# parseablehq/parseable

Measured on AMD Instinct MI355X. Metric: rows/sec scanned (SELECT...WHERE...GROUP BY, Parseable parquet dialect), higher is better.
Workload: dtype int64; 1 GPU; c2s; query=SELECT host,count(*),max(latency) WHERE ts BETWEEN ... GROUP BY host, rows_per_gpu=100000000, parallelism=dp1

## Files before the change

### include/gpuq.h

```cpp
#ifndef GPUQ_H
#define GPUQ_H

#include <stdint.h>

#ifdef __cplusplus
extern "C" {
#endif

typedef struct gpuq_ctx gpuq_ctx;
typedef struct gpuq_plan gpuq_plan;

#ifndef ARROW_C_DATA_INTERFACE
#define ARROW_C_DATA_INTERFACE
struct ArrowSchema {
  const char* format;
  const char* name;
  const char* metadata;
  int64_t flags;
  int64_t n_children;
  struct ArrowSchema** children;
  struct ArrowSchema* dictionary;
  void (*release)(struct ArrowSchema*);
  void* private_data;
};
struct ArrowArray {
  int64_t length;
  int64_t null_count;
  int64_t offset;
  int64_t n_buffers;
  int64_t n_children;
  const void** buffers;
  struct ArrowArray** children;
  struct ArrowArray* dictionary;
  void (*release)(struct ArrowArray*);
  void* private_data;
};
#endif
#ifndef ARROW_C_STREAM_INTERFACE
#define ARROW_C_STREAM_INTERFACE
struct ArrowArrayStream {
  int (*get_schema)(struct ArrowArrayStream*, struct ArrowSchema* out);
  int (*get_next)(struct ArrowArrayStream*, struct ArrowArray* out);
  const char* (*get_last_error)(struct ArrowArrayStream*);
  void (*release)(struct ArrowArrayStream*);
  void* private_data;
};
#endif


typedef struct {
  const char* path;
  const int32_t* row_groups;
  int32_t n_row_groups;
} gpuq_file;

typedef enum {
  GPUQ_EQ = 0, GPUQ_NE, GPUQ_LT, GPUQ_LE, GPUQ_GT, GPUQ_GE,
  GPUQ_BETWEEN,
  GPUQ_CONTAINS,
  GPUQ_ICONTAINS = 8,
  GPUQ_STARTS_WITH,
  GPUQ_ENDS_WITH,
  GPUQ_NOT_CONTAINS,
  GPUQ_NOT_ICONTAINS,
  GPUQ_NOT_STARTS_WITH,
  GPUQ_NOT_ENDS_WITH,
  GPUQ_IS_NULL,
  GPUQ_IS_NOT_NULL
} gpuq_op;

typedef enum { GPUQ_LIT_I64 = 0, GPUQ_LIT_F64, GPUQ_LIT_STR } gpuq_lit;

typedef struct {
  const char* column;
  int32_t op;
  int32_t lit_kind;
  int64_t i64[2];
  double f64[2];
  const char* str;
  int32_t hi_exclusive;
} gpuq_pred;

typedef enum {
  GPUQ_AGG_COUNT_STAR = 0, GPUQ_AGG_COUNT, GPUQ_AGG_SUM,
  GPUQ_AGG_MIN, GPUQ_AGG_MAX,
  GPUQ_AGG_COUNT_DISTINCT
} gpuq_agg_op;

typedef struct { int32_t op; const char* column; } gpuq_agg;


gpuq_ctx* gpuq_session_create(uint64_t device_mask);
void gpuq_session_destroy(gpuq_ctx*);
const char* gpuq_last_error(gpuq_ctx*);


gpuq_plan* gpuq_plan_build(gpuq_ctx*,
    const gpuq_file* files, int32_t n_files,
    const char* const* projection, int32_t n_projection,
    const gpuq_pred* preds, int32_t n_preds,
    const char* const* group_by, int32_t n_group_by,
    const gpuq_agg* aggs, int32_t n_aggs,
    int64_t limit);

gpuq_plan* gpuq_plan_build_from_stream(gpuq_ctx*, const char* stream_dir,
    const char* const* projection, int32_t n_projection,
    const gpuq_pred* preds, int32_t n_preds,
    const char* const* group_by, int32_t n_group_by,
    const gpuq_agg* aggs, int32_t n_aggs, int64_t limit,
    int64_t* fast_count);

int32_t gpuq_plan_partition_count(gpuq_plan*);

int32_t gpuq_plan_load(gpuq_plan*, int32_t partition);

int32_t gpuq_plan_execute(gpuq_plan*, int32_t partition,
                          struct ArrowArrayStream* out);

typedef struct {
  int64_t rows_scanned;
  int64_t rows_out;
  int64_t bytes_scanned;
  int64_t rowgroup_bytes_total;
  int64_t hbm_bytes_est;
  int64_t kernel_ns;
  int64_t exec_ns;
  int64_t load_ns;
  int64_t decomp_ns;
  int64_t cache_hit_bytes;
} gpuq_metrics;
int32_t gpuq_plan_metrics(gpuq_plan*, gpuq_metrics* out);

void gpuq_plan_destroy(gpuq_plan*);

int32_t gpuq_device_count(void);



typedef struct {
  int32_t codec;
  const uint8_t* comp;
  uint32_t comp_len;
  uint32_t uncomp_len;
} gpuq_decomp_page;

enum {
  GPUQ_DECOMP_AUTO = 0,
  GPUQ_DECOMP_FORCE_SEGMENT,
  GPUQ_DECOMP_FORCE_LITPAR,
  GPUQ_DECOMP_FORCE_FALLBACK
};
#define GPUQ_DECOMP_HOST_ONLY   0x100
#define GPUQ_DECOMP_HOST_REPLAY 0x200

enum {
  GPUQ_DECOMP_PAGE_SEGMENT = 0,
  GPUQ_DECOMP_PAGE_LITPAR,
  GPUQ_DECOMP_PAGE_FALLBACK,
  GPUQ_DECOMP_PAGE_RAW,
  GPUQ_DECOMP_PAGE_HOST_IMAGE
};

typedef struct {
  int32_t mode;
  uint32_t n_seq;
  uint32_t n_segs, n_big;
  uint32_t n_lit_lane, n_lit_wave;
  uint32_t n_inl;
  uint32_t n_res_lane, n_res_wave;
  uint32_t n_pieces;
  uint32_t n_backrefs, n_far;
} gpuq_decomp_stats;

int32_t gpuq_test_decompress(gpuq_ctx*, const gpuq_decomp_page* pages,
                             int32_t n_pages, int32_t raw_lead, int32_t mode,
                             uint8_t sentinel, uint8_t* out, uint64_t out_cap,
                             uint64_t* arena_len, uint64_t* guard_len,
                             gpuq_decomp_stats* stats, int32_t* d_err);

#ifdef __cplusplus
}
#endif
#endif
```

### parseable_amd/_lib.py

```python

from __future__ import annotations

import ctypes as C
import os

_DIR = os.path.dirname(os.path.abspath(__file__))
LIB_PATH = os.path.join(_DIR, "libgpuq.so")


class GpuqFile(C.Structure):
    _fields_ = [
        ("path", C.c_char_p),
        ("row_groups", C.POINTER(C.c_int32)),
        ("n_row_groups", C.c_int32),
    ]


class GpuqPred(C.Structure):
    _fields_ = [
        ("column", C.c_char_p),
        ("op", C.c_int32),
        ("lit_kind", C.c_int32),
        ("i64", C.c_int64 * 2),
        ("f64", C.c_double * 2),
        ("str", C.c_char_p),
        ("hi_exclusive", C.c_int32),
    ]


class GpuqAgg(C.Structure):
    _fields_ = [("op", C.c_int32), ("column", C.c_char_p)]


class GpuqMetrics(C.Structure):
    _fields_ = [
        ("rows_scanned", C.c_int64),
        ("rows_out", C.c_int64),
        ("bytes_scanned", C.c_int64),
        ("rowgroup_bytes_total", C.c_int64),
        ("hbm_bytes_est", C.c_int64),
        ("kernel_ns", C.c_int64),
        ("exec_ns", C.c_int64),
        ("load_ns", C.c_int64),
        ("decomp_ns", C.c_int64),
        ("cache_hit_bytes", C.c_int64),
    ]


class GpuqDecompPage(C.Structure):
    _fields_ = [
        ("codec", C.c_int32),
        ("comp", C.c_void_p),
        ("comp_len", C.c_uint32),
        ("uncomp_len", C.c_uint32),
    ]


class GpuqDecompStats(C.Structure):
    _fields_ = [("mode", C.c_int32)] + [
        (n, C.c_uint32) for n in (
            "n_seq", "n_segs", "n_big", "n_lit_lane", "n_lit_wave", "n_inl",
            "n_res_lane", "n_res_wave", "n_pieces", "n_backrefs", "n_far")
    ]


DECOMP_MODES = {"auto": 0, "segment": 1, "litpar": 2, "fallback": 3}
DECOMP_HOST_ONLY = 0x100
DECOMP_HOST_REPLAY = 0x200
DECOMP_PATHS = ("segment", "litpar", "fallback", "raw", "host_image")
CODECS = {"uncompressed": 0, "snappy": 1, "lz4_raw": 7}

OPS = {"eq": 0, "ne": 1, "lt": 2, "le": 3, "gt": 4, "ge": 5, "between": 6, "contains": 7,
       "icontains": 8, "starts_with": 9, "ends_with": 10, "not_contains": 11,
       "not_icontains": 12, "not_starts_with": 13, "not_ends_with": 14,
       "is_null": 15, "is_not_null": 16}
STR_OPS = ("contains", "icontains", "starts_with", "ends_with", "not_contains",
           "not_icontains", "not_starts_with", "not_ends_with")
NULL_OPS = ("is_null", "is_not_null")
AGGS = {"count_star": 0, "count": 1, "sum": 2, "min": 3, "max": 4,
        "count_distinct": 5}

_lib = None


def load():
    global _lib
    if _lib is not None:
        return _lib
    if not os.path.exists(LIB_PATH):
        raise RuntimeError(
            f"libgpuq.so not built at {LIB_PATH} — run __graft_entry__.build(). "
            "parseable_amd has no CPU fallback."
        )
    lib = C.CDLL(LIB_PATH)
    lib.gpuq_session_create.restype = C.c_void_p
    lib.gpuq_session_create.argtypes = [C.c_uint64]
    lib.gpuq_session_destroy.argtypes = [C.c_void_p]
    lib.gpuq_last_error.restype = C.c_char_p
    lib.gpuq_last_error.argtypes = [C.c_void_p]
    lib.gpuq_device_count.restype = C.c_int32
    lib.gpuq_plan_build_from_stream.restype = C.c_void_p
    lib.gpuq_plan_build_from_stream.argtypes = [
        C.c_void_p, C.c_char_p,
        C.POINTER(C.c_char_p), C.c_int32,
        C.POINTER(GpuqPred), C.c_int32,
        C.POINTER(C.c_char_p), C.c_int32,
        C.POINTER(GpuqAgg), C.c_int32,
        C.c_int64, C.POINTER(C.c_int64),
    ]
    lib.gpuq_plan_build.restype = C.c_void_p
    lib.gpuq_plan_build.argtypes = [
        C.c_void_p,
        C.POINTER(GpuqFile), C.c_int32,
        C.POINTER(C.c_char_p), C.c_int32,
        C.POINTER(GpuqPred), C.c_int32,
        C.POINTER(C.c_char_p), C.c_int32,
        C.POINTER(GpuqAgg), C.c_int32,
        C.c_int64,
    ]
    lib.gpuq_plan_partition_count.restype = C.c_int32
    lib.gpuq_plan_partition_count.argtypes = [C.c_void_p]
    lib.gpuq_plan_load.restype = C.c_int32
    lib.gpuq_plan_load.argtypes = [C.c_void_p, C.c_int32]
    lib.gpuq_plan_execute.restype = C.c_int32
    lib.gpuq_plan_execute.argtypes = [C.c_void_p, C.c_int32, C.c_void_p]
    lib.gpuq_plan_metrics.restype = C.c_int32
    lib.gpuq_plan_metrics.argtypes = [C.c_void_p, C.POINTER(GpuqMetrics)]
    lib.gpuq_plan_destroy.argtypes = [C.c_void_p]
    lib.gpuq_test_decompress.restype = C.c_int32
    lib.gpuq_test_decompress.argtypes = [
        C.c_void_p, C.POINTER(GpuqDecompPage), C.c_int32, C.c_int32, C.c_int32,
        C.c_uint8, C.c_void_p, C.c_uint64,
        C.POINTER(C.c_uint64), C.POINTER(C.c_uint64),
        C.POINTER(GpuqDecompStats), C.POINTER(C.c_int32),
    ]
    _lib = lib
    return lib


def device_count() -> int:
    return load().gpuq_device_count()


def decompress_pages(pages, mode="auto", raw_lead=0, host=None, session=None,
                     sentinel=0xA5):
    lib = load()
    n = len(pages)
    arr = (GpuqDecompPage * max(n, 1))()
    keep = []
    cap = 16384 + 64
    for i, (codec, comp, uncomp) in enumerate(pages):
        buf = C.create_string_buffer(bytes(comp), max(len(comp), 1))
        keep.append(buf)
        arr[i] = GpuqDecompPage(CODECS[codec], C.addressof(buf), len(comp), uncomp)
        cap += (uncomp + 15) & ~15
    flags = DECOMP_MODES[mode] | {None: 0, "decode": DECOMP_HOST_ONLY,
                                  "replay": DECOMP_HOST_REPLAY}[host]
    out = C.create_string_buffer(cap)
    arena_len, guard_len, d_err = C.c_uint64(), C.c_uint64(), C.c_int32()
    stats = (GpuqDecompStats * max(n, 1))()
    rc = lib.gpuq_test_decompress(
        session if host is None else None, arr, n, raw_lead, flags, sentinel,
        out, cap, C.byref(arena_len), C.byref(guard_len), stats, C.byref(d_err))
    if rc != 0:
        msg = lib.gpuq_last_error(session if host is None else None)
        raise RuntimeError(msg.decode(errors="replace"))
    st = []
    for i in range(n):
        d = {f: getattr(stats[i], f) for f, _ in GpuqDecompStats._fields_}
        d["mode"] = DECOMP_PATHS[d["mode"]]
        st.append(d)
    return out.raw[:arena_len.value], st, guard_len.value, d_err.value
```

### parseable_amd/csrc/dev_types.h

```cpp
#pragma once
#include <cstdint>

namespace gpuq {

struct DevPage {
  uint64_t src_off;
  uint64_t dst_off;
  uint32_t comp_size;
  uint32_t uncomp_size;
  uint32_t num_values;
  uint32_t row_start;
  uint32_t aux;
  uint32_t aux_val;
  uint32_t aux_lut;
  uint32_t dict_n;
  uint8_t  optional;
  uint8_t  raw_copy;
  uint8_t  encoding;
  uint8_t  phys;
};

struct DevSeg {
  uint64_t src_off;
  uint64_t dst_off;
  uint32_t comp_len;
  uint32_t out_len;
  uint8_t big;
  uint8_t raw;
};
struct DevBr {
  uint64_t dst, src;
  uint32_t len;
  uint32_t _pad;
};
struct DevPageBr { uint32_t start, count; };
struct DevBrRes {
  uint64_t dst;
  uint32_t len, off;
  uint32_t piece_start, piece_n;
};
struct DevPiece { uint64_t src; uint32_t len; uint32_t _pad; };
struct DevLit { uint64_t a, b; };
struct DevBrInl { uint64_t meta, pat; };
struct DevCWin {
  uint64_t src;
  uint64_t starts;
  uint32_t nbytes;
  uint32_t n_values;
  uint32_t dense0;
  int32_t page_id;
};

enum CmpMode { CMP_EQ = 0, CMP_NE, CMP_LT, CMP_LE, CMP_GT, CMP_GE, CMP_RANGE };

enum StrKind { STR_CONTAINS = 0, STR_PREFIX = 1, STR_SUFFIX = 2 };
enum { STRF_KIND = 3, STRF_FOLD = 4, STRF_NEG = 8 };
enum { CMP_STR_LIKE = 16 };
constexpr int cmp_str_like(int mode) { return CMP_STR_LIKE | mode; }
constexpr int cmp_str_like_mode(int op) {
  return (op & CMP_STR_LIKE) ? (op & ~CMP_STR_LIKE) : -1;
}

enum { AGGK_COUNT_STAR = 0, AGGK_COUNT, AGGK_SUM_I64, AGGK_SUM_F64,
       AGGK_MIN_I64, AGGK_MAX_I64, AGGK_MIN_F64, AGGK_MAX_F64,
       AGGK_MIN_RANK, AGGK_MAX_RANK,
       AGGK_MIN_STR, AGGK_MAX_STR,
       AGGK_COUNT_DISTINCT };

constexpr int MAX_KEYS = 4;
constexpr int MAX_AGGS = 8;

struct AggArgs {
  const uint8_t* mask;
  int64_t n_rows;
  int n_keys;
  const int32_t* key_gid[MAX_KEYS];
  int32_t key_size[MAX_KEYS];
  int n_aggs;
  int32_t agg_kind[MAX_AGGS];
  const int64_t* agg_val[MAX_AGGS];
  const uint8_t* agg_valid[MAX_AGGS];
  uint8_t cnt_skip[MAX_AGGS];
  int32_t fsum_idx[MAX_AGGS];
  int32_t fsum_n;
  uint64_t* fsum;
  const uint8_t* dec;
  uint64_t* table;
  int32_t n_groups;
  int32_t* err;
};

struct DistinctArgs {
  const uint8_t* mask;
  int64_t n_rows;
  int n_keys;
  const int32_t* key_gid[MAX_KEYS];
  int32_t key_size[MAX_KEYS];
  int32_t n_groups;
  const int32_t* vgid;
  int32_t vcard;
  uint64_t* pairs;
  uint32_t* count;
  uint32_t pair_cap;
  int32_t* err;
};

enum { ERR_NONE = 0, ERR_LZ4 = 1, ERR_RLE = 2, ERR_DELTA = 3, ERR_DICT_RANGE = 4,
       ERR_PAGE = 5, ERR_FSUM_RANGE = 6, ERR_HASH_CAP = 7, ERR_HASH_PROBE = 8,
       ERR_PAIR_CAP = 9, ERR_PAIR_PROBE = 10, ERR_DISTINCT_CAP = 11,
       ERR_DISTINCT_PROBE = 12 };

}
```

### parseable_amd/csrc/gpuq.cpp

```cpp
#include "../../include/gpuq.h"
#include "catalog.h"
#include "meta.h"
#include "kernels_api.h"
#include "dev_types.h"

#include <hip/hip_runtime.h>
#include <fcntl.h>
#include <sys/mman.h>
#include <sys/stat.h>
#include <unistd.h>

#include <algorithm>
#include <array>
#include <atomic>
#include <cstring>
#include <thread>
#include <map>
#include <memory>
#include <mutex>
#include <string>
#include <unordered_map>
#include <vector>

using namespace gpuq;
// ... 42 lines not shown
    std::lock_guard<std::mutex> g(cache_mu);
    auto it = cache.find(key);
    if (it == cache.end() || it->second.bytes != expect_bytes) return false;
    it->second.refs++;
    it->second.last_use = ++cache_clock;
    return true;
  }
  void cache_unpin(const std::string& key) {
    std::lock_guard<std::mutex> g(cache_mu);
    auto it = cache.find(key);
    if (it != cache.end() && it->second.refs > 0) it->second.refs--;
  }
  void* cache_get(const std::string& key) {
    std::lock_guard<std::mutex> g(cache_mu);
    auto it = cache.find(key);
    return it == cache.end() ? nullptr : it->second.dev;
  }
  void cache_put(const std::string& key, void* dev, size_t bytes, int device) {
    std::lock_guard<std::mutex> g(cache_mu);
    if (cache.count(key)) { (void)hipFree(dev); return; }
    while (cache_bytes + bytes > cache_budget) {
      auto victim = cache.end();
      for (auto it = cache.begin(); it != cache.end(); ++it)
        if (it->second.refs == 0 &&
            (victim == cache.end() ||
             it->second.last_use < victim->second.last_use))
          victim = it;
      if (victim == cache.end()) break;
      (void)hipSetDevice(victim->second.device);
      (void)hipFree(victim->second.dev);
      cache_bytes -= victim->second.bytes;
      cache.erase(victim);
    }
    CacheEntry e;
    e.dev = dev;
    e.bytes = bytes;
    e.device = device;
    e.last_use = ++cache_clock;
    cache.emplace(key, e);
    cache_bytes += bytes;
  }
};

namespace {

struct MappedFile {
  std::string path;
  int fd = -1;
  const uint8_t* data = nullptr;
  size_t size = 0;
  int64_t mtime_ns = 0;
  FileMeta meta;
  ~MappedFile() {
    if (data) munmap((void*)data, size);
    if (fd >= 0) close(fd);
  }
};

struct ColPlan {
  std::string name;
  int phys = -1;
  bool optional = false;
  bool need_gid = false;
  bool need_val = false;
  bool val_always = false;
  bool hash_mode = false;
  bool numeric_key = false;
  bool need_gid_valid = false;
  bool distinct_val = false;
  std::vector<int> lut_preds;
  std::vector<int> cmp_preds;
  std::vector<int> contains_preds;
  std::vector<int> null_preds;
  bool need_rank = false;
  bool is_bin = false;
  int bin_src = -1;
  int64_t bin_stride = 0, bin_origin = 0, bin_min_idx = 0;
  int32_t nbins = 0;
  std::vector<int32_t> rank_to_gid;
  std::vector<std::string> gdict;
  std::unordered_map<std::string, int32_t> gmap;
  int32_t gid_of(const std::string& s) {
    auto it = gmap.find(s);
    if (it != gmap.end()) return it->second;
    gdict.push_back(s);
    int32_t id = (int32_t)gdict.size();
    gmap.emplace(gdict.back(), id);
    return id;
  }
};

struct PredPlan {
  gpuq_pred p;
  std::string col, str_lit;
};

struct AggPlan {
  int op;
  std::string col;
  int col_idx = -1;
  int kind = 0;
  bool is_f64 = false;
  bool cnt_is_presence = false;
  int fsum_idx = -1;
};

struct ChunkTask {
  int file_idx, rg_idx, col_idx;
  size_t dictv_pool_base = (size_t)-1;
  uint64_t raw_off = 0;
  const ColumnChunkMeta* cm = nullptr;
  std::vector<PageInfo> pages;
  std::vector<int32_t> remap;
  std::vector<int64_t> dictv;
  std::vector<uint8_t> lut;
  bool has_plain_data_pages = false;
  std::vector<int64_t> strof;
  std::vector<int64_t> pvals;
  std::vector<uint32_t> pval_page_n;
  std::vector<uint32_t> pval_base;
  uint64_t dict_dst = (uint64_t)-1;
  std::string cache_key;
  bool cached = false;
  uint64_t dec_base = 0, dec_len = 0;
};

struct RgRef {
  int file_idx, rg_idx;
  int64_t rows = 0, needed_bytes = 0, total_bytes = 0;
  uint32_t row_start = 0;
};

enum TaskKind { TK_DICT_GID, TK_DICT_VAL, TK_PLAIN_VAL, TK_DELTA_VAL,
                TK_DICT_MASK, TK_BYTES_CONTAINS, TK_POOL_VAL,
                TK_IS_NULL, TK_IS_NOT_NULL,
                TK_N };

struct Partition {
  int device = -1;
  std::vector<RgRef> rgs;
  int64_t n_rows = 0;
  std::vector<ChunkTask> chunks;
  std::vector<DevPage> pages;
  std::vector<int32_t> ids[TK_N];
  std::map<std::pair<int,int>, std::vector<int32_t>> tasks;
  std::vector<int32_t> remap_pool;
  std::vector<int64_t> dictv_pool;
  std::vector<uint8_t> lut_pool;
  std::vector<DevSeg> segs;
  std::vector<DevBr> brs;
  std::vector<DevPageBr> pagebrs;
  std::vector<DevBrRes> res_lane, res_wave;
  std::vector<DevPiece> piece_pool;
  std::vector<DevBrInl> brinl;
  std::vector<DevLit> lits_lane, lits_wave;
  std::vector<DevCWin> cwins;
  std::vector<uint16_t> cstarts;
  std::map<int, std::pair<uint32_t, uint32_t>> cwin_ranges;
  uint64_t raw_bytes = 0, dec_bytes = 0;
  int64_t bytes_scanned = 0, rowgroup_bytes_total = 0;
  int64_t bytes_cache_hit = 0;
  bool populated = false;
  std::map<int, std::vector<std::pair<int64_t, int64_t>>> pred_ranges;
  std::vector<std::pair<uint64_t, std::vector<uint8_t>>> himgs;

  bool loaded = false;
  hipStream_t stream = nullptr;
  uint8_t *d_raw = nullptr, *d_dec = nullptr;
  DevPage* d_pages = nullptr;
  int32_t* d_remap = nullptr;
  int64_t* d_dictv = nullptr;
  uint8_t* d_lut = nullptr;
  uint8_t* d_mask = nullptr;
  int32_t* d_err = nullptr;
  uint64_t* d_table = nullptr;
  uint64_t* d_fsum = nullptr;
  uint64_t* d_hkeys = nullptr;
  int32_t* d_hgids = nullptr;
  uint32_t* d_hcount = nullptr;
  std::map<int, uint64_t*> d_gid2ref;
  std::map<int, uint32_t> hash_claimed;
  int32_t* d_cgid = nullptr;
  std::vector<uint64_t*> d_gid2pair;
  int32_t* d_agg_kind = nullptr;
  uint8_t* d_needle = nullptr;
  std::vector<uint32_t> needle_off;
  uint32_t* d_rowof = nullptr;
  uint32_t* d_rank = nullptr;
  uint8_t* d_scr = nullptr;
  uint32_t* d_present = nullptr;
  uint8_t* d_tmpvalid = nullptr;
  int32_t* d_all_ids = nullptr;
  DevSeg* d_segs = nullptr;
  DevBr* d_brs = nullptr;
  DevPageBr* d_pagebrs = nullptr;
  DevBrRes* d_res_lane = nullptr;
  DevBrRes* d_res_wave = nullptr;
  DevBrInl* d_brinl = nullptr;
  DevPiece* d_piece_pool = nullptr;
  DevLit* d_lits_lane = nullptr;
  DevLit* d_lits_wave = nullptr;
  DevCWin* d_cwins = nullptr;
  uint16_t* d_cstarts = nullptr;
  int64_t* d_keys = nullptr;
  int64_t* d_keys_sorted = nullptr;
  uint32_t* d_rows = nullptr;
  uint32_t* d_rows_sorted = nullptr;
  unsigned long long* d_count = nullptr;
  void* d_sort_temp = nullptr;
  size_t sort_temp_bytes = 0;
  std::map<std::pair<int,int>, int32_t*> d_ids;
  std::map<int, int32_t*> d_gid;
  std::map<int, int64_t*> d_val;
  std::map<int, uint8_t*> d_valid;
  std::vector<uint8_t> col_null_free;
  std::vector<int32_t> valagg_ids;
  int32_t* d_valagg_ids = nullptr;
  uint64_t* d_dbitmap = nullptr;
  std::vector<uint64_t*> d_dpairs;
  uint32_t* d_dcount = nullptr;
  int64_t load_ns = 0;
};

struct Ring {
  static constexpr size_t BUFSZ = 256ull << 20;
  static constexpr int NBUF = 4;
  void* bufs[NBUF] = {};
  hipEvent_t evts[NBUF] = {};
  hipStream_t stream;
  int b = 0;
  explicit Ring(hipStream_t st);
  ~Ring();
  struct Span { const uint8_t* src; uint64_t len; };
  void copy_spans(uint8_t* d_dst, const std::vector<Span>& spans);
  void copy(void* d_dst, const void* src, size_t len);
};

}

namespace {
constexpr int HASH_LOG2 = 24;
constexpr int32_t GID_CAP = 1 << 22;
constexpr uint32_t DISTINCT_PAIR_CAP = 1u << 23;
constexpr uint64_t DISTINCT_BITMAP_BITS = 1ull << 28;
constexpr uint64_t DISTINCT_LDS_BITS = 1ull << 17;
}

struct gpuq_plan {
  gpuq_ctx* ctx = nullptr;
  std::vector<std::unique_ptr<MappedFile>> files;
  std::vector<ColPlan> cols;
  std::vector<PredPlan> preds;
  std::vector<AggPlan> aggs;
  std::vector<int> group_cols;
  std::vector<int> projection;
  bool is_projection = false;
  int ts_col = -1;
  int64_t limit = -1;
  std::vector<Partition> parts;
  int32_t n_groups = 0;
  int32_t n_fsum = 0;
  bool has_hash = false;
  bool needs_cascade = false;
  bool has_numkey = false;
  std::vector<std::string> pinned_keys;
  int64_t m_cache_hit_bytes = 0;
  bool fused_count = false;
  bool fused_valagg = false;
  int valagg_col = -1;
  bool valagg_late = false;
  int valagg_blocks = 1024;
  bool exec_dbg = false;
  std::vector<int> distinct_aggs;
  uint64_t distinct_bitmap_bits = DISTINCT_BITMAP_BITS;
  uint64_t distinct_lds_bits = DISTINCT_LDS_BITS;
  uint32_t distinct_pair_cap = DISTINCT_PAIR_CAP;
  bool distinct_force_hash = false;
  std::mutex mu;
  int64_t m_rows_scanned = 0, m_rows_out = 0, m_kernel_ns = 0, m_exec_ns = 0,
          m_load_ns = 0, m_decomp_ns = 0, m_hbm_est = 0;
  ~gpuq_plan();
};

extern "C" gpuq_ctx* gpuq_session_create(uint64_t device_mask) {
  auto* c = new gpuq_ctx();
  int n = 0;
  if (hipGetDeviceCount(&n) != hipSuccess) n = 0;
  if (n == 0 && getenv("GPUQ_FAKE_DEVICE")) n = 1;
  for (int i = 0; i < 64 && i < n; i++)
    if (device_mask & (1ull << i)) c->devices.push_back(i);
  if (c->devices.empty() && device_mask == 0 && n > 0) c->devices.push_back(0);
  return c;
}
extern "C" void gpuq_session_destroy(gpuq_ctx* c) { delete c; }
namespace {
thread_local std::string g_null_ctx_error = "null ctx";
}
extern "C" const char* gpuq_last_error(gpuq_ctx* c) {
  return c ? c->last_error.c_str() : g_null_ctx_error.c_str();
}
extern "C" int32_t gpuq_device_count(void) {
  int n = 0;
  if (hipGetDeviceCount(&n) != hipSuccess) return -1;
  return n;
}

namespace {

int find_or_add_col(std::vector<ColPlan>& cols, const std::string& name) {
  for (size_t i = 0; i < cols.size(); i++)
    if (cols[i].name == name) return (int)i;
  cols.push_back(ColPlan{});
  cols.back().name = name;
  return (int)cols.size() - 1;
}

bool op_is_like(int op) {
  return op == GPUQ_CONTAINS || (op >= GPUQ_ICONTAINS && op <= GPUQ_NOT_ENDS_WITH);
}
bool op_is_null(int op) { return op == GPUQ_IS_NULL || op == GPUQ_IS_NOT_NULL; }
int like_mode(int op) {
  switch (op) {
    case GPUQ_ICONTAINS: return STR_CONTAINS | STRF_FOLD;
    case GPUQ_STARTS_WITH: return STR_PREFIX;
    case GPUQ_ENDS_WITH: return STR_SUFFIX;
    case GPUQ_NOT_CONTAINS: return STR_CONTAINS | STRF_NEG;
    case GPUQ_NOT_ICONTAINS: return STR_CONTAINS | STRF_FOLD | STRF_NEG;
    case GPUQ_NOT_STARTS_WITH: return STR_PREFIX | STRF_NEG;
    case GPUQ_NOT_ENDS_WITH: return STR_SUFFIX | STRF_NEG;
    default: return STR_CONTAINS;
  }
}
const char* op_name(int op) {
  static const char* names[] = {
      "eq", "ne", "lt", "le", "gt", "ge", "between", "contains", "icontains",
      "starts_with", "ends_with", "not_contains", "not_icontains",
      "not_starts_with", "not_ends_with", "is_null", "is_not_null"};
  return (op >= 0 && op <= GPUQ_IS_NOT_NULL) ? names[op] : "?";
}

enum NullState { NULLP_EVAL = 0, NULLP_PROVEN, NULLP_UNSAT };
NullState null_pred_state(int op, const ColumnChunkMeta& cm, bool optional) {
  const bool none_null = !optional || cm.null_count == 0;
  const bool all_null = optional && cm.null_count >= 0 &&
                        cm.null_count == cm.num_values && cm.num_values > 0;
  if (op == GPUQ_IS_NOT_NULL)
    return none_null ? NULLP_PROVEN : all_null ? NULLP_UNSAT : NULLP_EVAL;
  return none_null ? NULLP_UNSAT : all_null ? NULLP_PROVEN : NULLP_EVAL;
}

bool rg_pruned_by_stats(const gpuq_plan& plan, const FileMeta& fm,
                        const RowGroupMeta& rg) {
  for (const auto& pp : plan.preds) {
// ... 97 lines not shown
  if (codec == CODEC_LZ4_RAW) {
    int n = lz4_decompress_host(src, comp, buf.data(), buf.size());
    if (n == (int)uncomp) return buf.data();
    if (comp == uncomp) return src;
    throw std::runtime_error("page lz4 failure");
  }
  if (codec == CODEC_SNAPPY) {
    int n = snappy_decompress_host(src, comp, buf.data(), buf.size());
    if (n == (int)uncomp) return buf.data();
    throw std::runtime_error("page snappy failure");
  }
  throw std::runtime_error("unsupported codec");
}

uint32_t parse_def1(const uint8_t* data, uint32_t nv, std::vector<uint8_t>& defs) {
  uint32_t dl;
  memcpy(&dl, data, 4);
  defs.assign(nv, 1);
  const uint8_t* p = data + 4;
  const uint8_t* end = p + dl;
  uint32_t v = 0;
  while (v < nv && p < end) {
    uint64_t hdr = 0;
    int sh = 0;
    for (;;) {
      uint8_t b = *p++;
      hdr |= (uint64_t)(b & 0x7f) << sh;
      if (!(b & 0x80)) break;
      sh += 7;
    }
    if (hdr & 1) {
      uint32_t groups = (uint32_t)(hdr >> 1);
      for (uint32_t g = 0; g < groups; g++) {
        uint8_t byte = p[g];
        for (int j = 0; j < 8; j++) {
          uint32_t idx = v + g * 8 + j;
          if (idx < nv) defs[idx] = (byte >> j) & 1;
        }
      }
      p += groups;
      uint32_t add = groups * 8;
      v += add > nv - v ? nv - v : add;
    } else {
      uint32_t cnt = (uint32_t)(hdr >> 1);
      uint8_t val = *p++;
      if (cnt > nv - v) cnt = nv - v;
      std::fill(defs.begin() + v, defs.begin() + v + cnt, val);
      v += cnt;
    }
  }
  return 4 + dl;
}

int64_t now_ns() {
  struct timespec ts;
  clock_gettime(CLOCK_MONOTONIC, &ts);
  return (int64_t)ts.tv_sec * 1000000000 + ts.tv_nsec;
}

template <class F>
void parallel_for(size_t n, F&& fn, size_t max_threads = 0) {
  if (n == 0) return;
  size_t hw = std::thread::hardware_concurrency();
  if (hw == 0) hw = 8;
  static const size_t env_cap = [] {
    const char* e = getenv("GPUQ_HOST_THREADS");
    return e ? (size_t)strtoul(e, nullptr, 10) : (size_t)0;
  }();
  if (env_cap) hw = std::min(hw, env_cap);
  if (max_threads) hw = std::min(hw, max_threads);
  size_t nthreads = std::min(n, hw);
  if (nthreads <= 1) {
    for (size_t i = 0; i < n; i++) fn(i);
    return;
  }
  std::atomic<size_t> next{0};
  std::mutex emu;
  std::exception_ptr eptr;
  auto worker = [&]() {
    for (;;) {
      size_t i = next.fetch_add(1);
      if (i >= n) return;
      try {
        fn(i);
      } catch (...) {
        std::lock_guard<std::mutex> g(emu);
        if (!eptr) eptr = std::current_exception();
        next.store(n);
        return;
      }
    }
  };
  std::vector<std::thread> pool;
  pool.reserve(nthreads);
  for (size_t t = 0; t < nthreads; t++) pool.emplace_back(worker);
  for (auto& th : pool) th.join();
  if (eptr) std::rethrow_exception(eptr);
}

Ring::Ring(hipStream_t st) : stream(st) {
  for (int i = 0; i < NBUF; i++) {
    HIP_TRY(hipHostMalloc(&bufs[i], BUFSZ));
    HIP_TRY(hipEventCreate(&evts[i]));
    HIP_TRY(hipEventRecord(evts[i], stream));
  }
}
Ring::~Ring() {
  for (int i = 0; i < NBUF; i++) {
    if (bufs[i]) (void)hipHostFree(bufs[i]);
    if (evts[i]) (void)hipEventDestroy(evts[i]);
  }
}
void Ring::copy_spans(uint8_t* d_dst, const std::vector<Span>& spans) {
  size_t si = 0;
  uint64_t soff = 0, dst = 0;
  while (si < spans.size()) {
    if (spans[si].len == 0) { si++; continue; }
    HIP_TRY(hipEventSynchronize(evts[b]));
    struct Fill { const uint8_t* src; uint8_t* dstp; size_t len; };
    std::vector<Fill> fills;
    size_t filled = 0;
    while (si < spans.size() && filled < BUFSZ) {
      uint64_t take = std::min<uint64_t>(spans[si].len - soff, BUFSZ - filled);
      while (take > 0) {
        uint64_t piece = std::min<uint64_t>(take, 4ull << 20);
        fills.push_back({spans[si].src + soff, (uint8_t*)bufs[b] + filled,
                         piece});
        filled += piece;
        soff += piece;
        take -= piece;
      }
      if (soff == spans[si].len) { si++; soff = 0; }
    }
    parallel_for(fills.size(), [&](size_t f) {
      memcpy(fills[f].dstp, fills[f].src, fills[f].len);
    }, 32);
    HIP_TRY(hipMemcpyAsync(d_dst + dst, bufs[b], filled,
                           hipMemcpyHostToDevice, stream));
    HIP_TRY(hipEventRecord(evts[b], stream));
    dst += filled;
    b = (b + 1) % NBUF;
  }
}
void Ring::copy(void* d_dst, const void* src, size_t len) {
  if (len) copy_spans((uint8_t*)d_dst, {{(const uint8_t*)src, len}});
}

struct DecompRecs {
  std::vector<DevSeg> segs;
  std::vector<DevBr> brs;
  std::vector<DevPageBr> pagebrs;
  std::vector<DevBrRes> res_lane, res_wave;
  std::vector<DevPiece> piece_pool;
  std::vector<DevBrInl> brinl;
  std::vector<DevLit> lits_lane, lits_wave;
  std::vector<std::pair<uint64_t, std::vector<uint8_t>>> himgs;
};

constexpr uint32_t BR_FAR = 16384 / 2;

void plan_decomp_page(DecompRecs& cb, int codec, const uint8_t* praw,
                      uint64_t src_abs, uint64_t dst_abs, uint32_t comp,
                      uint32_t uncomp, bool raw_page,
                      int force = GPUQ_DECOMP_AUTO,
                      gpuq_decomp_stats* st = nullptr) {
  Lz4Plan lp;
  if (st) *st = gpuq_decomp_stats{};
  if (!raw_page && codec == CODEC_SNAPPY) {
    lp = snappy_walk(praw, comp, uncomp);
    if (st) st->n_seq = lp.n_seq;
    if (lp.fallback) {
      std::vector<uint8_t> img(uncomp);
      if (snappy_decompress_host(praw, comp, img.data(), uncomp) !=
          (int)uncomp)
        throw std::runtime_error("snappy page decode failure");
      cb.himgs.emplace_back(dst_abs, std::move(img));
      if (st) st->mode = GPUQ_DECOMP_PAGE_HOST_IMAGE;
      return;
    }
  } else if (!raw_page) {
    static const bool env_fb =
        std::getenv("GPUQ_FORCE_LZ4_FALLBACK") != nullptr;
    const bool force_fb = force == GPUQ_DECOMP_FORCE_FALLBACK ||
                          (force == GPUQ_DECOMP_AUTO && env_fb);
    try {
      lp = lz4_walk(praw, comp, uncomp, 8192);
      if (force_fb) {
        lp.fallback = true;
        lp.resolved.clear();
        lp.pieces.clear();
      }
      const bool want_litpar =
          force == GPUQ_DECOMP_FORCE_LITPAR ||
          (force == GPUQ_DECOMP_AUTO && lp.n_seq >= 256 &&
           uncomp / lp.n_seq < 96);
      if (!lp.fallback && want_litpar) {
        Lz4Plan lp2 = lz4_walk(praw, comp, uncomp, 8192, true);
        if (!lp2.fallback) lp = std::move(lp2);
      }
    } catch (const std::exception&) {
      if (comp == uncomp) raw_page = true;
      else throw;
    }
    if (st) st->n_seq = lp.n_seq;
  }
  if (raw_page) {
    DevSeg sgl{};
    sgl.src_off = src_abs;
    sgl.dst_off = dst_abs;
    sgl.comp_len = comp;
    sgl.out_len = uncomp;
    sgl.raw = 1;
    cb.segs.push_back(sgl);
    if (st) {
      st->mode = GPUQ_DECOMP_PAGE_RAW;
      st->n_seq = 0;
      st->n_segs = 1;
    }
    return;
  }
  if (st) {
    st->mode = lp.fallback ? GPUQ_DECOMP_PAGE_FALLBACK
               : lp.litpar ? GPUQ_DECOMP_PAGE_LITPAR
                           : GPUQ_DECOMP_PAGE_SEGMENT;
    st->n_segs = (uint32_t)lp.segs.size();
    for (const auto& sg : lp.segs) st->n_big += sg.big != 0;
  }
  for (const auto& sg : lp.segs) {
    DevSeg d2{};
    d2.src_off = src_abs + sg.s_off;
    d2.dst_off = dst_abs + sg.d_off;
    d2.comp_len = sg.comp_len;
    d2.out_len = sg.out_len;
    d2.big = sg.big;
    cb.segs.push_back(d2);
  }
  for (const auto& lt : lp.lits) {
    DevLit dl{(src_abs + lt.src) | ((uint64_t)lt.len << 40),
              dst_abs + lt.dst};
    (lt.len <= 256 ? cb.lits_lane : cb.lits_wave).push_back(dl);
    if (st) (lt.len <= 256 ? st->n_lit_lane : st->n_lit_wave)++;
  }
  if (lp.fallback) {
    DevPageBr pb{(uint32_t)cb.brs.size(), (uint32_t)lp.backrefs.size()};
    cb.pagebrs.push_back(pb);
    for (const auto& br : lp.backrefs) {
      cb.brs.push_back({dst_abs + br.dst, dst_abs + br.src, br.len, 0});
      if (st) {
        st->n_backrefs++;
        st->n_far += (br.dst - br.src) + br.len > BR_FAR;
      }
    }
  } else if (!lp.resolved.empty()) {
    auto lit_bytes = [&](uint32_t src, uint32_t len,
                         uint8_t* out) -> bool {
      const auto& Ls = lp.lits;
      size_t lo = 0, hi = Ls.size();
      while (lo < hi) {
        size_t mid = (lo + hi) / 2;
        if (Ls[mid].dst <= src) lo = mid + 1;
        else hi = mid;
      }
      if (lo == 0) return false;
      const Lz4Lit& L = Ls[lo - 1];
      if (src < L.dst || src + len > L.dst + L.len) return false;
      std::memcpy(out, praw + L.src + (src - L.dst), len);
      return true;
    };
    for (const auto& rr : lp.resolved) {
      uint32_t pat_len = 0;
      for (uint32_t k = 0; k < rr.piece_n; k++)
        pat_len += lp.pieces[rr.piece_start + k].len;
      if (lp.litpar && pat_len > 0 && pat_len <= 8 && rr.len <= 256) {
        uint8_t buf[8] = {0};
        uint32_t o = 0;
        bool ok = true;
        for (uint32_t k = 0; k < rr.piece_n && ok; k++) {
          const Lz4Piece& pc = lp.pieces[rr.piece_start + k];
          ok = lit_bytes(pc.src, pc.len, buf + o);
          o += pc.len;
        }
        if (ok) {
          uint64_t pat;
          std::memcpy(&pat, buf, 8);
          cb.brinl.push_back({(dst_abs + rr.dst) |
                                  ((uint64_t)rr.len << 40) |
                                  ((uint64_t)pat_len << 52),
                              pat});
          if (st) st->n_inl++;
          continue;
        }
      }
      uint32_t ps = (uint32_t)cb.piece_pool.size();
      for (uint32_t k = 0; k < rr.piece_n; k++) {
        const Lz4Piece& pc = lp.pieces[rr.piece_start + k];
        cb.piece_pool.push_back({dst_abs + pc.src, pc.len, 0});
      }
      DevBrRes rec{dst_abs + rr.dst, rr.len, rr.off, ps, rr.piece_n};
      if (rr.len <= 256) cb.res_lane.push_back(rec);
      else cb.res_wave.push_back(rec);
      if (st) {
        (rr.len <= 256 ? st->n_res_lane : st->n_res_wave)++;
        st->n_pieces += rr.piece_n;
      }
    }
  }
}

struct DecompDev {
  const uint8_t* d_raw;
  uint8_t* d_dec;
  const DevSeg* d_segs; int n_segs;
  const DevLit* d_lits_lane; int64_t n_lits_lane;
  const DevLit* d_lits_wave; int n_lits_wave;
  const DevBrInl* d_brinl; int64_t n_brinl;
  const DevBrRes* d_res_lane; int64_t n_res_lane;
  const DevBrRes* d_res_wave; int n_res_wave;
  const DevPiece* d_piece_pool;
  const DevBr* d_brs;
  const DevPageBr* d_pagebrs; int n_pagebrs;
  int32_t* d_err;
};

void launch_decompress(hipStream_t st, const DecompDev& d) {
  launch_lz4_seg(st, d.d_raw, d.d_dec, d.d_segs, d.n_segs, d.d_err);
  launch_lit_lane(st, d.d_raw, d.d_dec, d.d_lits_lane, d.n_lits_lane);
  launch_lit_wave(st, d.d_raw, d.d_dec, d.d_lits_wave, d.n_lits_wave);
  launch_brres_inl(st, d.d_dec, d.d_brinl, d.n_brinl);
  launch_brres_lane(st, d.d_dec, d.d_res_lane, d.d_piece_pool, d.n_res_lane);
  launch_brres_wave(st, d.d_dec, d.d_res_wave, d.d_piece_pool, d.n_res_wave);
  launch_lz4_backrefs(st, d.d_dec, d.d_brs, d.d_pagebrs, d.n_pagebrs);
}

}

extern "C" gpuq_plan* gpuq_plan_build(
    gpuq_ctx* ctx, const gpuq_file* files, int32_t n_files,
    const char* const* projection, int32_t n_projection,
    const gpuq_pred* preds, int32_t n_preds,
    const char* const* group_by, int32_t n_group_by,
    const gpuq_agg* aggs, int32_t n_aggs, int64_t limit) try {
  (void)projection; (void)n_projection;
  auto plan = std::make_unique<gpuq_plan>();
  plan->ctx = ctx;
  plan->limit = limit;
  if (ctx->devices.empty())
    throw std::runtime_error("no GPU devices in session (gpuq never falls back to CPU)");
  if (n_files <= 0)
    throw std::runtime_error("empty file list: caller should use the empty-relation path "
                             "(provider returns the empty aggregate without a scan)");

  plan->files.resize(n_files);
  parallel_for((size_t)n_files, [&](size_t i) {
    auto mf = std::make_unique<MappedFile>();
    mf->path = files[i].path;
    mf->fd = open(files[i].path, O_RDONLY);
    if (mf->fd < 0) throw std::runtime_error("cannot open " + mf->path);
    struct stat st;
    fstat(mf->fd, &st);
    mf->size = st.st_size;
    mf->mtime_ns = (int64_t)st.st_mtim.tv_sec * 1000000000 + st.st_mtim.tv_nsec;
    mf->data = (const uint8_t*)mmap(nullptr, mf->size, PROT_READ, MAP_PRIVATE, mf->fd, 0);
    if (mf->data == MAP_FAILED) throw std::runtime_error("mmap failed: " + mf->path);
    mf->meta = parse_footer(mf->data, mf->size);
    plan->files[i] = std::move(mf);
  });
  const FileMeta& fm0 = plan->files[0]->meta;

  for (int32_t i = 0; i < n_preds; i++) {
    PredPlan pp;
    pp.p = preds[i];
    pp.col = preds[i].column;
    if (pp.p.op < GPUQ_EQ || pp.p.op > GPUQ_IS_NOT_NULL)
      throw std::runtime_error("unknown predicate op on " + pp.col);
    if (!op_is_null(pp.p.op) && preds[i].str) pp.str_lit = preds[i].str;
    plan->preds.push_back(std::move(pp));
  }
  for (int32_t i = 0; i < n_group_by; i++) {
    std::string g = group_by[i];
    if (g.rfind("__bin:", 0) == 0) {
      size_t a = 6, b = g.find(':', a), c2 = g.find(':', b + 1);
      std::string src = g.substr(a, b - a);
      int ci = find_or_add_col(plan->cols, g);
      auto& bc = plan->cols[ci];
      bc.is_bin = true;
      bc.bin_stride = std::stoll(g.substr(b + 1, c2 - b - 1));
      bc.bin_origin = std::stoll(g.substr(c2 + 1));
      if (bc.bin_stride <= 0) throw std::runtime_error("bad bin stride");
      int si = find_or_add_col(plan->cols, src);
      plan->cols[si].need_val = true;
      plan->cols[si].val_always = true;
      plan->cols[ci].bin_src = si;
      plan->group_cols.push_back(ci);
      continue;
    }
    int ci = find_or_add_col(plan->cols, g);
    plan->cols[ci].need_gid = true;
    plan->group_cols.push_back(ci);
  }
  for (int32_t i = 0; i < n_aggs; i++) {
    AggPlan ap;
    ap.op = aggs[i].op;
    if (aggs[i].op == GPUQ_AGG_COUNT_DISTINCT) {
      if (!aggs[i].column)
        throw std::runtime_error("count_distinct needs a column");
      if (n_projection > 0)
        throw std::runtime_error(
            "count_distinct is not allowed in a projection plan");
    }
    if (aggs[i].op != GPUQ_AGG_COUNT_STAR) {
      ap.col = aggs[i].column;
      ap.col_idx = find_or_add_col(plan->cols, ap.col);
    }
    plan->aggs.push_back(std::move(ap));
  }
  for (auto& c : plan->cols) {
    if (c.is_bin) continue;
    int si = fm0.col_index(c.name);
    if (si < 0) throw std::runtime_error("no such column: " + c.name);
    c.phys = fm0.columns[si].phys_type;
    c.optional = fm0.columns[si].optional;
    if (c.need_gid && c.phys != PT_BYTE_ARRAY) {
      if (c.phys == PT_INT64 || c.phys == PT_INT32 || c.phys == PT_DOUBLE) {
        c.need_gid = false;
        c.numeric_key = true;
        c.need_val = true;
        c.val_always = true;
        plan->has_numkey = true;
      } else {
        throw std::runtime_error(
            "unsupported group-key type (utf8/i64/i32/f64/timestamp): " +
            c.name);
      }
    }
  }
  for (size_t pi = 0; pi < plan->preds.size(); pi++) {
    auto& pp = plan->preds[pi];
    int ci = find_or_add_col(plan->cols, pp.col);
    auto& c = plan->cols[ci];
    if (c.phys == -1) {
      int si = fm0.col_index(c.name);
      if (si < 0) throw std::runtime_error("no such column: " + c.name);
      c.phys = fm0.columns[si].phys_type;
      c.optional = fm0.columns[si].optional;
    }
    if (op_is_null(pp.p.op)) {
      if (c.phys != PT_BYTE_ARRAY && c.phys != PT_INT64 &&
          c.phys != PT_INT32 && c.phys != PT_DOUBLE)
        throw std::runtime_error("unsupported predicate column type: " + pp.col);
      c.null_preds.push_back((int)pi);
      continue;
    }
    if (op_is_like(pp.p.op) && pp.p.op != GPUQ_CONTAINS &&
        c.phys != PT_BYTE_ARRAY)
      throw std::runtime_error(std::string("string predicate ") +
                               op_name(pp.p.op) + " on non-utf8 column: " +
                               pp.col);
    if (c.phys == PT_BYTE_ARRAY) {
      if (pp.p.lit_kind != GPUQ_LIT_STR)
        throw std::runtime_error("string column needs string literal: " + pp.col);
      if (op_is_like(pp.p.op) && (like_mode(pp.p.op) & STRF_FOLD)) {
        for (char& ch : pp.str_lit) {
          if ((unsigned char)ch >= 0x80)
            throw std::runtime_error(
                std::string(op_name(pp.p.op)) + " literal must be ASCII "
                "(case folding is ASCII-only): " + pp.col);
          if (ch >= 'A' && ch <= 'Z') ch = (char)(ch | 0x20);
        }
      }
      if (op_is_like(pp.p.op)) c.contains_preds.push_back((int)pi);
      c.lut_preds.push_back((int)pi);
    } else if (c.phys == PT_INT64 || c.phys == PT_INT32) {
      if (pp.p.lit_kind != GPUQ_LIT_I64)
        throw std::runtime_error("int column needs int literal: " + pp.col);
      c.cmp_preds.push_back((int)pi);
      c.need_val = true;
    } else if (c.phys == PT_DOUBLE) {
      if (pp.p.lit_kind != GPUQ_LIT_F64)
        throw std::runtime_error("double column needs float literal: " + pp.col);
      c.cmp_preds.push_back((int)pi);
      c.need_val = true;
// ... 413 lines not shown
        if (pi.type != PAGE_DATA) continue;
        uint64_t pg_dst = part.dec_bytes;
        pid_cursor++;
        part.dec_bytes += ((uint64_t)pi.uncomp_size + 15) & ~15ull;
        if (c.hash_mode && pi.encoding == ENC_PLAIN) {
          t.pval_base.push_back((uint32_t)part.dictv_pool.size());
          uint32_t nvp = t.pval_page_n[plain_i++];
          for (uint32_t k = 0; k < nvp; k++)
            part.dictv_pool.push_back((int64_t)(pg_dst + (uint64_t)t.pvals[pv_off + k]));
          pv_off += nvp;
        }
      }
      t.dec_len = part.dec_bytes - t.dec_base;
      {
        const auto& mf2 = *plan->files[t.file_idx];
        t.cache_key = mf2.path + "\x01" + std::to_string(mf2.size) + ":" +
                      std::to_string(mf2.mtime_ns) + ":" +
                      std::to_string(t.rg_idx) + ":" + c.name +
                      (c.hash_mode ? ":h" : "");
        if (ctx->cache_pin(t.cache_key, (size_t)t.dec_len)) {
          t.cached = true;
          plan->pinned_keys.push_back(t.cache_key);
          part.bytes_cache_hit += (int64_t)t.cm->total_compressed_size;
        }
      }
    }

    phase_mark("phase3 pools+cache");

    struct CItem {
      const uint8_t* praw;
      int32_t comp, uncomp, page_id;
      uint64_t dst_off;
      uint32_t num_values;
      bool optional;
      int codec;
      int col;
    };
    std::vector<CItem> citems;
    struct CB : DecompRecs {
      std::vector<DevPage> pages;
      std::map<std::pair<int,int>, std::vector<int32_t>> tasks;
      std::vector<CItem> citems;
    };
    std::vector<CB> cbs(part.chunks.size());
    parallel_for(part.chunks.size(), [&](size_t ti) {
      auto& t = part.chunks[ti];
      auto& c = plan->cols[t.col_idx];
      auto& cb = cbs[ti];
      const auto& mf = *plan->files[t.file_idx];
      const uint32_t remap_base = bases[ti].remap;
      const uint32_t dictv_base = bases[ti].dictv;
      const uint32_t lut_base = bases[ti].lut;
      uint64_t dec_off = bases[ti].dec;
      int32_t page_id = bases[ti].pid;
      const uint32_t rstart = stubs[ti].rstart;

      const int chunk_codec = t.cm->codec;
      auto plan_decomp = [&](const uint8_t* praw, uint64_t src_abs,
                             uint64_t dst_abs, uint32_t comp, uint32_t uncomp,
                             bool raw_page) {
        plan_decomp_page(cb, chunk_codec, praw, src_abs, dst_abs, comp, uncomp,
                         raw_page);
      };

      if (c.hash_mode) {
        for (auto& pi : t.pages) {
          if (pi.type != PAGE_DICT) continue;
          if (!t.cached)
            plan_decomp(mf.data + pi.payload_off,
                        t.raw_off + (uint64_t)(pi.payload_off - t.cm->start_offset()),
                        t.dict_dst, pi.comp_size, pi.uncomp_size,
                        t.cm->codec == CODEC_UNCOMPRESSED);
          dec_off += ((uint64_t)pi.uncomp_size + 15) & ~15ull;
        }
      }

      uint32_t row_in_rg = 0;
      size_t plain_i4 = 0;
      for (auto& pi : t.pages) {
        if (pi.type != PAGE_DATA) continue;
        DevPage dp{};
        dp.src_off = t.raw_off + (uint64_t)(pi.payload_off - t.cm->start_offset());
        dp.dst_off = dec_off;
        dec_off += ((uint64_t)pi.uncomp_size + 15) & ~15ull;
        dp.comp_size = pi.comp_size;
        dp.uncomp_size = pi.uncomp_size;
        dp.num_values = pi.num_values;
        dp.row_start = rstart + row_in_rg;
        row_in_rg += pi.num_values;
        dp.optional = mf.meta.columns[mf.meta.col_index(c.name)].optional;
        dp.raw_copy = (t.cm->codec == CODEC_UNCOMPRESSED);
        dp.dict_n = (uint32_t)std::max(
            {t.remap.size(), t.dictv.size(), t.lut.size(), t.strof.size()});
        dp.encoding = (uint8_t)pi.encoding;
        dp.phys = (uint8_t)c.phys;
        const int32_t this_pid = page_id++;
        if (!t.cached)
          plan_decomp(mf.data + pi.payload_off, dp.src_off, dp.dst_off,
                      pi.comp_size, pi.uncomp_size, dp.raw_copy != 0);
        bool dict_enc = (pi.encoding == ENC_RLE_DICT || pi.encoding == ENC_PLAIN_DICT);
        if (c.need_gid && dict_enc && !c.hash_mode) {
          dp.aux = remap_base;
          cb.tasks[{TK_DICT_GID, t.col_idx}].push_back(this_pid);
        }
        if (c.need_val && stubs[ti].need_val_decode) {
          if (c.hash_mode) {
            if (dict_enc) {
              dp.aux_val = dictv_base;
              cb.tasks[{TK_DICT_VAL, t.col_idx}].push_back(this_pid);
            } else if (pi.encoding == ENC_PLAIN) {
              dp.aux_val = t.pval_base[plain_i4++];
              cb.tasks[{TK_POOL_VAL, t.col_idx}].push_back(this_pid);
            } else throw std::runtime_error("unsupported encoding for hash col");
          } else if (dict_enc) {
            dp.aux_val = dictv_base;
            cb.tasks[{TK_DICT_VAL, t.col_idx}].push_back(this_pid);
          } else if (pi.encoding == ENC_PLAIN) {
            cb.tasks[{TK_PLAIN_VAL, t.col_idx}].push_back(this_pid);
          } else if (pi.encoding == ENC_DELTA_BP) {
            cb.tasks[{TK_DELTA_VAL, t.col_idx}].push_back(this_pid);
          } else throw std::runtime_error("unsupported encoding for values");
        }
        if (!c.lut_preds.empty() && !c.hash_mode) {
          if (dict_enc) {
            dp.aux_lut = lut_base;
            cb.tasks[{TK_DICT_MASK, t.col_idx}].push_back(this_pid);
          } else if (pi.encoding == ENC_PLAIN) {
            if ((int)c.contains_preds.size() != (int)c.lut_preds.size())
              throw std::runtime_error("non-LIKE predicate on PLAIN utf8 pages: next row");
            cb.tasks[{TK_BYTES_CONTAINS, t.col_idx}].push_back(this_pid);
            cb.citems.push_back({mf.data + pi.payload_off, pi.comp_size,
                                 pi.uncomp_size, this_pid, dp.dst_off,
                                 (uint32_t)pi.num_values, dp.optional != 0,
                                 t.cm->codec, t.col_idx});
          } else throw std::runtime_error("unsupported encoding for string predicate");
        }
        if (stubs[ti].need_is_null)
          cb.tasks[{TK_IS_NULL, t.col_idx}].push_back(this_pid);
        if (stubs[ti].need_is_not_null)
          cb.tasks[{TK_IS_NOT_NULL, t.col_idx}].push_back(this_pid);
        cb.pages.push_back(dp);
      }
      if (row_in_rg != (uint32_t)mf.meta.row_groups[t.rg_idx].num_rows)
        throw std::runtime_error("page rows mismatch");
    });

    phase_mark("phase4 lz4 walks");

    {
      const size_t nc = cbs.size();
      std::vector<size_t> o_pages(nc + 1, 0), o_segs(nc + 1, 0),
          o_brs(nc + 1, 0), o_pagebrs(nc + 1, 0), o_rl(nc + 1, 0),
          o_rw(nc + 1, 0), o_pp(nc + 1, 0), o_bi(nc + 1, 0),
          o_ll(nc + 1, 0), o_lw(nc + 1, 0);
      for (size_t i = 0; i < nc; i++) {
        const auto& cb = cbs[i];
        o_pages[i + 1] = o_pages[i] + cb.pages.size();
        o_segs[i + 1] = o_segs[i] + cb.segs.size();
        o_brs[i + 1] = o_brs[i] + cb.brs.size();
        o_pagebrs[i + 1] = o_pagebrs[i] + cb.pagebrs.size();
        o_rl[i + 1] = o_rl[i] + cb.res_lane.size();
        o_rw[i + 1] = o_rw[i] + cb.res_wave.size();
        o_pp[i + 1] = o_pp[i] + cb.piece_pool.size();
        o_bi[i + 1] = o_bi[i] + cb.brinl.size();
        o_ll[i + 1] = o_ll[i] + cb.lits_lane.size();
        o_lw[i + 1] = o_lw[i] + cb.lits_wave.size();
      }
      part.pages.resize(o_pages[nc]);
      part.segs.resize(o_segs[nc]);
      part.brs.resize(o_brs[nc]);
      part.pagebrs.resize(o_pagebrs[nc]);
      part.res_lane.resize(o_rl[nc]);
      part.res_wave.resize(o_rw[nc]);
      part.piece_pool.resize(o_pp[nc]);
      part.brinl.resize(o_bi[nc]);
      part.lits_lane.resize(o_ll[nc]);
      part.lits_wave.resize(o_lw[nc]);
      parallel_for(nc, [&](size_t i) {
        auto& cb = cbs[i];
        std::copy(cb.pages.begin(), cb.pages.end(),
                  part.pages.begin() + o_pages[i]);
        std::copy(cb.segs.begin(), cb.segs.end(),
                  part.segs.begin() + o_segs[i]);
        std::copy(cb.brs.begin(), cb.brs.end(), part.brs.begin() + o_brs[i]);
        const uint32_t br_base = (uint32_t)o_brs[i];
        for (size_t j = 0; j < cb.pagebrs.size(); j++) {
          DevPageBr pb = cb.pagebrs[j];
          pb.start += br_base;
          part.pagebrs[o_pagebrs[i] + j] = pb;
        }
        std::copy(cb.piece_pool.begin(), cb.piece_pool.end(),
                  part.piece_pool.begin() + o_pp[i]);
        const uint32_t piece_base = (uint32_t)o_pp[i];
        for (size_t j = 0; j < cb.res_lane.size(); j++) {
          DevBrRes r2 = cb.res_lane[j];
          r2.piece_start += piece_base;
          part.res_lane[o_rl[i] + j] = r2;
        }
        for (size_t j = 0; j < cb.res_wave.size(); j++) {
          DevBrRes r2 = cb.res_wave[j];
          r2.piece_start += piece_base;
          part.res_wave[o_rw[i] + j] = r2;
        }
        std::copy(cb.brinl.begin(), cb.brinl.end(),
                  part.brinl.begin() + o_bi[i]);
        std::copy(cb.lits_lane.begin(), cb.lits_lane.end(),
                  part.lits_lane.begin() + o_ll[i]);
        std::copy(cb.lits_wave.begin(), cb.lits_wave.end(),
                  part.lits_wave.begin() + o_lw[i]);
      });
      for (size_t i = 0; i < nc; i++) {
        auto& cb = cbs[i];
        for (auto& [key, ids] : cb.tasks) {
          auto& dstv = part.tasks[key];
          dstv.insert(dstv.end(), ids.begin(), ids.end());
        }
        citems.insert(citems.end(), cb.citems.begin(), cb.citems.end());
        for (auto& h : cb.himgs)
          part.himgs.emplace_back(h.first, std::move(h.second));
      }
    }
    phase_mark("phase5 merge");
    part.dec_bytes += 16384 + 64;

    if (!citems.empty()) {
      struct CLocal {
        std::vector<DevCWin> wins;
        std::vector<uint16_t> starts;
      };
      std::vector<CLocal> locals(citems.size());
      std::atomic<size_t> next{0};
      std::atomic<bool> failed{false};
      auto worker = [&]() {
        std::vector<uint8_t> img, defs;
        for (;;) {
          size_t i = next.fetch_add(1);
          if (i >= citems.size() || failed.load()) return;
          const auto& it = citems[i];
          auto& L = locals[i];
          const uint8_t* data;
          try {
            data = host_page_payload(it.codec, it.praw, it.comp, it.uncomp,
                                     img);
          } catch (const std::exception&) {
            failed.store(true);
            return;
          }
          uint32_t pos = 0;
          const uint32_t nv = it.num_values;
          bool has_def = false;
          if (it.optional) {
            uint32_t dl;
            std::memcpy(&dl, data, 4);
            defs.assign(nv, 1);
            const uint8_t* p = data + 4;
            const uint8_t* end = p + dl;
            uint32_t v = 0;
            while (v < nv && p < end) {
              uint64_t hdr = 0;
              int sh = 0;
              for (;;) {
                uint8_t b = *p++;
                hdr |= (uint64_t)(b & 0x7f) << sh;
                if (!(b & 0x80)) break;
                sh += 7;
              }
              if (hdr & 1) {
                uint32_t groups = (uint32_t)(hdr >> 1);
                for (uint32_t g = 0; g < groups; g++) {
                  uint8_t byte = p[g];
                  for (int j = 0; j < 8; j++) {
                    uint32_t idx = v + g * 8 + j;
                    if (idx < nv) defs[idx] = (byte >> j) & 1;
                  }
                }
                p += groups;
                uint32_t add = groups * 8;
                v += add > nv - v ? nv - v : add;
              } else {
                uint32_t cnt = (uint32_t)(hdr >> 1);
                uint8_t val = *p++;
                if (cnt > nv - v) cnt = nv - v;
                std::fill(defs.begin() + v, defs.begin() + v + cnt, val);
                v += cnt;
              }
            }
            pos = 4 + dl;
            has_def = true;
          }
          uint32_t dense = 0;
          int64_t wfirst = -1;
          uint32_t wbytes = 0, wvals = 0, wdense0 = 0;
          auto flush = [&]() {
            if (wfirst < 0) return;
            L.wins.push_back({it.dst_off + (uint64_t)wfirst,
                              (uint64_t)(L.starts.size() - wvals), wbytes,
                              wvals, wdense0, it.page_id});
            wfirst = -1;
            wbytes = wvals = 0;
          };
          for (uint32_t vI = 0; vI < nv; vI++) {
            if (has_def && !defs[vI]) continue;
            if (pos + 4 > (uint32_t)it.uncomp) { failed.store(true); return; }
            uint32_t len;
            std::memcpy(&len, data + pos, 4);
            uint64_t rec = 4ull + len;
            if (pos + rec > (uint64_t)it.uncomp) { failed.store(true); return; }
            if (rec > 16384) {
              flush();
              L.starts.push_back(0);
              L.wins.push_back({it.dst_off + pos, L.starts.size() - 1,
                                (uint32_t)rec, 1, dense, it.page_id});
            } else {
              if (wfirst >= 0 && wbytes + rec > 16384) flush();
              if (wfirst < 0) { wfirst = pos; wdense0 = dense; }
              L.starts.push_back((uint16_t)(pos - wfirst));
              wbytes += (uint32_t)rec;
              wvals++;
            }
            pos += (uint32_t)rec;
            dense++;
          }
          flush();
        }
      };
      size_t nthreads = std::min<size_t>(
          std::max(1u, std::thread::hardware_concurrency()), citems.size());
      std::vector<std::thread> pool;
      for (size_t i = 0; i < nthreads; i++) pool.emplace_back(worker);
      for (auto& th : pool) th.join();
      if (failed.load())
        throw std::runtime_error("contains window walk failed (corrupt page)");
      std::map<int32_t, size_t> by_page;
      for (size_t i = 0; i < citems.size(); i++) by_page[citems[i].page_id] = i;
      for (auto& [key, ids] : part.tasks) {
        if (key.first != TK_BYTES_CONTAINS) continue;
        uint32_t off = (uint32_t)part.cwins.size();
        for (int32_t pid : ids) {
          const auto& L = locals[by_page.at(pid)];
          uint64_t sbase = part.cstarts.size();
          part.cstarts.insert(part.cstarts.end(), L.starts.begin(),
                              L.starts.end());
          for (DevCWin w : L.wins) {
            w.starts += sbase;
            part.cwins.push_back(w);
          }
        }
        part.cwin_ranges[key.second] = {off, (uint32_t)part.cwins.size() - off};
      }
    }
  }

  for (auto& c : plan->cols) {
    if (!c.is_bin) continue;
    const auto& src = plan->cols[c.bin_src];
    bool any = false;
    int64_t mn = 0, mx = 0;
    for (auto& part : plan->parts)
      for (auto& r : part.rgs) {
        const auto& mf = *plan->files[r.file_idx];
        int si = mf.meta.col_index(src.name);
        const auto& cm = mf.meta.row_groups[r.rg_idx].chunks[si];
        if (!cm.has_i64_stats)
          throw std::runtime_error("DATE_BIN needs footer i64 stats on " + src.name);
        if (!any) { mn = cm.stat_min; mx = cm.stat_max; any = true; }
        else { mn = std::min(mn, cm.stat_min); mx = std::max(mx, cm.stat_max); }
      }
    auto fdiv = [](int64_t v, int64_t s) {
      return v >= 0 ? v / s : -((-v + s - 1) / s);
    };
    c.bin_min_idx = any ? fdiv(mn - c.bin_origin, c.bin_stride) : 0;
    int64_t max_idx = any ? fdiv(mx - c.bin_origin, c.bin_stride) : 0;
    int64_t nb = max_idx - c.bin_min_idx + 1;
    if (nb > (1 << 21)) throw std::runtime_error("too many DATE_BIN bins");
    c.nbins = (int32_t)std::max<int64_t>(nb, 1);
  }

  int64_t g = 1;
  for (int ci : plan->group_cols) {
    const auto& c = plan->cols[ci];
    int64_t sz = c.is_bin ? (int64_t)c.nbins + 1 : (int64_t)c.gdict.size() + 1;
    g = (g > (int64_t)GID_CAP) ? g : g * sz;
  }
  if (g > (int64_t)GID_CAP) {
    plan->needs_cascade = true;
    g = GID_CAP;
  }
  plan->n_groups = (int32_t)g;

  for (auto& part : plan->parts)
    plan->m_rows_scanned += part.n_rows;

  for (auto& ap : plan->aggs) {
    if (ap.op == GPUQ_AGG_COUNT_STAR || ap.col_idx < 0) continue;
    bool all0 = true;
    for (auto& part : plan->parts)
      for (auto& t : part.chunks)
        if (t.col_idx == ap.col_idx && t.cm->null_count != 0) all0 = false;
    ap.cnt_is_presence = all0;
  }

  for (size_t ci = 0; ci < plan->cols.size(); ci++) {
    auto& c = plan->cols[ci];
    if (!c.need_rank) continue;
    std::vector<int32_t> order((size_t)c.gdict.size());
    for (size_t i = 0; i < order.size(); i++) order[i] = (int32_t)i;
    std::sort(order.begin(), order.end(), [&](int32_t a, int32_t b) {
      return c.gdict[a] < c.gdict[b];
    });
    std::vector<int64_t> rank_of_gid(c.gdict.size() + 1, 0);
    c.rank_to_gid.assign(c.gdict.size(), 0);
    for (size_t r = 0; r < order.size(); r++) {
      rank_of_gid[(size_t)order[r] + 1] = (int64_t)r;
      c.rank_to_gid[r] = order[r] + 1;
    }
    for (auto& part : plan->parts)
      for (auto& t : part.chunks)
        if (t.col_idx == (int)ci && t.dictv_pool_base != (size_t)-1)
          for (size_t k = 0; k < t.dictv.size(); k++)
            part.dictv_pool[t.dictv_pool_base + k] =
                rank_of_gid[(size_t)part.dictv_pool[t.dictv_pool_base + k]];
  }

  {
    bool aggs_ok = true;
    for (auto& ap : plan->aggs) aggs_ok &= (ap.kind == AGGK_COUNT_STAR);
    plan->fused_count = plan->group_cols.size() == 1 && aggs_ok &&
                        plan->preds.empty() && plan->n_groups <= 8192 &&
                        !plan->cols[plan->group_cols[0]].is_bin &&
                        !plan->cols[plan->group_cols[0]].hash_mode &&
                        !plan->cols[plan->group_cols[0]].numeric_key;
  }

  for (auto& part : plan->parts) {
    part.col_null_free.assign(plan->cols.size(), 1);
    for (auto& t : part.chunks)
      if (t.cm->null_count != 0) part.col_null_free[t.col_idx] = 0;
  }

  plan->exec_dbg = getenv("GPUQ_PLAN_DEBUG") != nullptr;
  if (const char* e = getenv("GPUQ_VALAGG_BLOCKS"))
    plan->valagg_blocks = std::max(1, atoi(e));
  if (const char* e = getenv("GPUQ_DISTINCT_BITMAP_BITS"))
    plan->distinct_bitmap_bits =
        std::min<uint64_t>(strtoull(e, nullptr, 10), 1ull << 31);
  if (const char* e = getenv("GPUQ_DISTINCT_LDS_BITS"))
    plan->distinct_lds_bits =
        std::min<uint64_t>(strtoull(e, nullptr, 10), 64 * 1024 * 8);
  if (const char* e = getenv("GPUQ_DISTINCT_PAIR_CAP"))
    plan->distinct_pair_cap = (uint32_t)std::min<uint64_t>(
        std::max<uint64_t>(strtoull(e, nullptr, 10), 1), DISTINCT_PAIR_CAP);
  if (const char* e = getenv("GPUQ_DISTINCT_FORCE_HASH"))
    plan->distinct_force_hash = atoi(e) != 0;
  if (!plan->distinct_aggs.empty()) plan->fused_count = false;
  if (!plan->is_projection && !getenv("GPUQ_NO_FUSED_VALAGG") &&
      plan->distinct_aggs.empty() &&
      plan->group_cols.size() == 1 && plan->aggs.size() == 2 &&
      plan->aggs[0].kind == AGGK_COUNT_STAR && plan->n_fsum == 0 &&
      (plan->aggs[1].kind == AGGK_SUM_I64 || plan->aggs[1].kind == AGGK_MIN_I64 ||
       plan->aggs[1].kind == AGGK_MAX_I64) &&
      plan->aggs[1].cnt_is_presence && !plan->needs_cascade) {
    const int vc = plan->aggs[1].col_idx;
    const auto& c = plan->cols[vc];
    const auto& kc = plan->cols[plan->group_cols[0]];
    bool ok = c.phys == PT_INT64 && !c.is_bin && !c.hash_mode &&
              !c.numeric_key && !c.need_gid && !c.need_rank &&
              c.cmp_preds.empty() && c.lut_preds.empty() &&
              c.null_preds.empty() &&
              plan->group_cols[0] != vc;
    for (auto& o : plan->cols) ok &= !(o.is_bin && o.bin_src == vc);
    const bool late = kc.hash_mode || kc.numeric_key;
    if (!late) ok &= (int64_t)plan->n_groups * 16 <= 64 * 1024;
    for (auto& part : plan->parts) {
      if (!ok) break;
      for (auto& kv : part.tasks) {
        if (kv.first.second != vc) continue;
        if (kv.first.first != TK_DICT_VAL && kv.first.first != TK_PLAIN_VAL)
          ok = false;
      }
    }
    if (ok) {
      plan->fused_valagg = true;
      plan->valagg_col = vc;
      plan->valagg_late = late;
      for (auto& part : plan->parts) {
        for (int k : {TK_DICT_VAL, TK_PLAIN_VAL}) {
          auto it = part.tasks.find({k, vc});
          if (it != part.tasks.end())
            part.valagg_ids.insert(part.valagg_ids.end(), it->second.begin(),
                                   it->second.end());
        }
        std::sort(part.valagg_ids.begin(), part.valagg_ids.end());
      }
    }
  }

  if (getenv("GPUQ_PLAN_DEBUG")) {
    fprintf(stderr, "[gpuq plan] fused_count=%d fused_valagg=%d%s\n",
            (int)plan->fused_count, (int)plan->fused_valagg,
            plan->fused_valagg && plan->valagg_late
                ? " (group count checked at execute)" : "");
    for (int ai : plan->distinct_aggs) {
      const auto& c = plan->cols[plan->aggs[ai].col_idx];
      fprintf(stderr, "[gpuq plan] distinct agg=%d col=%s gids=%s\n", ai,
              c.name.c_str(),
              c.numeric_key ? "numeric" : c.hash_mode ? "hash" : "dict");
    }
    for (size_t p = 0; p < plan->parts.size(); p++) {
      const auto& pt = plan->parts[p];
      fprintf(stderr,
              "[gpuq plan] part %zu: rows=%lld chunks=%zu pages=%zu segs=%zu "
              "lits=%zu/%zu brinl=%zu res=%zu/%zu pieces=%zu raw=%.2fGB "
              "dec=%.2fGB cwins=%zu\n",
              p, (long long)pt.n_rows, pt.chunks.size(), pt.pages.size(),
              pt.segs.size(), pt.lits_lane.size(), pt.lits_wave.size(),
              pt.brinl.size(), pt.res_lane.size(), pt.res_wave.size(),
              pt.piece_pool.size(), pt.raw_bytes / 1e9, pt.dec_bytes / 1e9,
              pt.cwins.size());
    }
    for (size_t pi = 0; pi < plan->preds.size(); pi++) {
      const auto& pp = plan->preds[pi];
      std::string path;
      if (op_is_like(pp.p.op)) {
        int ci = find_or_add_col(plan->cols, pp.col);
        if (plan->cols[ci].hash_mode) {
          path = "hash";
        } else {
          bool lut = false, win = false;
          for (auto& part : plan->parts) {
            lut |= part.tasks.count({TK_DICT_MASK, ci}) != 0;
            win |= part.tasks.count({TK_BYTES_CONTAINS, ci}) != 0;
          }
          path = lut && win ? "lut+window" : win ? "window" : lut ? "lut" : "pruned";
        }
        fprintf(stderr, "[gpuq plan] pred %zu col=%s op=%s path=%s\n", pi,
                pp.col.c_str(), op_name(pp.p.op), path.c_str());
      } else if (op_is_null(pp.p.op)) {
        const auto& n = null_dbg[pi];
        static const char* nm[] = {"nulltask", "proven", "pruned"};
        for (int k = 0; k < 3; k++)
          if (n[k]) path += (path.empty() ? "" : "+") + std::string(nm[k]);
        if (path.empty()) path = "pruned";
        fprintf(stderr,
                "[gpuq plan] pred %zu col=%s op=%s path=%s rowgroups: "
                "nulltask=%lld proven=%lld pruned=%lld\n",
                pi, pp.col.c_str(), op_name(pp.p.op), path.c_str(),
                (long long)n[0], (long long)n[1], (long long)n[2]);
      }
    }
  }
  return plan.release();
} catch (const std::exception& e) {
  if (ctx) ctx->set_error(e.what());
  return nullptr;
}

extern "C" gpuq_plan* gpuq_plan_build_from_stream(
    gpuq_ctx* ctx, const char* stream_dir,
    const char* const* projection, int32_t n_projection,
    const gpuq_pred* preds, int32_t n_preds,
    const char* const* group_by, int32_t n_group_by,
    const gpuq_agg* aggs, int32_t n_aggs, int64_t limit,
    int64_t* fast_count) try {
  if (fast_count) *fast_count = -1;
  bool bare = (n_aggs == 1 && aggs && aggs[0].op == GPUQ_AGG_COUNT_STAR &&
               n_group_by == 0);
  CatalogPlanInput in = catalog_plan(stream_dir, preds, n_preds, bare);
  if (in.fast_count >= 0) {
    if (fast_count) *fast_count = in.fast_count;
    return nullptr;
  }
  if (in.files.empty()) {
    if (fast_count) *fast_count = -2;
    return nullptr;
  }
  std::vector<gpuq_file> files(in.files.size());
  for (size_t i = 0; i < in.files.size(); i++) {
    files[i].path = in.files[i].c_str();
    files[i].row_groups = nullptr;
    files[i].n_row_groups = -1;
  }
  gpuq_plan* plan = gpuq_plan_build(ctx, files.data(), (int32_t)files.size(),
                                    projection, n_projection,
                                    preds, n_preds, group_by, n_group_by,
                                    aggs, n_aggs, limit);
  bool null_pred = false;
  for (int32_t i = 0; i < n_preds; i++) null_pred |= op_is_null(preds[i].op);
  if (plan && null_pred && plan->m_rows_scanned == 0) {
    gpuq_plan_destroy(plan);
    if (fast_count) *fast_count = -2;
    return nullptr;
  }
  return plan;
} catch (const std::exception& e) {
  if (ctx) ctx->set_error(e.what());
  return nullptr;
}

extern "C" int32_t gpuq_plan_partition_count(gpuq_plan* p) {
  return p ? (int32_t)p->parts.size() : 0;
}

extern "C" int32_t gpuq_plan_load(gpuq_plan* plan, int32_t pi) try {
  if (!plan || pi < 0 || pi >= (int32_t)plan->parts.size()) return -1;
  Partition& part = plan->parts[pi];
  if (part.loaded) return 0;
  int64_t t0 = now_ns();
  HIP_TRY(hipSetDevice(part.device));
  HIP_TRY(hipStreamCreateWithFlags(&part.stream, hipStreamNonBlocking));

  HIP_TRY(hipMalloc(&part.d_raw, std::max<uint64_t>(part.raw_bytes + 8192, 16)));
  HIP_TRY(hipMalloc(&part.d_dec, std::max<uint64_t>(part.dec_bytes, 16)));
  Ring ring(part.stream);
  {
    std::vector<Ring::Span> run;
    uint64_t run_dst = 0, cursor = 0;
    auto flush = [&]() {
      if (!run.empty()) {
        ring.copy_spans(part.d_raw + run_dst, run);
        run.clear();
      }
    };
    for (auto& t : part.chunks) {
      const auto& mf = *plan->files[t.file_idx];
      uint64_t len = (uint64_t)t.cm->total_compressed_size;
      if (t.cached) {
        flush();
      } else {
        if (run.empty()) run_dst = cursor;
        run.push_back({mf.data + t.cm->start_offset(), len});
      }
      cursor += len;
    }
    flush();
    for (auto& t : part.chunks) {
      if (!t.cached || !t.dec_len) continue;
      void* src = plan->ctx->cache_get(t.cache_key);
      if (!src) throw std::runtime_error("hot-tier entry vanished while pinned");
      HIP_TRY(hipMemcpyAsync(part.d_dec + t.dec_base, src, t.dec_len,
                             hipMemcpyDeviceToDevice, part.stream));
    }
    for (auto& h : part.himgs)
      ring.copy(part.d_dec + h.first, h.second.data(), h.second.size());
  }
  HIP_TRY(hipMalloc(&part.d_pages, std::max<size_t>(part.pages.size() * sizeof(DevPage), 16)));
  HIP_TRY(hipMemcpyAsync(part.d_pages, part.pages.data(),
                         part.pages.size() * sizeof(DevPage), hipMemcpyHostToDevice,
                         part.stream));
  auto upload_pool = [&](const void* src, size_t bytes, void** dst) {
    HIP_TRY(hipMalloc(dst, std::max<size_t>(bytes, 16)));
    if (bytes) ring.copy(*dst, src, bytes);
  };
  upload_pool(part.remap_pool.data(), part.remap_pool.size() * 4, (void**)&part.d_remap);
  upload_pool(part.dictv_pool.data(), part.dictv_pool.size() * 8, (void**)&part.d_dictv);
  upload_pool(part.lut_pool.data(), part.lut_pool.size(), (void**)&part.d_lut);
  for (auto& kv : part.tasks) {
    int32_t* d = nullptr;
    upload_pool(kv.second.data(), kv.second.size() * 4, (void**)&d);
    part.d_ids[kv.first] = d;
  }
  if (plan->fused_valagg)
    upload_pool(part.valagg_ids.data(), part.valagg_ids.size() * 4,
                (void**)&part.d_valagg_ids);
  for (size_t ci = 0; ci < plan->cols.size(); ci++) {
    auto& c = plan->cols[ci];
    if (c.is_bin || c.numeric_key) {
      int32_t* d; HIP_TRY(hipMalloc(&d, std::max<int64_t>(part.n_rows * 4, 16)));
      part.d_gid[(int)ci] = d;
      if (c.is_bin) continue;
    }
    if (c.need_gid) {
      int32_t* d; HIP_TRY(hipMalloc(&d, std::max<int64_t>(part.n_rows * 4, 16)));
      part.d_gid[(int)ci] = d;
      if (c.need_gid_valid) {
        uint8_t* v; HIP_TRY(hipMalloc(&v, std::max<int64_t>(part.n_rows, 16)));
        part.d_valid[(int)ci] = v;
      }
    }
    if (plan->fused_valagg && !plan->valagg_late && (int)ci == plan->valagg_col)
      continue;
    if (c.need_val) {
      int64_t* d; HIP_TRY(hipMalloc(&d, std::max<int64_t>(part.n_rows * 8, 16)));
      part.d_val[(int)ci] = d;
      uint8_t* v; HIP_TRY(hipMalloc(&v, std::max<int64_t>(part.n_rows, 16)));
      part.d_valid[(int)ci] = v;
    }
  }
  HIP_TRY(hipMalloc(&part.d_mask, std::max<int64_t>(part.n_rows, 16)));
  HIP_TRY(hipMalloc(&part.d_rowof, std::max<int64_t>(part.n_rows * 4, 16)));
  HIP_TRY(hipMalloc(&part.d_rank, std::max<int64_t>(part.n_rows * 4, 16)));
  HIP_TRY(hipMalloc(&part.d_scr, std::max<int64_t>(part.n_rows * 8, 16)));
  HIP_TRY(hipMalloc(&part.d_present, std::max<size_t>(part.pages.size() * 4, 16)));
  HIP_TRY(hipMalloc(&part.d_tmpvalid, std::max<int64_t>(part.n_rows, 16)));
  if (plan->is_projection) {
    int64_t n = std::max<int64_t>(part.n_rows, 16);
    HIP_TRY(hipMalloc(&part.d_keys, n * 8));
    HIP_TRY(hipMalloc(&part.d_keys_sorted, n * 8));
    HIP_TRY(hipMalloc(&part.d_rows, n * 4));
    HIP_TRY(hipMalloc(&part.d_rows_sorted, n * 4));
    HIP_TRY(hipMalloc(&part.d_count, 8));
    part.sort_temp_bytes = sort_pairs_desc(part.stream, nullptr, 0, part.d_keys,
                                           part.d_keys_sorted, part.d_rows,
                                           part.d_rows_sorted, part.n_rows);
    HIP_TRY(hipMalloc(&part.d_sort_temp, std::max<size_t>(part.sort_temp_bytes, 16)));
  }
  HIP_TRY(hipMalloc(&part.d_err, 4));
  bool hash_machinery = plan->has_hash || plan->needs_cascade ||
                        plan->has_numkey;
  size_t groups_cap = hash_machinery ? (size_t)GID_CAP : (size_t)plan->n_groups;
  size_t tsz = groups_cap * (1 + 2 * plan->aggs.size()) * 8;
  HIP_TRY(hipMalloc(&part.d_table, std::max<size_t>(tsz, 16)));
  size_t fsz = (size_t)plan->n_fsum * groups_cap * 4 * 8;
  HIP_TRY(hipMalloc(&part.d_fsum, std::max<size_t>(fsz, 16)));
  if (hash_machinery) {
    HIP_TRY(hipMalloc(&part.d_hkeys, ((1ull << HASH_LOG2) + 1) * 8));
    HIP_TRY(hipMalloc(&part.d_hgids, ((1ull << HASH_LOG2) + 1) * 4));
    HIP_TRY(hipMalloc(&part.d_hcount, 4));
    for (int ci : plan->group_cols)
      if (plan->cols[ci].hash_mode || plan->cols[ci].numeric_key) {
        uint64_t* g2r = nullptr;
        HIP_TRY(hipMalloc(&g2r, (size_t)GID_CAP * 8));
        part.d_gid2ref[ci] = g2r;
      }
    if (plan->group_cols.size() >= 2) {
      HIP_TRY(hipMalloc(&part.d_cgid, std::max<int64_t>(part.n_rows * 4, 16)));
      part.d_gid2pair.resize(plan->group_cols.size() - 1, nullptr);
      for (auto& ptr : part.d_gid2pair)
        HIP_TRY(hipMalloc(&ptr, (size_t)GID_CAP * 8));
    }
  }
  if (!plan->distinct_aggs.empty()) {
    if (!part.d_hkeys)
      HIP_TRY(hipMalloc(&part.d_hkeys, ((1ull << HASH_LOG2) + 1) * 8));
    for (int ai : plan->distinct_aggs) {
      int ci = plan->aggs[ai].col_idx;
      const auto& c = plan->cols[ci];
      if ((c.hash_mode || c.numeric_key) && !part.d_gid2ref.count(ci)) {
        uint64_t* g2r = nullptr;
        HIP_TRY(hipMalloc(&g2r, (size_t)GID_CAP * 8));
        part.d_gid2ref[ci] = g2r;
      }
      uint64_t* pl = nullptr;
      HIP_TRY(hipMalloc(&pl, (size_t)plan->distinct_pair_cap * 8));
      part.d_dpairs.push_back(pl);
    }
    HIP_TRY(hipMalloc(&part.d_dcount, plan->distinct_aggs.size() * 4));
    if (!plan->distinct_force_hash)
      HIP_TRY(hipMalloc(&part.d_dbitmap,
                        std::max<uint64_t>(plan->distinct_bitmap_bits / 8 + 8, 16)));
  }
  std::vector<int32_t> kinds;
  for (auto& a : plan->aggs) kinds.push_back(a.kind);
  upload_pool(kinds.data(), kinds.size() * 4, (void**)&part.d_agg_kind);
  upload_pool(part.segs.data(), part.segs.size() * sizeof(DevSeg),
              (void**)&part.d_segs);
  upload_pool(part.brs.data(), part.brs.size() * sizeof(DevBr),
              (void**)&part.d_brs);
  upload_pool(part.pagebrs.data(), part.pagebrs.size() * sizeof(DevPageBr),
              (void**)&part.d_pagebrs);
  upload_pool(part.res_lane.data(), part.res_lane.size() * sizeof(DevBrRes),
              (void**)&part.d_res_lane);
  upload_pool(part.res_wave.data(), part.res_wave.size() * sizeof(DevBrRes),
              (void**)&part.d_res_wave);
  upload_pool(part.piece_pool.data(), part.piece_pool.size() * sizeof(DevPiece),
              (void**)&part.d_piece_pool);
  upload_pool(part.lits_lane.data(), part.lits_lane.size() * sizeof(DevLit),
              (void**)&part.d_lits_lane);
  upload_pool(part.lits_wave.data(), part.lits_wave.size() * sizeof(DevLit),
              (void**)&part.d_lits_wave);
  upload_pool(part.brinl.data(), part.brinl.size() * sizeof(DevBrInl),
              (void**)&part.d_brinl);
  upload_pool(part.cwins.data(), part.cwins.size() * sizeof(DevCWin),
              (void**)&part.d_cwins);
  upload_pool(part.cstarts.data(), part.cstarts.size() * sizeof(uint16_t),
              (void**)&part.d_cstarts);
  std::string needle;
  part.needle_off.assign(plan->preds.size(), 0);
  {
    std::string pool;
    for (size_t i = 0; i < plan->preds.size(); i++) {
      if (plan->preds[i].p.lit_kind == GPUQ_LIT_STR) {
        part.needle_off[i] = (uint32_t)pool.size();
        pool += plan->preds[i].str_lit;
        pool.push_back('\0');
      }
    }
    needle = pool;
  }
  upload_pool(needle.data(), needle.size() + 1, (void**)&part.d_needle);

  HIP_TRY(hipStreamSynchronize(part.stream));
  part.loaded = true;
  part.load_ns = now_ns() - t0;
  {
    std::lock_guard<std::mutex> g(plan->mu);
    plan->m_load_ns += part.load_ns;
  }
  return 0;
} catch (const std::exception& e) {
  if (plan && plan->ctx) plan->ctx->set_error(e.what());
  return -1;
}

namespace {

struct ExportedBatch {
  std::vector<void*> allocs;
  void* grab(size_t n) {
    void* p = malloc(n ? n : 1);
    allocs.push_back(p);
    return p;
  }
};

void release_schema(struct ArrowSchema* s) {
  if (!s || !s->release) return;
  for (int64_t i = 0; i < s->n_children; i++)
    if (s->children[i]) { release_schema(s->children[i]); free(s->children[i]); }
  free(s->children);
  free((void*)s->format);
  free((void*)s->name);
  s->release = nullptr;
}
void release_array(struct ArrowArray* a) {
  if (!a || !a->release) return;
  for (int64_t i = 0; i < a->n_children; i++)
    if (a->children[i]) { release_array(a->children[i]); free(a->children[i]); }
  free(a->children);
  if (a->private_data) {
    auto* eb = (ExportedBatch*)a->private_data;
    for (void* p : eb->allocs) free(p);
    delete eb;
  }
  free(a->buffers);
  a->release = nullptr;
}

void make_schema_field(struct ArrowSchema* s, const char* fmt, const std::string& name) {
  memset(s, 0, sizeof(*s));
  s->format = strdup(fmt);
  s->name = strdup(name.c_str());
  s->flags = 2;
  s->release = release_schema;
}

struct StreamState {
  struct ArrowSchema schema;
  bool schema_moved = false;
  struct ArrowArray batch;
  bool batch_taken = false;
  std::string err;
};

int ss_get_schema(struct ArrowArrayStream* st, struct ArrowSchema* out) {
  auto* s = (StreamState*)st->private_data;
  *out = s->schema;
  s->schema_moved = true;
  s->schema.release = nullptr;
  return 0;
}
int ss_get_next(struct ArrowArrayStream* st, struct ArrowArray* out) {
  auto* s = (StreamState*)st->private_data;
  if (s->batch_taken) {
    memset(out, 0, sizeof(*out));
    out->release = nullptr;
    return 0;
  }
  *out = s->batch;
  s->batch.release = nullptr;
  s->batch_taken = true;
  return 0;
}
const char* ss_get_last_error(struct ArrowArrayStream* st) {
  auto* s = (StreamState*)st->private_data;
  return s->err.empty() ? nullptr : s->err.c_str();
}
void ss_release(struct ArrowArrayStream* st) {
  auto* s = (StreamState*)st->private_data;
  if (s) {
    if (s->schema.release) release_schema(&s->schema);
    if (s->batch.release) release_array(&s->batch);
    delete s;
  }
  st->release = nullptr;
}

std::vector<std::string> fetch_ref_strings(Partition& part, hipStream_t st,
                                           const std::vector<uint64_t>& refs) {
  int64_t n = (int64_t)refs.size();
  std::vector<std::string> out(n);
  if (!n) return out;
  uint64_t* d_refs = nullptr;
  uint32_t* d_lens = nullptr;
  HIP_TRY(hipMalloc(&d_refs, n * 8));
  HIP_TRY(hipMalloc(&d_lens, n * 4));
  HIP_TRY(hipMemcpyAsync(d_refs, refs.data(), n * 8, hipMemcpyHostToDevice, st));
  launch_ref_lens(st, part.d_dec, d_refs, n, d_lens);
  std::vector<uint32_t> lens(n);
  HIP_TRY(hipMemcpyAsync(lens.data(), d_lens, n * 4, hipMemcpyDeviceToHost, st));
  HIP_TRY(hipStreamSynchronize(st));
  std::vector<uint64_t> offs(n);
  uint64_t total = 0;
  for (int64_t i = 0; i < n; i++) { offs[i] = total; total += lens[i]; }
  uint64_t* d_offs = nullptr;
  uint8_t* d_out = nullptr;
  HIP_TRY(hipMalloc(&d_offs, n * 8));
  HIP_TRY(hipMalloc(&d_out, std::max<uint64_t>(total, 16)));
  HIP_TRY(hipMemcpyAsync(d_offs, offs.data(), n * 8, hipMemcpyHostToDevice, st));
  launch_ref_gather(st, part.d_dec, d_refs, d_offs, n, d_out);
  std::vector<uint8_t> bytes(total);
  if (total)
    HIP_TRY(hipMemcpyAsync(bytes.data(), d_out, total, hipMemcpyDeviceToHost, st));
  HIP_TRY(hipStreamSynchronize(st));
  for (int64_t i = 0; i < n; i++)
    out[i].assign((const char*)bytes.data() + offs[i], lens[i]);
  (void)hipFree(d_refs); (void)hipFree(d_lens);
  (void)hipFree(d_offs); (void)hipFree(d_out);
  return out;
}

void hot_tier_populate(gpuq_plan* plan, Partition& part, hipStream_t st) {
  if (part.populated) return;
  part.populated = true;
  bool any = false;
// ... 182 lines not shown
      int64_t nulls = 0;
      for (int64_t r = 0; r < k; r++) {
        offs[r] = (int32_t)off;
        if (const std::string* sp = str_at(r)) {
          memcpy(data + off, sp->data(), sp->size());
          off += sp->size();
        } else {
          validity[r / 8] &= (uint8_t)~(1 << (r % 8));
          nulls++;
        }
      }
      offs[k] = (int32_t)off;
      if (nulls) { ch->buffers[0] = validity; ch->null_count = nulls; }
      ch->buffers[1] = offs;
      ch->buffers[2] = data;
    } else {
      ch->n_buffers = 2;
      ch->buffers = (const void**)calloc(2, sizeof(void*));
      int64_t* v = (int64_t*)eb->grab(std::max<int64_t>(k * 8, 1));
      uint8_t* validity = (uint8_t*)eb->grab(std::max<int64_t>((k + 7) / 8, 1));
      memset(validity, 0xff, std::max<int64_t>((k + 7) / 8, 1));
      int64_t nulls = 0;
      for (int64_t r = 0; r < k; r++) {
        v[r] = vals[p][r];
        if (!valids[p][r]) {
          validity[r / 8] &= (uint8_t)~(1 << (r % 8));
          nulls++;
        }
      }
      if (nulls) { ch->buffers[0] = validity; ch->null_count = nulls; }
      ch->buffers[1] = v;
    }
  }
  s->cursor += k;
  return 0;
} catch (const std::exception& e) {
  auto* s = (ProjState*)st0->private_data;
  s->err = e.what();
  return 1;
}

}

int32_t execute_projection(gpuq_plan* plan, Partition& part, hipStream_t st,
                           hipEvent_t ev0, hipEvent_t ev1, hipEvent_t ev_decomp,
                           int64_t t0, bool need_mask,
                           struct ArrowArrayStream* out) {
  HIP_TRY(hipMemsetAsync(part.d_count, 0, 8, st));
  launch_compact(st, need_mask ? part.d_mask : nullptr,
                 part.d_val[plan->ts_col], part.n_rows, part.d_keys,
                 part.d_rows, part.d_count);
  unsigned long long cnt = 0;
  HIP_TRY(hipMemcpyAsync(&cnt, part.d_count, 8, hipMemcpyDeviceToHost, st));
  HIP_TRY(hipStreamSynchronize(st));
  if (cnt)
    sort_pairs_desc(st, part.d_sort_temp, part.sort_temp_bytes, part.d_keys,
                    part.d_keys_sorted, part.d_rows, part.d_rows_sorted,
                    (int64_t)cnt);
  int64_t k = plan->limit > 0 ? std::min<int64_t>((int64_t)cnt, plan->limit)
                              : (int64_t)cnt;

  HIP_TRY(hipEventRecord(ev1, st));
  int32_t herr = 0;
  HIP_TRY(hipMemcpyAsync(&herr, part.d_err, 4, hipMemcpyDeviceToHost, st));
  HIP_TRY(hipStreamSynchronize(st));
  if (herr != 0)
    throw std::runtime_error("kernel error code " + std::to_string(herr));
  hot_tier_populate(plan, part, st);
  float ms_total = 0, ms_decomp = 0;
  HIP_TRY(hipEventElapsedTime(&ms_total, ev0, ev1));
  HIP_TRY(hipEventElapsedTime(&ms_decomp, ev0, ev_decomp));
  HIP_TRY(hipEventDestroy(ev0));
  HIP_TRY(hipEventDestroy(ev1));
  HIP_TRY(hipEventDestroy(ev_decomp));

  int np = (int)plan->projection.size();
  auto* ps = new ProjState();
  ps->plan = plan;
  ps->part = &part;
  ps->total = k;
  HIP_TRY(hipMalloc(&ps->d_g64, PROJ_BATCH * 8));
  HIP_TRY(hipMalloc(&ps->d_g32, PROJ_BATCH * 4));
  HIP_TRY(hipMalloc(&ps->d_g8, PROJ_BATCH));
  memset(&ps->schema, 0, sizeof(ps->schema));
  ps->schema.format = strdup("+s");
  ps->schema.name = strdup("");
  ps->schema.release = release_schema;
  ps->schema.n_children = np;
  ps->schema.children = (struct ArrowSchema**)calloc(np, sizeof(void*));
  for (int p = 0; p < np; p++) {
    auto& c = plan->cols[plan->projection[p]];
    const char* fmt = (c.phys == PT_BYTE_ARRAY) ? "u"
                      : (c.phys == PT_DOUBLE) ? "g" : "l";
    ps->schema.children[p] = (struct ArrowSchema*)malloc(sizeof(struct ArrowSchema));
    make_schema_field(ps->schema.children[p], fmt, c.name);
  }
  memset(out, 0, sizeof(*out));
  out->get_schema = proj_get_schema;
  out->get_next = proj_get_next;
  out->get_last_error = proj_get_last_error;
  out->release = proj_release;
  out->private_data = ps;

  {
    std::lock_guard<std::mutex> g(plan->mu);
    plan->m_kernel_ns += (int64_t)(ms_total * 1e6);
    plan->m_decomp_ns += (int64_t)(ms_decomp * 1e6);
    plan->m_exec_ns += now_ns() - t0;
    plan->m_rows_out += k;
  }
  return 0;
}

}

extern "C" int32_t gpuq_plan_execute(gpuq_plan* plan, int32_t pi,
                                     struct ArrowArrayStream* out) try {
  if (!plan || pi < 0 || pi >= (int32_t)plan->parts.size()) return -1;
  Partition& part = plan->parts[pi];
  if (!part.loaded) {
    if (gpuq_plan_load(plan, pi) != 0) return -1;
  }
  HIP_TRY(hipSetDevice(part.device));
  hipStream_t st = part.stream;
  int64_t t0 = now_ns();

  hipEvent_t ev0, ev1, ev_decomp;
  HIP_TRY(hipEventCreate(&ev0));
  HIP_TRY(hipEventCreate(&ev1));
  HIP_TRY(hipEventCreate(&ev_decomp));

  const bool need_mask = !plan->preds.empty() && !part.pred_ranges.empty();
  HIP_TRY(hipMemsetAsync(part.d_err, 0, 4, st));
  if (need_mask) HIP_TRY(hipMemsetAsync(part.d_mask, 1, part.n_rows, st));
  int64_t n_groups_exec = plan->n_groups;
  bool cascaded = false;
  std::vector<uint32_t> level_claimed;
  std::vector<char> distinct_bitmap(plan->distinct_aggs.size(), 0);
  auto key_card = [&](int ci) -> int64_t {
    const auto& kc = plan->cols[ci];
    return kc.is_bin ? (int64_t)kc.nbins + 1
           : (kc.hash_mode || kc.numeric_key)
               ? (int64_t)part.hash_claimed[ci] + 1
               : (int64_t)kc.gdict.size() + 1;
  };
  if (plan->fused_count)
    launch_init_table(st, part.d_table, plan->n_groups, (int)plan->aggs.size(),
                      part.d_agg_kind);

  HIP_TRY(hipEventRecord(ev0, st));
  launch_decompress(st, DecompDev{
      part.d_raw, part.d_dec,
      part.d_segs, (int)part.segs.size(),
      part.d_lits_lane, (int64_t)part.lits_lane.size(),
      part.d_lits_wave, (int)part.lits_wave.size(),
      part.d_brinl, (int64_t)part.brinl.size(),
      part.d_res_lane, (int64_t)part.res_lane.size(),
      part.d_res_wave, (int)part.res_wave.size(),
      part.d_piece_pool, part.d_brs,
      part.d_pagebrs, (int)part.pagebrs.size(), part.d_err});
  HIP_TRY(hipEventRecord(ev_decomp, st));

  if (plan->fused_count) {
    int key_col = plan->group_cols[0];
    auto it = part.tasks.find({TK_DICT_GID, key_col});
    if (it != part.tasks.end())
      launch_dict_count(st, part.d_dec, part.d_pages, part.d_ids[it->first],
                        (int)it->second.size(), part.d_remap, part.d_table,
                        plan->n_groups, (int)plan->aggs.size(), part.d_err);
    HIP_TRY(hipEventRecord(ev1, st));
  } else {
  auto run_task = [&](const std::pair<const std::pair<int, int>,
                                      std::vector<int32_t>>& kv) {
    int kind = kv.first.first, col = kv.first.second;
    int n = (int)kv.second.size();
    int32_t* ids = part.d_ids[kv.first];
    if (part.col_null_free[col]) {
      switch (kind) {
        case TK_DICT_GID: {
          auto it = part.d_valid.find(col);
          launch_dict_gid(st, part.d_dec, part.d_pages, ids, n, part.d_remap,
                          part.d_gid[col],
                          it != part.d_valid.end() ? it->second : nullptr,
                          nullptr, 2, part.d_err);
          return;
        }
        case TK_DICT_VAL:
          launch_dict_i64(st, part.d_dec, part.d_pages, ids, n, part.d_dictv,
                          part.d_val[col], part.d_valid[col], nullptr, 2,
                          part.d_err);
          return;
        case TK_PLAIN_VAL:
          launch_plain_fixed(st, part.d_dec, part.d_pages, ids, n,
                             part.d_val[col], part.d_valid[col], nullptr, 2,
                             part.d_err);
          return;
        case TK_POOL_VAL:
          launch_pool_vals(st, part.d_dec, part.d_pages, ids, n, part.d_dictv,
                           part.d_val[col], part.d_valid[col], nullptr, 2);
          return;
        case TK_DICT_MASK:
          launch_dict_mask(st, part.d_dec, part.d_pages, ids, n, part.d_lut,
                           part.d_mask, 2, part.d_err);
          return;
        default: break;
      }
    }
    switch (kind) {
      case TK_DICT_GID: {
        auto it = part.d_valid.find(col);
        uint8_t* v = it != part.d_valid.end() ? it->second : part.d_tmpvalid;
        launch_def_levels(st, part.d_dec, part.d_pages, ids, n, v, nullptr,
                          nullptr, part.d_rank, part.d_present, part.d_err);
        launch_dict_gid(st, part.d_dec, part.d_pages, ids, n, part.d_remap,
                        part.d_gid[col],
                        it != part.d_valid.end() ? it->second : nullptr,
                        part.d_present, 0, part.d_err);
        launch_dict_gid(st, part.d_dec, part.d_pages, ids, n, part.d_remap,
                        (int32_t*)part.d_scr, nullptr, part.d_present, 1,
                        part.d_err);
        launch_expand(st, part.d_dec, part.d_pages, ids, n, part.d_scr,
                      part.d_rank, v, (uint8_t*)part.d_gid[col], 1);
        break;
      }
      case TK_DICT_VAL:
        launch_def_levels(st, part.d_dec, part.d_pages, ids, n,
                          part.d_valid[col], nullptr, nullptr,
                          part.d_rank, part.d_present, part.d_err);
        launch_dict_i64(st, part.d_dec, part.d_pages, ids, n, part.d_dictv,
                        part.d_val[col], part.d_valid[col], part.d_present, 0,
                        part.d_err);
        launch_dict_i64(st, part.d_dec, part.d_pages, ids, n, part.d_dictv,
                        (int64_t*)part.d_scr, nullptr, part.d_present, 1,
                        part.d_err);
        launch_expand(st, part.d_dec, part.d_pages, ids, n, part.d_scr,
                      part.d_rank, part.d_valid[col],
                      (uint8_t*)part.d_val[col], 0);
        break;
      case TK_PLAIN_VAL:
        launch_def_levels(st, part.d_dec, part.d_pages, ids, n,
                          part.d_valid[col], nullptr, nullptr,
                          part.d_rank, part.d_present, part.d_err);
        launch_plain_fixed(st, part.d_dec, part.d_pages, ids, n,
                           part.d_val[col], part.d_valid[col], part.d_present,
                           0, part.d_err);
        launch_plain_fixed(st, part.d_dec, part.d_pages, ids, n,
                           (int64_t*)part.d_scr, nullptr, part.d_present, 1,
                           part.d_err);
        launch_expand(st, part.d_dec, part.d_pages, ids, n, part.d_scr,
                      part.d_rank, part.d_valid[col],
                      (uint8_t*)part.d_val[col], 0);
        break;
      case TK_POOL_VAL:
        launch_def_levels(st, part.d_dec, part.d_pages, ids, n,
                          part.d_valid[col], nullptr, nullptr,
                          part.d_rank, part.d_present, part.d_err);
        launch_pool_vals(st, part.d_dec, part.d_pages, ids, n, part.d_dictv,
                         part.d_val[col], part.d_valid[col], part.d_present, 0);
        launch_pool_vals(st, part.d_dec, part.d_pages, ids, n, part.d_dictv,
                         (int64_t*)part.d_scr, nullptr, part.d_present, 1);
        launch_expand(st, part.d_dec, part.d_pages, ids, n, part.d_scr,
                      part.d_rank, part.d_valid[col],
                      (uint8_t*)part.d_val[col], 0);
        break;
      case TK_DELTA_VAL:
        launch_delta_i64(st, part.d_dec, part.d_pages, ids, n,
                         part.d_val[col], part.d_valid[col], part.d_err);
        break;
      case TK_DICT_MASK:
        launch_def_levels(st, part.d_dec, part.d_pages, ids, n,
                          part.d_tmpvalid, nullptr, nullptr,
                          part.d_rank, part.d_present, part.d_err);
        launch_dict_mask(st, part.d_dec, part.d_pages, ids, n, part.d_lut,
                         part.d_mask, 0, part.d_err);
        launch_dict_lut_scr(st, part.d_dec, part.d_pages, ids, n, part.d_lut,
                            part.d_scr, part.d_present, part.d_err);
        launch_expand(st, part.d_dec, part.d_pages, ids, n, part.d_scr,
                      part.d_rank, part.d_tmpvalid, part.d_mask, 2);
        break;
      case TK_BYTES_CONTAINS: {
        launch_def_levels(st, part.d_dec, part.d_pages, ids, n,
                          part.d_tmpvalid, part.d_mask, part.d_rowof,
                          part.d_rank, part.d_present, part.d_err);
        auto rng = part.cwin_ranges.at(col);
        for (int pidx : plan->cols[col].contains_preds) {
          const std::string& lit = plan->preds[pidx].str_lit;
          launch_str_win(st, part.d_dec, part.d_cwins + rng.first,
                         (int)rng.second, part.d_pages, part.d_cstarts,
                         part.d_needle + part.needle_off[pidx],
                         (int)lit.size(), like_mode(plan->preds[pidx].p.op),
                         part.d_rowof, part.d_mask);
        }
        break;
      }
      case TK_IS_NOT_NULL:
        launch_def_levels(st, part.d_dec, part.d_pages, ids, n,
                          part.d_tmpvalid, part.d_mask, nullptr, nullptr,
                          part.d_present, part.d_err);
        break;
      case TK_IS_NULL:
        launch_def_levels(st, part.d_dec, part.d_pages, ids, n,
                          part.d_tmpvalid, nullptr, nullptr, nullptr,
                          part.d_present, part.d_err);
        launch_null_clear_valid(st, part.d_dec, part.d_pages, ids, n,
                                part.d_tmpvalid, part.d_mask);
        break;
    }
  };
  for (auto& kv : part.tasks) {
// ... 641 lines not shown
      size_t base = (size_t)live[r] * slots;
      uint64_t cnt = empty_aggregate_row ? 0
                     : ((kind == AGGK_COUNT_STAR || cip)
                            ? table[base] : table[base + 2 + 2 * i]);
      uint64_t val = empty_aggregate_row ? 0 : table[base + 1 + 2 * i];
      if (kind == AGGK_COUNT_STAR || kind == AGGK_COUNT) {
        vv[r] = (int64_t)cnt;
      } else if (cnt == 0) {
        vv[r] = 0;
        validity[r / 8] &= (uint8_t)~(1 << (r % 8));
        nulls++;
      } else if (kind == AGGK_SUM_F64) {
        double d = acc256_to_double(
            &fsums[((size_t)fsi * n_groups_exec + (size_t)live[r]) * 4]);
        memcpy(&vv[r], &d, 8);
      } else {
        vv[r] = (int64_t)val;
      }
    }
    if (nulls) {
      chv->buffers[0] = validity;
      chv->null_count = nulls;
    }
    chv->buffers[1] = vv;

    auto* chc = make_child(f++);
    chc->n_buffers = 2;
    chc->buffers = (const void**)calloc(2, sizeof(void*));
    int64_t* cv = (int64_t*)eb->grab(nr * 8);
    for (int64_t r = 0; r < nr; r++) {
      size_t base = (size_t)live[r] * slots;
      cv[r] = empty_aggregate_row ? 0
              : (int64_t)((kind == AGGK_COUNT_STAR || cip)
                              ? table[base] : table[base + 2 + 2 * i]);
    }
    chc->buffers[1] = cv;
  }
  for (size_t di = 0; di < n_distinct; di++) {
    const int ci = plan->aggs[plan->distinct_aggs[di]].col_idx;
    const auto& c = plan->cols[ci];
    const auto& pr = dpairs[di];
    const int64_t np = (int64_t)pr.size();
    auto* chl = make_child(f++);
    chl->n_buffers = 2;
    chl->buffers = (const void**)calloc(2, sizeof(void*));
    int32_t* loffs = (int32_t*)eb->grab(((size_t)nr + 1) * 4);
    memcpy(loffs, doffs[di].data(), ((size_t)nr + 1) * 4);
    chl->buffers[1] = loffs;
    chl->n_children = 1;
    chl->children = (struct ArrowArray**)calloc(1, sizeof(void*));
    auto* item = (struct ArrowArray*)calloc(1, sizeof(struct ArrowArray));
    chl->children[0] = item;
    item->length = np;
    item->release = release_array;
    std::vector<uint64_t> g2r;
    if (c.hash_mode || c.numeric_key) {
      g2r.resize(part.hash_claimed[ci]);
      if (!g2r.empty())
        HIP_TRY(hipMemcpy(g2r.data(), part.d_gid2ref[ci], g2r.size() * 8,
                          hipMemcpyDeviceToHost));
    }
    auto vgid_of = [&](int64_t p) { return (size_t)(uint32_t)pr[(size_t)p]; };
    if (c.numeric_key) {
      item->n_buffers = 2;
      item->buffers = (const void**)calloc(2, sizeof(void*));
      int64_t* v = (int64_t*)eb->grab((size_t)np * 8);
      for (int64_t p = 0; p < np; p++) v[p] = (int64_t)g2r.at(vgid_of(p) - 1);
      item->buffers[1] = v;
      continue;
    }
    std::vector<std::string> ref_strs;
    if (c.hash_mode) {
      std::vector<uint64_t> refs((size_t)np);
      for (int64_t p = 0; p < np; p++) refs[(size_t)p] = g2r.at(vgid_of(p) - 1);
      ref_strs = fetch_ref_strings(part, st, refs);
    }
    auto str_of = [&](int64_t p) -> const std::string& {
      return c.hash_mode ? ref_strs[(size_t)p] : c.gdict.at(vgid_of(p) - 1);
    };
    size_t total = 0;
    for (int64_t p = 0; p < np; p++) total += str_of(p).size();
    if (total > (size_t)INT32_MAX)
      throw std::runtime_error("count_distinct: set column beyond 2 GiB");
    item->n_buffers = 3;
    item->buffers = (const void**)calloc(3, sizeof(void*));
    int32_t* soffs = (int32_t*)eb->grab(((size_t)np + 1) * 4);
    char* sdata = (char*)eb->grab(total);
    size_t off = 0;
    for (int64_t p = 0; p < np; p++) {
      soffs[p] = (int32_t)off;
      const auto& s = str_of(p);
      memcpy(sdata + off, s.data(), s.size());
      off += s.size();
    }
    soffs[np] = (int32_t)off;
    item->buffers[1] = soffs;
    item->buffers[2] = sdata;
  }

  memset(out, 0, sizeof(*out));
  out->get_schema = ss_get_schema;
  out->get_next = ss_get_next;
  out->get_last_error = ss_get_last_error;
  out->release = ss_release;
  out->private_data = ss;

  {
    std::lock_guard<std::mutex> g(plan->mu);
    plan->m_kernel_ns += (int64_t)(ms_total * 1e6);
    plan->m_decomp_ns += (int64_t)(ms_decomp * 1e6);
    plan->m_exec_ns += now_ns() - t0;
    plan->m_rows_out += rows_out_total;
  }
  return 0;
} catch (const std::exception& e) {
  if (plan && plan->ctx) plan->ctx->set_error(e.what());
  return -1;
}

extern "C" int32_t gpuq_plan_metrics(gpuq_plan* p, gpuq_metrics* out) {
  if (!p || !out) return -1;
  std::lock_guard<std::mutex> g(p->mu);
  memset(out, 0, sizeof(*out));
  out->rows_scanned = p->m_rows_scanned;
  out->rows_out = p->m_rows_out;
  for (auto& part : p->parts) {
    out->bytes_scanned += part.bytes_scanned;
    out->rowgroup_bytes_total += part.rowgroup_bytes_total;
    out->hbm_bytes_est += (int64_t)(part.raw_bytes + 2 * part.dec_bytes);
    out->cache_hit_bytes += part.bytes_cache_hit;
  }
  out->kernel_ns = p->m_kernel_ns;
  out->exec_ns = p->m_exec_ns;
  out->load_ns = p->m_load_ns;
  out->decomp_ns = p->m_decomp_ns;
  return 0;
}

gpuq_plan::~gpuq_plan() {
  if (ctx)
    for (auto& k : pinned_keys) ctx->cache_unpin(k);
  for (auto& part : parts) {
    if (!part.loaded) continue;
    (void)hipSetDevice(part.device);
    auto F = [](void* p) { if (p) (void)hipFree(p); };
    F(part.d_raw); F(part.d_dec); F(part.d_pages); F(part.d_remap);
    F(part.d_dictv); F(part.d_lut); F(part.d_mask); F(part.d_err);
    F(part.d_table); F(part.d_fsum); F(part.d_agg_kind);
    F(part.d_hkeys); F(part.d_hgids); F(part.d_hcount); F(part.d_cgid);
    for (auto& kv : part.d_gid2ref) F(kv.second);
    for (auto* ptr : part.d_gid2pair) F(ptr); F(part.d_needle); F(part.d_all_ids);
    F(part.d_rowof); F(part.d_rank); F(part.d_scr);
    F(part.d_present); F(part.d_tmpvalid);
    F(part.d_lits_lane); F(part.d_lits_wave);
    F(part.d_cwins); F(part.d_cstarts); F(part.d_brinl);
    F(part.d_segs); F(part.d_brs); F(part.d_pagebrs);
    F(part.d_res_lane); F(part.d_res_wave); F(part.d_piece_pool);
    F(part.d_keys); F(part.d_keys_sorted); F(part.d_rows);
    F(part.d_rows_sorted); F(part.d_count); F(part.d_sort_temp);
    for (auto& kv : part.d_ids) F(kv.second);
    F(part.d_valagg_ids);
    F(part.d_dbitmap); F(part.d_dcount);
    for (auto* ptr : part.d_dpairs) F(ptr);
    for (auto& kv : part.d_gid) F(kv.second);
    for (auto& kv : part.d_val) F(kv.second);
    for (auto& kv : part.d_valid) F(kv.second);
    if (part.stream) (void)hipStreamDestroy(part.stream);
  }
}

extern "C" void gpuq_plan_destroy(gpuq_plan* p) { delete p; }

namespace {

constexpr uint64_t DEC_PAD = 16384 + 64;
constexpr uint64_t RAW_SLACK = 8192;

void replay_decompress(const uint8_t* raw, uint8_t* dec, const DecompRecs& R) {
  for (const DevSeg& sg : R.segs) {
    const uint8_t* src = raw + sg.src_off;
    uint8_t* dst = dec + sg.dst_off;
    if (sg.raw) {
      std::memcpy(dst, src, sg.out_len);
      continue;
    }
    uint32_t s = 0, d = 0;
    while (s < sg.comp_len && d < sg.out_len) {
      uint32_t token = src[s++];
      uint32_t lit = token >> 4;
      if (lit == 15) {
        uint32_t b;
        do { b = src[s++]; lit += b; } while (b == 255);
      }
      if (s + lit > sg.comp_len || d + lit > sg.out_len)
        throw std::runtime_error("replay: segment literal overrun");
      std::memcpy(dst + d, src + s, lit);
      s += lit;
      d += lit;
      if (s >= sg.comp_len) break;
      uint32_t off = src[s] | ((uint32_t)src[s + 1] << 8);
      s += 2;
      uint32_t ml = token & 0xf;
      if (ml == 15) {
        uint32_t b;
        do { b = src[s++]; ml += b; } while (b == 255);
      }
      ml += 4;
      if (d + ml > sg.out_len)
        throw std::runtime_error("replay: segment match overrun");
      if (!sg.big && off <= d)
        for (uint32_t i = 0; i < ml; i++) dst[d + i] = dst[d + i - off];
      d += ml;
    }
    if (d != sg.out_len) throw std::runtime_error("replay: segment size mismatch");
  }
  for (const auto* lits : {&R.lits_lane, &R.lits_wave})
    for (const DevLit& L : *lits)
      std::memcpy(dec + L.b, raw + (L.a & ((1ull << 40) - 1)), L.a >> 40);
  for (const DevBrInl& r : R.brinl) {
    uint8_t* o = dec + (r.meta & ((1ull << 40) - 1));
    uint32_t len = (uint32_t)(r.meta >> 40) & 0xfff;
    uint32_t period = (uint32_t)(r.meta >> 52);
    for (uint32_t j = 0; j < len; j++)
      o[j] = (uint8_t)(r.pat >> ((j % period) * 8));
  }
  for (const auto* recs : {&R.res_lane, &R.res_wave})
    for (const DevBrRes& rec : *recs) {
      uint32_t pat_off = 0;
      for (uint32_t k = 0; k < rec.piece_n; k++) {
        const DevPiece& pc = R.piece_pool[rec.piece_start + k];
        for (uint32_t base = pat_off; base < rec.len; base += rec.off) {
          uint32_t m = std::min(pc.len, rec.len - base);
          for (uint32_t j = 0; j < m; j++)
            dec[rec.dst + base + j] = dec[pc.src + j];
        }
        pat_off += pc.len;
      }
    }
  for (const DevPageBr& pb : R.pagebrs)
    for (uint32_t r = 0; r < pb.count; r++) {
      const DevBr& br = R.brs[pb.start + r];
      for (uint32_t i = 0; i < br.len; i++) dec[br.dst + i] = dec[br.src + i];
    }
}

void check_decomp_bounds(const DecompRecs& R, uint64_t raw_len,
                         uint64_t img_len) {
  auto need = [](bool ok) {
    if (!ok) throw std::runtime_error("decompress record out of bounds");
  };
  for (const DevSeg& s : R.segs)
    need(s.src_off + s.comp_len <= raw_len && s.dst_off + s.out_len <= img_len);
  for (const auto* lits : {&R.lits_lane, &R.lits_wave})
    for (const DevLit& L : *lits)
      need((L.a & ((1ull << 40) - 1)) + (L.a >> 40) <= raw_len &&
           L.b + (L.a >> 40) <= img_len);
  for (const DevBrInl& r : R.brinl) {
    uint64_t period = r.meta >> 52;
    need(period >= 1 && period <= 8 &&
         (r.meta & ((1ull << 40) - 1)) + ((r.meta >> 40) & 0xfff) <= img_len);
  }
  for (const auto* recs : {&R.res_lane, &R.res_wave})
    for (const DevBrRes& r : *recs) {
      need(r.off >= 1 && r.dst + r.len <= img_len &&
           (uint64_t)r.piece_start + r.piece_n <= R.piece_pool.size());
      for (uint32_t k = 0; k < r.piece_n; k++) {
        const DevPiece& pc = R.piece_pool[r.piece_start + k];
        need(pc.src + pc.len <= img_len);
      }
    }
  for (const DevPageBr& pb : R.pagebrs) {
    need((uint64_t)pb.start + pb.count <= R.brs.size());
    for (uint32_t r = 0; r < pb.count; r++) {
      const DevBr& br = R.brs[pb.start + r];
      need(br.src < br.dst && br.dst + br.len <= img_len);
    }
  }
  for (const auto& h : R.himgs) need(h.first + h.second.size() <= img_len);
}

struct DevBufs {
  std::vector<void*> ptrs;
  hipStream_t stream = nullptr;
  template <class T> T* alloc(size_t bytes) {
    void* p = nullptr;
    HIP_TRY(hipMalloc(&p, std::max<size_t>(bytes, 16)));
    ptrs.push_back(p);
    return (T*)p;
  }
  template <class T> T* upload(const std::vector<T>& v) {
    T* d = alloc<T>(v.size() * sizeof(T));
    if (!v.empty())
      HIP_TRY(hipMemcpyAsync(d, v.data(), v.size() * sizeof(T),
                             hipMemcpyHostToDevice, stream));
    return d;
  }
  ~DevBufs() {
    for (void* p : ptrs) (void)hipFree(p);
    if (stream) (void)hipStreamDestroy(stream);
  }
};

}

extern "C" int32_t gpuq_test_decompress(
    gpuq_ctx* ctx, const gpuq_decomp_page* pages, int32_t n_pages,
    int32_t raw_lead, int32_t mode, uint8_t sentinel, uint8_t* out,
    uint64_t out_cap, uint64_t* arena_len, uint64_t* guard_len,
    gpuq_decomp_stats* stats, int32_t* d_err) try {
  const int pmode = mode & 0xff;
  const bool host_only = mode & (GPUQ_DECOMP_HOST_ONLY | GPUQ_DECOMP_HOST_REPLAY);
  const bool replay = mode & GPUQ_DECOMP_HOST_REPLAY;
  if (!pages || n_pages < 0 || raw_lead < 0 || raw_lead > 15 || !out ||
      !stats || pmode > GPUQ_DECOMP_FORCE_FALLBACK ||
      (mode & ~(0xff | GPUQ_DECOMP_HOST_ONLY | GPUQ_DECOMP_HOST_REPLAY)))
    throw std::runtime_error("gpuq_test_decompress: bad argument");
  if (!host_only && (!ctx || ctx->devices.empty()))
    throw std::runtime_error("gpuq_test_decompress: device mode needs a session");

  std::vector<uint64_t> src_off(n_pages), dst_off(n_pages);
  uint64_t raw_len = (uint64_t)raw_lead, img_len = 0;
  for (int32_t i = 0; i < n_pages; i++) {
    const int codec = pages[i].codec;
    if (codec != CODEC_UNCOMPRESSED && codec != CODEC_SNAPPY &&
        codec != CODEC_LZ4_RAW)
      throw std::runtime_error("gpuq_test_decompress: unsupported codec");
    if (codec == CODEC_UNCOMPRESSED && pages[i].comp_len != pages[i].uncomp_len)
      throw std::runtime_error("gpuq_test_decompress: uncompressed size mismatch");
    src_off[i] = raw_len;
    dst_off[i] = img_len;
    raw_len += pages[i].comp_len;
    img_len += ((uint64_t)pages[i].uncomp_len + 15) & ~15ull;
  }
  const uint64_t arena = img_len + DEC_PAD;
  if (arena_len) *arena_len = arena;
  if (guard_len) *guard_len = DEC_PAD;
  if (d_err) *d_err = 0;
  if (out_cap < arena)
    throw std::runtime_error("gpuq_test_decompress: output buffer too small");

  DecompRecs R;
  for (int32_t i = 0; i < n_pages; i++)
    plan_decomp_page(R, pages[i].codec, pages[i].comp, src_off[i], dst_off[i],
                     pages[i].comp_len, pages[i].uncomp_len,
                     pages[i].codec == CODEC_UNCOMPRESSED, pmode, &stats[i]);
  check_decomp_bounds(R, raw_len, img_len);

  std::vector<uint8_t> raw;
  if (!host_only || replay) {
    raw.assign(raw_len + (replay ? RAW_SLACK : 0), 0);
    for (int32_t i = 0; i < n_pages; i++)
      if (pages[i].comp_len)
        std::memcpy(raw.data() + src_off[i], pages[i].comp, pages[i].comp_len);
  }

  if (host_only) {
    std::memset(out, sentinel, arena);
    if (replay) {
      replay_decompress(raw.data(), out, R);
      for (const auto& h : R.himgs)
        std::memcpy(out + h.first, h.second.data(), h.second.size());
      return 0;
    }
    for (int32_t i = 0; i < n_pages; i++) {
      const gpuq_decomp_page& p = pages[i];
      uint8_t* o = out + dst_off[i];
      int got;
      if (stats[i].mode == GPUQ_DECOMP_PAGE_RAW) {
        if (p.uncomp_len) std::memcpy(o, p.comp, p.uncomp_len);
        got = (int)p.uncomp_len;
      } else if (p.codec == CODEC_SNAPPY) {
        got = snappy_decompress_host(p.comp, p.comp_len, o, p.uncomp_len);
      } else {
        got = lz4_decompress_host(p.comp, p.comp_len, o, p.uncomp_len);
      }
      if (got != (int)p.uncomp_len)
        throw std::runtime_error("gpuq_test_decompress: host decode failure");
    }
    return 0;
  }

  HIP_TRY(hipSetDevice(ctx->devices[0]));
  DevBufs B;
  HIP_TRY(hipStreamCreateWithFlags(&B.stream, hipStreamNonBlocking));
  uint8_t* d_raw = B.alloc<uint8_t>(raw_len + RAW_SLACK);
  uint8_t* d_dec = B.alloc<uint8_t>(arena);
  int32_t* d_e = B.alloc<int32_t>(4);
  HIP_TRY(hipMemsetAsync(d_dec, sentinel, arena, B.stream));
  HIP_TRY(hipMemsetAsync(d_e, 0, 4, B.stream));
  if (raw_len)
    HIP_TRY(hipMemcpyAsync(d_raw, raw.data(), raw_len, hipMemcpyHostToDevice,
                           B.stream));
  for (const auto& h : R.himgs)
    if (!h.second.empty())
      HIP_TRY(hipMemcpyAsync(d_dec + h.first, h.second.data(), h.second.size(),
                             hipMemcpyHostToDevice, B.stream));
  DecompDev D{
      d_raw, d_dec,
      B.upload(R.segs), (int)R.segs.size(),
      B.upload(R.lits_lane), (int64_t)R.lits_lane.size(),
      B.upload(R.lits_wave), (int)R.lits_wave.size(),
      B.upload(R.brinl), (int64_t)R.brinl.size(),
      B.upload(R.res_lane), (int64_t)R.res_lane.size(),
      B.upload(R.res_wave), (int)R.res_wave.size(),
      B.upload(R.piece_pool), B.upload(R.brs),
      B.upload(R.pagebrs), (int)R.pagebrs.size(), d_e};
  launch_decompress(B.stream, D);
  HIP_TRY(hipGetLastError());
  int32_t err = 0;
  HIP_TRY(hipMemcpyAsync(out, d_dec, arena, hipMemcpyDeviceToHost, B.stream));
  HIP_TRY(hipMemcpyAsync(&err, d_e, 4, hipMemcpyDeviceToHost, B.stream));
  HIP_TRY(hipStreamSynchronize(B.stream));
  if (d_err) *d_err = err;
  return 0;
} catch (const std::exception& e) {
  if (ctx) ctx->set_error(e.what());
  else g_null_ctx_error = e.what();
  return -1;
}
```

### parseable_amd/csrc/kernels.hip

```cpp
#include <hip/hip_runtime.h>
#include <cstring>
#include <rocprim/device/device_radix_sort.hpp>
#include "dev_types.h"
#include "meta.h"

namespace gpuq {

#define WAVE 64

#define LZ4_RING 16384
#define LZ4_IN 4096

#define SEG_MAX 8192
__global__ void __launch_bounds__(WAVE)
k_lz4_seg(const uint8_t* __restrict__ raw, uint8_t* __restrict__ dec,
          const DevSeg* __restrict__ segs, int n, int32_t* __restrict__ d_error) {
  __shared__ uint8_t seg[SEG_MAX];
  __shared__ uint8_t inbuf[LZ4_IN + 256];
  int si = blockIdx.x;
  if (si >= n) return;
  const DevSeg sg = segs[si];
  const uint8_t* src = raw + sg.src_off;
  uint8_t* dst = dec + sg.dst_off;
  const int lane = threadIdx.x;
// ... 11 lines not shown

  const uint32_t comp = sg.comp_len, uncomp = sg.out_len;
  uint32_t in_base = 0;
  bool in_valid = false;
  auto refill = [&](uint32_t pos) {
    in_base = pos & ~15u;
    uint32_t v[17];
#pragma unroll
    for (int k = 0; k < 17; k++)
      __builtin_memcpy(&v[k], src + in_base + lane * 4u + (uint32_t)k * (WAVE * 4u), 4);
#pragma unroll
    for (int k = 0; k < 17; k++)
      *(uint32_t*)&inbuf[lane * 4u + (uint32_t)k * (WAVE * 4u)] = v[k];
    __builtin_amdgcn_wave_barrier();
    asm volatile("s_waitcnt lgkmcnt(0)" ::: "memory");
    in_valid = true;
  };
  auto inb = [&](uint32_t pos) -> uint8_t {
    if (!in_valid || pos - in_base >= LZ4_IN) refill(pos);
    return inbuf[pos - in_base];
  };
  const uint32_t* in32 = (const uint32_t*)inbuf;
  uint32_t s = 0, d = 0;
  bool bad = false;
  const bool big = sg.big != 0;
  while (s < comp && d < uncomp) {
    if (!in_valid || s - in_base >= LZ4_IN) refill(s);
    uint32_t rel = s - in_base;
    uint32_t w[6];
#pragma unroll
    for (int k = 0; k < 6; k++) w[k] = in32[(rel >> 2) + k];
    uint32_t sub = rel & 3;
    auto gb = [&](uint32_t j) {
      uint32_t t = sub + j;
      return (w[t >> 2] >> ((t & 3) * 8)) & 0xffu;
    };
    uint32_t token = gb(0);
    uint32_t lit = token >> 4;
    uint32_t off, ml;
    if (lit < 15 && !big) {
      if (s + 1 + lit > comp || d + lit > uncomp) { bad = true; break; }
      if ((uint32_t)lane < lit)
        seg[d + lane] = (uint8_t)gb(1 + lane);
      __builtin_amdgcn_wave_barrier();
      s += 1 + lit; d += lit;
      if (s >= comp) break;
      if (s + 2 > comp) { bad = true; break; }
      off = gb(1 + lit) | (gb(2 + lit) << 8);
      s += 2;
      ml = token & 0xf;
      if (ml == 15) {
        uint32_t b;
        do { if (s >= comp) { bad = true; break; } b = inb(s); s++; ml += b; } while (b == 255);
        if (bad) break;
      }
    } else {
      s++;
      if (lit == 15) {
        uint32_t b;
        do { if (s >= comp) { bad = true; break; } b = inb(s); s++; lit += b; } while (b == 255);
        if (bad) break;
      }
      if (s + lit > comp || d + lit > uncomp) { bad = true; break; }
      uint32_t doneL = 0;
      while (doneL < lit) {
        if (!in_valid || (s + doneL) - in_base >= LZ4_IN) refill(s + doneL);
        uint32_t avail = LZ4_IN - ((s + doneL) - in_base);
        uint32_t chunk = min(lit - doneL, avail);
        if (big) {
          const uint8_t* lsrc = &inbuf[(s + doneL) - in_base];
          uint32_t base = d + doneL;
          for (uint32_t i = lane; i < chunk; i += WAVE) dst[base + i] = lsrc[i];
        } else {
          const uint8_t* lsrc = &inbuf[(s + doneL) - in_base];
          uint32_t base = d + doneL;
          for (uint32_t i = lane; i < chunk; i += WAVE) seg[base + i] = lsrc[i];
        }
        doneL += chunk;
      }
      __builtin_amdgcn_wave_barrier();
      s += lit; d += lit;
      if (s >= comp) break;
      if (s + 2 > comp) { bad = true; break; }
      off = inb(s) | ((uint32_t)inb(s + 1) << 8);
      s += 2;
      ml = token & 0xf;
      if (ml == 15) {
        uint32_t b2;
        do { if (s >= comp) { bad = true; break; } b2 = inb(s); s++; ml += b2; } while (b2 == 255);
        if (bad) break;
      }
    }
    ml += 4;
    if (d + ml > uncomp) { bad = true; break; }
    if (big || off > d) {
      d += ml;
      continue;
    }
    {
      uint32_t done = 0;
      __builtin_amdgcn_wave_barrier();
      while (done < ml) {
        uint32_t chunk = min(ml - done, off);
        uint32_t sbase = d + done - off;
        uint32_t dbase = d + done;
        for (uint32_t i = lane; i < chunk; i += WAVE)
          seg[dbase + i] = seg[sbase + i];
        __builtin_amdgcn_wave_barrier();
        done += chunk;
      }
      d += ml;
    }
  }
  if (bad || d != uncomp) {
    if (lane == 0) atomicExch(d_error, ERR_LZ4);
    return;
  }
  if (!big) {
    __builtin_amdgcn_wave_barrier();
    asm volatile("s_waitcnt lgkmcnt(0)" ::: "memory");
    uint32_t head = (uint32_t)((4 - ((uintptr_t)dst & 3)) & 3);
    if (head > uncomp) head = uncomp;
    for (uint32_t i = lane; i < head; i += WAVE) dst[i] = seg[i];
    uint32_t body = (uncomp - head) & ~3u;
    for (uint32_t i = lane * 4u; i < body; i += WAVE * 4u) {
      uint32_t t = head + i;
      uint32_t sh = (t & 3) * 8;
      const uint32_t* s32 = (const uint32_t*)seg;
      uint32_t v = s32[t >> 2] >> sh;
      if (sh) v |= s32[(t >> 2) + 1] << (32 - sh);
      *(uint32_t*)(dst + t) = v;
    }
    for (uint32_t i = head + body + lane; i < uncomp; i += WAVE) dst[i] = seg[i];
  }
}

__global__ void k_brres_lane(uint8_t* __restrict__ dec,
                             const DevBrRes* __restrict__ recs,
                             const DevPiece* __restrict__ pieces, int64_t n) {
  int64_t r = (int64_t)blockIdx.x * blockDim.x + threadIdx.x;
  if (r >= n) return;
  const DevBrRes rec = recs[r];
  uint32_t pat_off = 0;
  for (uint32_t k = 0; k < rec.piece_n; k++) {
    const DevPiece pc = pieces[rec.piece_start + k];
    for (uint32_t base = pat_off; base < rec.len; base += rec.off) {
      uint32_t m = min(pc.len, rec.len - base);
      for (uint32_t j = 0; j < m; j++)
        dec[rec.dst + base + j] = dec[pc.src + j];
    }
    pat_off += pc.len;
  }
}
__global__ void k_brres_inl(uint8_t* __restrict__ dec,
                            const DevBrInl* __restrict__ recs, int64_t n) {
  int64_t r = (int64_t)blockIdx.x * blockDim.x + threadIdx.x;
  if (r >= n) return;
  const DevBrInl R = recs[r];
  const uint64_t dst = R.meta & ((1ull << 40) - 1);
  const uint32_t len = (uint32_t)(R.meta >> 40) & 0xfff;
  const uint32_t period = (uint32_t)(R.meta >> 52);
  uint8_t* o = dec + dst;
  for (uint32_t j = 0; j < len; j++)
    o[j] = (uint8_t)(R.pat >> ((j % period) * 8));
}
__global__ void __launch_bounds__(WAVE)
k_brres_wave(uint8_t* __restrict__ dec, const DevBrRes* __restrict__ recs,
             const DevPiece* __restrict__ pieces, int n) {
  int r = blockIdx.x;
  if (r >= n) return;
  const DevBrRes rec = recs[r];
  uint32_t pat_off = 0;
  for (uint32_t k = 0; k < rec.piece_n; k++) {
    const DevPiece pc = pieces[rec.piece_start + k];
    for (uint32_t base = pat_off; base < rec.len; base += rec.off) {
      uint32_t m = min(pc.len, rec.len - base);
      for (uint32_t j = threadIdx.x; j < m; j += WAVE)
        dec[rec.dst + base + j] = dec[pc.src + j];
    }
    pat_off += pc.len;
  }
}

__global__ void k_lit_lane(const uint8_t* __restrict__ raw,
                           uint8_t* __restrict__ dec,
                           const DevLit* __restrict__ lits, int64_t n) {
  int64_t i = (int64_t)blockIdx.x * blockDim.x + threadIdx.x;
  if (i >= n) return;
  const DevLit L = lits[i];
  const uint8_t* s = raw + (L.a & ((1ull << 40) - 1));
  const uint32_t len = (uint32_t)(L.a >> 40);
  uint8_t* o = dec + L.b;
  uint32_t k = 0;
  for (; k + 8 <= len; k += 8) {
    uint64_t w;
    __builtin_memcpy(&w, s + k, 8);
    __builtin_memcpy(o + k, &w, 8);
  }
  for (; k < len; k++) o[k] = s[k];
}
__global__ void __launch_bounds__(WAVE)
k_lit_wave(const uint8_t* __restrict__ raw, uint8_t* __restrict__ dec,
           const DevLit* __restrict__ lits, int n) {
  if (blockIdx.x >= (unsigned)n) return;
  const DevLit L = lits[blockIdx.x];
  const uint8_t* s = raw + (L.a & ((1ull << 40) - 1));
  const uint32_t len = (uint32_t)(L.a >> 40);
  uint8_t* o = dec + L.b;
  uint32_t nw = len / 8;
  for (uint32_t w = threadIdx.x; w < nw; w += WAVE) {
    uint64_t v;
    __builtin_memcpy(&v, s + w * 8, 8);
    __builtin_memcpy(o + w * 8, &v, 8);
  }
  uint32_t t = nw * 8 + threadIdx.x;
  if (t < len) o[t] = s[t];
}

#define BR_WIN 16384
__global__ void __launch_bounds__(WAVE)
k_lz4_backrefs(uint8_t* __restrict__ dec, const DevBr* __restrict__ brs,
               const DevPageBr* __restrict__ pages, int n) {
  __shared__ uint8_t win[BR_WIN];
  int pi = blockIdx.x;
  if (pi >= n) return;
  const DevPageBr pb = pages[pi];
  const int lane = threadIdx.x;
  uint64_t page0 = pb.count ? brs[pb.start].dst : 0;
  uint64_t wend = page0 > BR_WIN ? page0 - BR_WIN : 0;
  for (uint32_t r = 0; r < pb.count; r++) {
    const DevBr br = brs[pb.start + r];
    uint64_t off = br.dst - br.src;
    if (off + br.len > BR_WIN / 2) {
      asm volatile("s_waitcnt vmcnt(0)" ::: "memory");
      uint32_t done = 0;
      while (done < br.len) {
        uint32_t chunk = (uint32_t)min((uint64_t)(br.len - done), off);
        for (uint32_t i = lane; i < chunk; i += WAVE)
          dec[br.dst + done + i] = dec[br.src + done + i];
        done += chunk;
        asm volatile("s_waitcnt vmcnt(0)" ::: "memory");
      }
      {
        uint64_t wlo = wend > BR_WIN ? wend - BR_WIN : 0;
        uint64_t a = br.dst > wlo ? br.dst : wlo;
        uint64_t b = (br.dst + br.len) < wend ? (br.dst + br.len) : wend;
        if (a < b) {
          for (uint64_t x = a + lane; x < b; x += WAVE)
            win[x & (BR_WIN - 1)] = dec[x];
          __builtin_amdgcn_wave_barrier();
          asm volatile("s_waitcnt lgkmcnt(0)" ::: "memory");
        }
      }
      continue;
    }
    uint64_t need_end = br.dst + br.len;
    if (need_end > wend) {
      uint64_t target = need_end + BR_WIN / 2;
      uint64_t new_w0 = target > BR_WIN ? target - BR_WIN : 0;
      uint64_t load_from = wend > new_w0 ? wend : new_w0;
      asm volatile("s_waitcnt vmcnt(0)" ::: "memory");
      for (uint64_t b = load_from + lane; b < target; b += WAVE)
        win[b & (BR_WIN - 1)] = dec[b];
      __builtin_amdgcn_wave_barrier();
      asm volatile("s_waitcnt lgkmcnt(0)" ::: "memory");
      wend = target;
    }
    uint32_t off32 = (uint32_t)off;
    uint32_t pow2 = (off32 & (off32 - 1)) == 0;
    for (uint32_t i = lane; i < br.len; i += WAVE) {
      uint32_t j = pow2 ? (i & (off32 - 1)) : (i % off32);
      uint8_t v = win[(br.src + j) & (BR_WIN - 1)];
      dec[br.dst + i] = v;
      win[(br.dst + i) & (BR_WIN - 1)] = v;
    }
    __builtin_amdgcn_wave_barrier();
  }
}

struct SerialRle {
  const uint8_t* p;
  const uint8_t* end;
  int bit_width, byte_w;
  uint32_t run_left = 0;
  bool packed = false;
  uint32_t rle_val = 0;
  uint64_t bit_acc = 0;
  int bit_cnt = 0;
  uint32_t pending = 0;
  bool has_pending = false;
  __device__ SerialRle(const uint8_t* p_, const uint8_t* end_, int bw)
      : p(p_), end(end_), bit_width(bw), byte_w((bw + 7) / 8) {}
  __device__ void unread(uint32_t v) { pending = v; has_pending = true; }
  __device__ uint32_t varint() {
    uint64_t v = 0; int sh = 0;
    for (;;) {
      uint8_t b = (p < end) ? *p++ : 0;
      v |= (uint64_t)(b & 0x7f) << sh;
      if (!(b & 0x80)) return (uint32_t)v;
      sh += 7;
    }
  }
  __device__ uint32_t next() {
    if (has_pending) { has_pending = false; return pending; }
    if (!run_left) {
      uint32_t hdr = varint();
      if (hdr & 1) {
        packed = true;
        run_left = (hdr >> 1) * 8;
        bit_acc = 0; bit_cnt = 0;
      } else {
        packed = false;
        run_left = hdr >> 1;
        rle_val = 0;
        for (int b = 0; b < byte_w; b++)
          rle_val |= (uint32_t)((p < end) ? *p++ : 0) << (8 * b);
      }
    }
    run_left--;
    if (!packed) return rle_val;
    while (bit_cnt < bit_width) {
      bit_acc |= (uint64_t)((p < end) ? *p++ : 0) << bit_cnt;
      bit_cnt += 8;
    }
    uint32_t v = (uint32_t)(bit_acc & ((bit_width >= 32) ? 0xffffffffull
                                                         : ((1ull << bit_width) - 1)));
    bit_acc >>= bit_width;
    bit_cnt -= bit_width;
    return v;
  }
};

__device__ inline const uint8_t* def_levels(const DevPage& pg, const uint8_t* payload,
                                            const uint8_t** def_start, uint32_t* def_len,
                                            bool* all_valid) {
  if (!pg.optional) { *def_start = nullptr; *def_len = 0; *all_valid = true; return payload; }
  uint32_t dl;
  memcpy(&dl, payload, 4);
  *def_start = payload + 4;
  *def_len = dl;
  const uint8_t* q = payload + 4;
  uint64_t hdr = 0; int sh = 0;
  for (;;) {
    uint8_t b = *q++;
    hdr |= (uint64_t)(b & 0x7f) << sh;
    if (!(b & 0x80)) break;
    sh += 7;
  }
  *all_valid = (!(hdr & 1)) && ((hdr >> 1) >= pg.num_values) && (*q == 1);
  return payload + 4 + dl;
}

// ... 1794 lines not shown
      int64_t v = val[i];
      if (K1 == AGGK_SUM_I64)
        atomicAdd((unsigned long long*)&row[3], (unsigned long long)v);
      else if (K1 == AGGK_MIN_I64) atomic_min_i64(&row[3], v);
      else if (K1 == AGGK_MAX_I64) atomic_max_i64(&row[3], v);
    }
  }
  if (USE_LDS) {
    __syncthreads();
    for (int64_t t = threadIdx.x; t < tsz; t += blockDim.x) {
      int sl = (int)(t % slots);
      uint64_t v = tab[t];
      uint64_t* g = &a.table[t];
      if (sl == 0) {
        if (v) atomicAdd((unsigned long long*)g, (unsigned long long)v);
      } else if (sl == 3 && K1 != AGGF_NONE) {
        if (K1 == AGGK_SUM_I64) {
          if (v) atomicAdd((unsigned long long*)g, (unsigned long long)v);
        } else if (K1 == AGGK_MIN_I64) {
          if ((int64_t)v != INT64_MAX) atomic_min_i64(g, (int64_t)v);
        } else if ((int64_t)v != INT64_MIN) {
          atomic_max_i64(g, (int64_t)v);
        }
      }
    }
  }
}

template <int K1>
__device__ inline void valagg_update(uint64_t* lt, int32_t g, int64_t v) {
  atomicAdd((unsigned long long*)&lt[2 * g], 1ull);
  if (K1 == AGGK_SUM_I64)
    atomicAdd((unsigned long long*)&lt[2 * g + 1], (unsigned long long)v);
  else if (K1 == AGGK_MIN_I64) atomic_min_i64(&lt[2 * g + 1], v);
  else atomic_max_i64(&lt[2 * g + 1], v);
}
template <int K1, bool MASK>
struct EmitValAgg {
  const int64_t* dictv;
  const int32_t* gid;
  const uint8_t* mask;
  uint64_t* lt;
  __device__ void operator()(uint32_t row, uint32_t idx) const {
    if (MASK && !mask[row]) return;
    valagg_update<K1>(lt, gid[row], dictv[idx]);
  }
  struct Pending { int64_t v; int32_t g; uint8_t m; bool on; };
  __device__ Pending fetch(uint32_t row, uint32_t idx, bool live) const {
    Pending p;
    p.g = gid[row];
    p.v = dictv[idx];
    p.m = MASK ? mask[row] : (uint8_t)1;
    p.on = live;
    return p;
  }
  __device__ void apply(const Pending& p) const {
    if (p.on && p.m) valagg_update<K1>(lt, p.g, p.v);
  }
};
#define VALAGG_BATCH 4
template <int K1, bool MASK> struct EmitBatch<EmitValAgg<K1, MASK>> {
  static constexpr int N = VALAGG_BATCH;
};

template <int K1, bool MASK>
__global__ void __launch_bounds__(WAVE * DP_WAVES)
k_val_agg(const uint8_t* __restrict__ dec, const DevPage* __restrict__ pages,
          const int32_t* __restrict__ ids, int n,
          const int64_t* __restrict__ dictv_pool,
          const int32_t* __restrict__ gid, const uint8_t* __restrict__ mask,
          uint64_t* __restrict__ table, int32_t n_groups, int slots,
          int32_t* d_error) {
  extern __shared__ uint64_t lt[];
  const uint64_t vinit = K1 == AGGK_MIN_I64 ? (uint64_t)INT64_MAX
                         : K1 == AGGK_MAX_I64 ? (uint64_t)INT64_MIN : 0ull;
  for (int i = threadIdx.x; i < 2 * n_groups; i += blockDim.x)
    lt[i] = (i & 1) ? vinit : 0ull;
  __syncthreads();

  for (int pi = blockIdx.x; pi < n; pi += gridDim.x) {
    const DevPage pg = pages[ids[pi]];
    const uint8_t* payload = dec + pg.dst_off;
    if (pg.encoding == ENC_PLAIN) {
      uint32_t skip = 0;
      if (pg.optional) { memcpy(&skip, payload, 4); skip += 4; }
      const uint32_t nv = pg.num_values, row0 = pg.row_start;
      if ((uint64_t)skip + (uint64_t)nv * 8 > pg.uncomp_size) {
        if (threadIdx.x == 0) atomicExch(d_error, ERR_PAGE);
        continue;
      }
      const uint8_t* vals = payload + skip;
      for (uint32_t i0 = threadIdx.x; i0 < nv; i0 += blockDim.x * VALAGG_BATCH) {
        int64_t v[VALAGG_BATCH];
        int32_t g[VALAGG_BATCH];
        uint8_t m[VALAGG_BATCH];
        bool on[VALAGG_BATCH];
#pragma unroll
        for (int u = 0; u < VALAGG_BATCH; u++) {
          uint32_t i = i0 + u * blockDim.x;
          on[u] = i < nv;
          uint32_t row = row0 + (on[u] ? i : i0);
          __builtin_memcpy(&v[u], vals + (size_t)(on[u] ? i : i0) * 8, 8);
          g[u] = gid[row];
          m[u] = MASK ? mask[row] : (uint8_t)1;
        }
#pragma unroll
        for (int u = 0; u < VALAGG_BATCH; u++)
          if (on[u] && m[u]) valagg_update<K1>(lt, g[u], v[u]);
      }
    } else {
      EmitValAgg<K1, MASK> e{dictv_pool + pg.aux_val, gid, mask, lt};
      dict_page_decode(pg, payload, e, (const uint32_t*)nullptr, ids[pi], 2,
                       d_error);
    }
  }
  __syncthreads();
  for (int g = threadIdx.x; g < n_groups; g += blockDim.x) {
    uint64_t c = lt[2 * g];
    if (!c) continue;
    uint64_t* row = table + (int64_t)g * slots;
    atomicAdd((unsigned long long*)&row[0], (unsigned long long)c);
    uint64_t v = lt[2 * g + 1];
    if (K1 == AGGK_SUM_I64) atomicAdd((unsigned long long*)&row[3], (unsigned long long)v);
    else if (K1 == AGGK_MIN_I64) atomic_min_i64(&row[3], (int64_t)v);
    else atomic_max_i64(&row[3], (int64_t)v);
  }
}

__global__ void k_init_table(uint64_t* table, int32_t n_groups, int n_aggs,
                             const int32_t* agg_kind) {
  int slots = 1 + 2 * n_aggs;
  int64_t tsz = (int64_t)n_groups * slots;
  int64_t i = (int64_t)blockIdx.x * blockDim.x + threadIdx.x;
  int64_t stride = (int64_t)gridDim.x * blockDim.x;
  for (; i < tsz; i += stride) {
    int s = (int)(i % slots);
    uint64_t init = 0;
    if (s > 0 && ((s - 1) & 1) == 0) {
      int k = agg_kind[(s - 1) / 2];
      if (k == AGGK_MIN_I64 || k == AGGK_MIN_RANK) init = (uint64_t)INT64_MAX;
      else if (k == AGGK_MAX_I64 || k == AGGK_MAX_RANK) init = (uint64_t)INT64_MIN;
      else if (k == AGGK_MIN_F64) init = 0x7ff0000000000000ull;
      else if (k == AGGK_MAX_F64) init = 0xfff0000000000000ull;
      else if (k == AGGK_MIN_STR || k == AGGK_MAX_STR) init = ~0ull;
    }
    table[i] = init;
  }
}

void launch_lz4_seg(hipStream_t st, const uint8_t* raw, uint8_t* dec,
                    const DevSeg* segs, int n, int32_t* d_err) {
  if (n) hipLaunchKernelGGL(k_lz4_seg, dim3(n), dim3(WAVE), 0, st, raw, dec, segs, n, d_err);
}
void launch_lit_lane(hipStream_t st, const uint8_t* raw, uint8_t* dec,
                     const DevLit* lits, int64_t n) {
  if (n) hipLaunchKernelGGL(k_lit_lane, dim3((int)((n + 255) / 256)), dim3(256), 0, st, raw, dec, lits, n);
}
void launch_lit_wave(hipStream_t st, const uint8_t* raw, uint8_t* dec,
                     const DevLit* lits, int n) {
  if (n) hipLaunchKernelGGL(k_lit_wave, dim3(n), dim3(WAVE), 0, st, raw, dec, lits, n);
}
void launch_lz4_backrefs(hipStream_t st, uint8_t* dec, const DevBr* brs,
                         const DevPageBr* pages, int n) {
  if (n) hipLaunchKernelGGL(k_lz4_backrefs, dim3(n), dim3(WAVE), 0, st, dec, brs, pages, n);
}
void launch_brres_lane(hipStream_t st, uint8_t* dec, const DevBrRes* recs,
                       const DevPiece* pieces, int64_t n) {
  if (n) hipLaunchKernelGGL(k_brres_lane, dim3((int)((n + 255) / 256)), dim3(256), 0, st, dec, recs, pieces, n);
}
void launch_brres_inl(hipStream_t st, uint8_t* dec, const DevBrInl* recs,
                      int64_t n) {
  if (n) hipLaunchKernelGGL(k_brres_inl, dim3((int)((n + 255) / 256)), dim3(256), 0, st, dec, recs, n);
}
void launch_brres_wave(hipStream_t st, uint8_t* dec, const DevBrRes* recs,
                       const DevPiece* pieces, int n) {
  if (n) hipLaunchKernelGGL(k_brres_wave, dim3(n), dim3(WAVE), 0, st, dec, recs, pieces, n);
}
void launch_str_win(hipStream_t st, const uint8_t* dec, const DevCWin* wins,
                    int n, const DevPage* pages, const uint16_t* starts_pool,
                    const uint8_t* needle, int nlen, int mode,
                    const uint32_t* rowof, uint8_t* mask) {
  if (!n) return;
  const bool fold = mode & STRF_FOLD, neg = mode & STRF_NEG;
  auto launch = [&](auto kern, auto... extra) {
    hipLaunchKernelGGL(kern, dim3(n), dim3(CTHREADS), 0, st, dec, wins, n,
                       pages, starts_pool, needle, nlen, extra..., rowof, mask);
  };
  switch (mode & STRF_KIND) {
    case STR_PREFIX: launch(k_affix_win<false>, (int)neg); break;
    case STR_SUFFIX: launch(k_affix_win<true>, (int)neg); break;
    default:
      if (fold && neg) launch(k_contains_win<true, true>);
      else if (fold) launch(k_contains_win<true, false>);
      else if (neg) launch(k_contains_win<false, true>);
      else launch(k_contains_win<false, false>);
      break;
  }
}
void launch_null_clear_valid(hipStream_t st, const uint8_t* dec,
                             const DevPage* pages, const int32_t* ids, int n,
                             const uint8_t* valid, uint8_t* mask) {
  if (n) hipLaunchKernelGGL(k_null_clear_valid, dim3(n), dim3(CTHREADS), 0, st, dec, pages, ids, n, valid, mask);
}
void launch_def_levels(hipStream_t st, const uint8_t* dec, const DevPage* pages,
                       const int32_t* ids, int n, uint8_t* valid,
                       uint8_t* null_mask, uint32_t* rowof, uint32_t* rank,
                       uint32_t* present, int32_t* d_err) {
  if (n) hipLaunchKernelGGL(k_def_levels, dim3(n), dim3(WAVE), 0, st, dec, pages, ids, n, valid, null_mask, rowof, rank, present, d_err);
}
void launch_dict_gid(hipStream_t st, const uint8_t* dec, const DevPage* pages,
                     const int32_t* ids, int n, const int32_t* remap_pool,
                     int32_t* out, uint8_t* valid, const uint32_t* present,
                     int mode, int32_t* d_err) {
  if (!n) return;
  EmitGidP e{}; e.pool = remap_pool; e.out = out; e.valid = valid;
  hipLaunchKernelGGL(k_dict_pages<EmitGidP>, dim3(n), dim3(WAVE * DP_WAVES), 0, st, dec, pages, ids, n, e, present, mode, d_err);
}
void launch_dict_i64(hipStream_t st, const uint8_t* dec, const DevPage* pages,
                     const int32_t* ids, int n, const int64_t* dictv_pool,
                     int64_t* out, uint8_t* valid, const uint32_t* present,
                     int mode, int32_t* d_err) {
  if (!n) return;
  EmitDictI64P e{}; e.pool = dictv_pool; e.out = out; e.valid = valid;
  hipLaunchKernelGGL(k_dict_pages<EmitDictI64P>, dim3(n), dim3(WAVE * DP_WAVES), 0, st, dec, pages, ids, n, e, present, mode, d_err);
}
void launch_dict_mask(hipStream_t st, const uint8_t* dec, const DevPage* pages,
                      const int32_t* ids, int n, const uint8_t* lut_pool,
                      uint8_t* mask, int mode, int32_t* d_err) {
  if (!n) return;
  EmitDictMaskP e{}; e.pool = lut_pool; e.mask = mask;
  hipLaunchKernelGGL(k_dict_pages<EmitDictMaskP>, dim3(n), dim3(WAVE * DP_WAVES), 0, st, dec, pages, ids, n, e, (const uint32_t*)nullptr, mode, d_err);
}
void launch_dict_lut_scr(hipStream_t st, const uint8_t* dec,
                         const DevPage* pages, const int32_t* ids, int n,
                         const uint8_t* lut_pool, uint8_t* scr,
                         const uint32_t* present, int32_t* d_err) {
  if (!n) return;
  EmitLutD e{}; e.pool = lut_pool; e.scr = scr;
  hipLaunchKernelGGL(k_dict_pages<EmitLutD>, dim3(n), dim3(WAVE * DP_WAVES), 0, st, dec, pages, ids, n, e, present, 1, d_err);
}
void launch_plain_fixed(hipStream_t st, const uint8_t* dec, const DevPage* pages,
                        const int32_t* ids, int n, int64_t* out, uint8_t* valid,
                        const uint32_t* present, int mode, int32_t* d_err) {
  if (n) hipLaunchKernelGGL(k_plain_fixed, dim3(n), dim3(WAVE), 0, st, dec, pages, ids, n, out, valid, present, mode, d_err);
}
void launch_expand(hipStream_t st, const uint8_t* dec, const DevPage* pages,
                   const int32_t* ids, int n, const uint8_t* scr,
                   const uint32_t* rank, const uint8_t* valid, uint8_t* out,
                   int mode) {
  if (n) hipLaunchKernelGGL(k_expand, dim3(n), dim3(WAVE), 0, st, dec, pages, ids, n, scr, rank, valid, out, mode);
}
void launch_delta_i64(hipStream_t st, const uint8_t* dec, const DevPage* pages,
                      const int32_t* ids, int n, int64_t* out, uint8_t* valid,
                      int32_t* d_err) {
  if (n) hipLaunchKernelGGL(k_delta_i64, dim3(n), dim3(DELTA_T), 0, st, dec, pages, ids, n, out, valid, d_err);
}
void launch_cmp_i64(hipStream_t st, const int64_t* col, const uint8_t* valid,
                    int64_t lo, int64_t hi, int mode, int hi_excl, int is_f64,
                    uint8_t* mask, int64_t n) {
  int blocks = (int)((n + 255) / 256);
  if (blocks > 4096) blocks = 4096;
  if (n) hipLaunchKernelGGL(k_cmp_i64, dim3(blocks), dim3(256), 0, st, col, valid, lo, hi, mode, hi_excl, is_f64, mask, n);
}
void launch_compact(hipStream_t st, const uint8_t* mask, const int64_t* key_col,
                    int64_t n_rows, int64_t* out_keys, uint32_t* out_rows,
                    unsigned long long* counter) {
  int blocks = (int)((n_rows + 255) / 256);
  if (blocks > 4096) blocks = 4096;
  if (n_rows)
    hipLaunchKernelGGL(k_compact_selected, dim3(blocks), dim3(256), 0, st,
                       mask, key_col, n_rows, out_keys, out_rows, counter);
}
void launch_gather_i64(hipStream_t st, const uint32_t* rows, int64_t k,
                       const int64_t* col, int64_t* out) {
  if (k) hipLaunchKernelGGL(k_gather_i64, dim3((int)((k + 255) / 256)), dim3(256), 0, st, rows, k, col, out);
}
void launch_gather_i32(hipStream_t st, const uint32_t* rows, int64_t k,
                       const int32_t* col, int32_t* out) {
  if (k) hipLaunchKernelGGL(k_gather_i32, dim3((int)((k + 255) / 256)), dim3(256), 0, st, rows, k, col, out);
}
void launch_gather_u8(hipStream_t st, const uint32_t* rows, int64_t k,
                      const uint8_t* col, uint8_t* out) {
  if (k) hipLaunchKernelGGL(k_gather_u8, dim3((int)((k + 255) / 256)), dim3(256), 0, st, rows, k, col, out);
}

void launch_bin_i64(hipStream_t st, const int64_t* col, const uint8_t* valid,
                    int64_t origin, int64_t stride, int64_t min_idx,
                    int32_t nbins, int32_t* out, int64_t n) {
  int blocks = (int)((n + 255) / 256);
  if (blocks > 4096) blocks = 4096;
  if (n) hipLaunchKernelGGL(k_bin_i64, dim3(blocks), dim3(256), 0, st, col, valid, origin, stride, min_idx, nbins, out, n);
}

void launch_init_table(hipStream_t st, uint64_t* table, int32_t n_groups,
                       int n_aggs, const int32_t* d_agg_kind) {
  int64_t tsz = (int64_t)n_groups * (1 + 2 * n_aggs);
  int blocks = (int)((tsz + 255) / 256);
  if (blocks > 4096) blocks = 4096;
  hipLaunchKernelGGL(k_init_table, dim3(blocks), dim3(256), 0, st, table, n_groups, n_aggs, d_agg_kind);
}
void launch_dict_count(hipStream_t st, const uint8_t* dec, const DevPage* pages,
                       const int32_t* ids, int n, const int32_t* remap_pool,
                       uint64_t* table, int32_t n_groups, int n_aggs,
                       int32_t* d_err) {
  if (!n) return;
  int blocks = n < 16384 ? n : 16384;
  size_t lds = (size_t)n_groups * 8;
  hipLaunchKernelGGL(k_dict_count, dim3(blocks), dim3(WAVE), lds, st,
                     dec, pages, ids, n, remap_pool, table, n_groups, n_aggs, d_err);
}

void launch_val_agg(hipStream_t st, const uint8_t* dec, const DevPage* pages,
                    const int32_t* ids, int n, const int64_t* dictv_pool,
                    const int32_t* gid, const uint8_t* mask, uint64_t* table,
                    int32_t n_groups, int n_aggs, int kind, int max_blocks,
                    int32_t* d_err) {
  if (!n) return;
  if (max_blocks < 1) max_blocks = 1;
  int per = (n + max_blocks - 1) / max_blocks;
  int blocks = (n + per - 1) / per;
  size_t lds = (size_t)n_groups * 16;
  int slots = 1 + 2 * n_aggs;
  auto launch = [&](auto kern) {
    hipLaunchKernelGGL(kern, dim3(blocks), dim3(WAVE * DP_WAVES), lds, st, dec,
                       pages, ids, n, dictv_pool, gid, mask, table, n_groups,
// ... 196 lines not shown
```

### parseable_amd/csrc/kernels_api.h

```cpp
#pragma once
#include <hip/hip_runtime.h>
#include "dev_types.h"

namespace gpuq {
void launch_lz4_seg(hipStream_t, const uint8_t* raw, uint8_t* dec,
                    const DevSeg*, int n, int32_t* d_err);
void launch_lit_lane(hipStream_t, const uint8_t* raw, uint8_t* dec,
                     const DevLit* lits, int64_t n);
void launch_lit_wave(hipStream_t, const uint8_t* raw, uint8_t* dec,
                     const DevLit* lits, int n);
void launch_lz4_backrefs(hipStream_t, uint8_t* dec, const DevBr*,
                         const DevPageBr*, int n);
void launch_brres_lane(hipStream_t, uint8_t* dec, const DevBrRes*,
                       const DevPiece*, int64_t n);
void launch_brres_inl(hipStream_t, uint8_t* dec, const DevBrInl* recs,
                      int64_t n);
void launch_brres_wave(hipStream_t, uint8_t* dec, const DevBrRes*,
                       const DevPiece*, int n);
void launch_def_levels(hipStream_t, const uint8_t* dec, const DevPage*,
                       const int32_t* ids, int n, uint8_t* valid,
                       uint8_t* null_mask, uint32_t* rowof, uint32_t* rank,
                       uint32_t* present, int32_t* d_err);
void launch_str_win(hipStream_t, const uint8_t* dec, const DevCWin* wins,
                    int n, const DevPage* pages, const uint16_t* starts_pool,
                    const uint8_t* needle, int nlen, int mode,
                    const uint32_t* rowof, uint8_t* mask);
void launch_null_clear_valid(hipStream_t, const uint8_t* dec, const DevPage*,
                             const int32_t* ids, int n, const uint8_t* valid,
                             uint8_t* mask);
void launch_dict_gid(hipStream_t, const uint8_t* dec, const DevPage*,
                     const int32_t* ids, int n, const int32_t* remap_pool,
                     int32_t* out, uint8_t* valid, const uint32_t* present,
                     int mode, int32_t* d_err);
void launch_dict_i64(hipStream_t, const uint8_t* dec, const DevPage*,
                     const int32_t* ids, int n, const int64_t* dictv_pool,
                     int64_t* out, uint8_t* valid, const uint32_t* present,
                     int mode, int32_t* d_err);
void launch_dict_mask(hipStream_t, const uint8_t* dec, const DevPage*,
                      const int32_t* ids, int n, const uint8_t* lut_pool,
                      uint8_t* mask, int mode, int32_t* d_err);
void launch_dict_lut_scr(hipStream_t, const uint8_t* dec, const DevPage*,
                         const int32_t* ids, int n, const uint8_t* lut_pool,
                         uint8_t* scr, const uint32_t* present, int32_t* d_err);
void launch_plain_fixed(hipStream_t, const uint8_t* dec, const DevPage*,
                        const int32_t* ids, int n, int64_t* out, uint8_t* valid,
                        const uint32_t* present, int mode, int32_t* d_err);
void launch_expand(hipStream_t, const uint8_t* dec, const DevPage*,
                   const int32_t* ids, int n, const uint8_t* scr,
                   const uint32_t* rank, const uint8_t* valid, uint8_t* out,
                   int mode);
void launch_delta_i64(hipStream_t, const uint8_t* dec, const DevPage*,
                      const int32_t* ids, int n, int64_t* out, uint8_t* valid,
                      int32_t* d_err);
void launch_cmp_i64(hipStream_t, const int64_t* col, const uint8_t* valid,
                    int64_t lo, int64_t hi, int mode, int hi_excl, int is_f64,
                    uint8_t* mask, int64_t n);
void launch_bin_i64(hipStream_t, const int64_t* col, const uint8_t* valid,
                    int64_t origin, int64_t stride, int64_t min_idx,
                    int32_t nbins, int32_t* out, int64_t n);
void launch_init_table(hipStream_t, uint64_t* table, int32_t n_groups,
                       int n_aggs, const int32_t* d_agg_kind);
void launch_dict_count(hipStream_t, const uint8_t* dec, const DevPage*,
                       const int32_t* ids, int n, const int32_t* remap_pool,
                       uint64_t* table, int32_t n_groups, int n_aggs,
                       int32_t* d_err);
void launch_val_agg(hipStream_t, const uint8_t* dec, const DevPage*,
                    const int32_t* ids, int n, const int64_t* dictv_pool,
                    const int32_t* gid, const uint8_t* mask, uint64_t* table,
                    int32_t n_groups, int n_aggs, int kind, int max_blocks,
                    int32_t* d_err);
void launch_agg(hipStream_t, const AggArgs&);
void launch_pool_vals(hipStream_t, const uint8_t* dec, const DevPage*,
                      const int32_t* ids, int n, const int64_t* pool,
                      int64_t* out, uint8_t* valid, const uint32_t* present,
                      int mode);
void launch_hash_build(hipStream_t, const uint8_t* dec, const int64_t* refs,
                       const uint8_t* valid, int64_t n_rows, uint64_t* hkeys,
                       int32_t* hgids, int clog2, uint32_t* counter,
                       uint64_t* gid2ref, int32_t gid_cap, int32_t* d_err);
void launch_hash_lookup(hipStream_t, const uint8_t* dec, const int64_t* refs,
                        const uint8_t* valid, int64_t n_rows,
                        const uint64_t* hkeys, const int32_t* hgids, int clog2,
                        int32_t* out_gid);
void launch_pair_build(hipStream_t, const int32_t* a, const int32_t* b,
                       int64_t n_rows, uint64_t* hkeys, int32_t* hgids,
                       int clog2, uint32_t* counter, uint64_t* gid2pair,
                       int32_t gid_cap, int32_t* d_err);
void launch_pair_lookup(hipStream_t, const int32_t* a, const int32_t* b,
                        int64_t n_rows, const uint64_t* hkeys,
                        const int32_t* hgids, int clog2, int32_t* out);
void launch_numhash_build(hipStream_t, const int64_t* vals,
                          const uint8_t* valid, int64_t n_rows,
                          uint64_t* hkeys, int32_t* hgids, int clog2,
                          uint32_t* counter, uint64_t* gid2key,
                          int32_t gid_cap, int is_f64, int32_t* d_err);
void launch_numhash_lookup(hipStream_t, const int64_t* vals,
                           const uint8_t* valid, int64_t n_rows,
                           const uint64_t* hkeys, const int32_t* hgids,
                           int clog2, int is_f64, int32_t* out_gid);
void launch_distinct_bitmap(hipStream_t, const DistinctArgs& d,
                            uint64_t* bitmap, uint32_t vpad, bool use_lds);
void launch_distinct_claim(hipStream_t, const DistinctArgs& d, uint64_t* hkeys,
                           int clog2);
void launch_cmp_str(hipStream_t, const uint8_t* dec, const int64_t* refs,
                    const uint8_t* valid, const uint8_t* lit, uint32_t lit_len,
                    int op, uint8_t* mask, int64_t n_rows);
void launch_ref_lens(hipStream_t, const uint8_t* dec, const uint64_t* refs,
                     int64_t n, uint32_t* lens);
void launch_ref_gather(hipStream_t, const uint8_t* dec, const uint64_t* refs,
                       const uint64_t* offs, int64_t n, uint8_t* out);
void launch_compact(hipStream_t, const uint8_t* mask, const int64_t* key_col,
                    int64_t n_rows, int64_t* out_keys, uint32_t* out_rows,
                    unsigned long long* counter);
void launch_gather_i64(hipStream_t, const uint32_t* rows, int64_t k,
                       const int64_t* col, int64_t* out);
void launch_gather_i32(hipStream_t, const uint32_t* rows, int64_t k,
                       const int32_t* col, int32_t* out);
void launch_gather_u8(hipStream_t, const uint32_t* rows, int64_t k,
                      const uint8_t* col, uint8_t* out);
size_t sort_pairs_desc(hipStream_t, void* d_temp, size_t temp_bytes,
                       const int64_t* keys_in, int64_t* keys_out,
                       const uint32_t* rows_in, uint32_t* rows_out, int64_t n);
}
```

Measured before the change: 29.07 billion rows/s.

## Fuse short literals and inline matches into LDS-staged sequence tiles

Short LZ4 literals and small-period inlined matches, previously written by two separate per-thread kernels with scattered byte stores, are merged into ordered sequence records grouped into contiguous tiles. Each tile is processed by one block: a prefix scan computes record offsets, the bytes are assembled in shared memory, and the block then writes them out with aligned 16-byte stores. This is meant to cut one kernel launch and replace uncoalesced small writes with coalesced ones. In exchange it adds host-side tiling logic, a block barrier per tile, and limits of 256 records and 16 KB per tile.

```diff
diff --git a/include/gpuq.h b/include/gpuq.h
--- a/include/gpuq.h
+++ b/include/gpuq.h
@@ -170,6 +170,7 @@
   uint32_t n_res_lane, n_res_wave;
   uint32_t n_pieces;
   uint32_t n_backrefs, n_far;
+  uint32_t n_tile, n_tile_rec;
 } gpuq_decomp_stats;
 
 int32_t gpuq_test_decompress(gpuq_ctx*, const gpuq_decomp_page* pages,
diff --git a/parseable_amd/_lib.py b/parseable_amd/_lib.py
--- a/parseable_amd/_lib.py
+++ b/parseable_amd/_lib.py
@@ -60,7 +60,8 @@
     _fields_ = [("mode", C.c_int32)] + [
         (n, C.c_uint32) for n in (
             "n_seq", "n_segs", "n_big", "n_lit_lane", "n_lit_wave", "n_inl",
-            "n_res_lane", "n_res_wave", "n_pieces", "n_backrefs", "n_far")
+            "n_res_lane", "n_res_wave", "n_pieces", "n_backrefs", "n_far",
+            "n_tile", "n_tile_rec")
     ]
 
 
diff --git a/parseable_amd/csrc/dev_types.h b/parseable_amd/csrc/dev_types.h
--- a/parseable_amd/csrc/dev_types.h
+++ b/parseable_amd/csrc/dev_types.h
@@ -41,7 +41,10 @@
 };
 struct DevPiece { uint64_t src; uint32_t len; uint32_t _pad; };
 struct DevLit { uint64_t a, b; };
-struct DevBrInl { uint64_t meta, pat; };
+struct DevSeq { uint64_t a, pat; };
+constexpr uint32_t SEQ_TILE_RECS = 256;
+constexpr uint32_t SEQ_TILE_BYTES = 16384;
+struct DevSeqTile { uint64_t dst0; uint64_t rec0; uint32_t n_rec; uint32_t out_len; };
 struct DevCWin {
   uint64_t src;
   uint64_t starts;
diff --git a/parseable_amd/csrc/gpuq.cpp b/parseable_amd/csrc/gpuq.cpp
--- a/parseable_amd/csrc/gpuq.cpp
+++ b/parseable_amd/csrc/gpuq.cpp
@@ -218,8 +218,9 @@
   std::vector<DevPageBr> pagebrs;
   std::vector<DevBrRes> res_lane, res_wave;
   std::vector<DevPiece> piece_pool;
-  std::vector<DevBrInl> brinl;
-  std::vector<DevLit> lits_lane, lits_wave;
+  std::vector<DevSeq> seqs;
+  std::vector<DevSeqTile> tiles;
+  std::vector<DevLit> lits_wave;
   std::vector<DevCWin> cwins;
   std::vector<uint16_t> cstarts;
   std::map<int, std::pair<uint32_t, uint32_t>> cwin_ranges;
@@ -262,9 +263,9 @@
   DevPageBr* d_pagebrs = nullptr;
   DevBrRes* d_res_lane = nullptr;
   DevBrRes* d_res_wave = nullptr;
-  DevBrInl* d_brinl = nullptr;
+  DevSeq* d_seqs = nullptr;
+  DevSeqTile* d_tiles = nullptr;
   DevPiece* d_piece_pool = nullptr;
-  DevLit* d_lits_lane = nullptr;
   DevLit* d_lits_wave = nullptr;
   DevCWin* d_cwins = nullptr;
   uint16_t* d_cstarts = nullptr;
@@ -668,8 +669,9 @@
   std::vector<DevPageBr> pagebrs;
   std::vector<DevBrRes> res_lane, res_wave;
   std::vector<DevPiece> piece_pool;
-  std::vector<DevBrInl> brinl;
-  std::vector<DevLit> lits_lane, lits_wave;
+  std::vector<DevSeq> seqs;
+  std::vector<DevSeqTile> tiles;
+  std::vector<DevLit> lits_wave;
   std::vector<std::pair<uint64_t, std::vector<uint8_t>>> himgs;
 };
 
@@ -751,12 +753,6 @@
     d2.big = sg.big;
     cb.segs.push_back(d2);
   }
-  for (const auto& lt : lp.lits) {
-    DevLit dl{(src_abs + lt.src) | ((uint64_t)lt.len << 40),
-              dst_abs + lt.dst};
-    (lt.len <= 256 ? cb.lits_lane : cb.lits_wave).push_back(dl);
-    if (st) (lt.len <= 256 ? st->n_lit_lane : st->n_lit_wave)++;
-  }
   if (lp.fallback) {
     DevPageBr pb{(uint32_t)cb.brs.size(), (uint32_t)lp.backrefs.size()};
     cb.pagebrs.push_back(pb);
@@ -767,57 +763,108 @@
         st->n_far += (br.dst - br.src) + br.len > BR_FAR;
       }
     }
-  } else if (!lp.resolved.empty()) {
-    auto lit_bytes = [&](uint32_t src, uint32_t len,
-                         uint8_t* out) -> bool {
-      const auto& Ls = lp.lits;
-      size_t lo = 0, hi = Ls.size();
-      while (lo < hi) {
-        size_t mid = (lo + hi) / 2;
-        if (Ls[mid].dst <= src) lo = mid + 1;
-        else hi = mid;
-      }
-      if (lo == 0) return false;
-      const Lz4Lit& L = Ls[lo - 1];
-      if (src < L.dst || src + len > L.dst + L.len) return false;
-      std::memcpy(out, praw + L.src + (src - L.dst), len);
-      return true;
-    };
-    for (const auto& rr : lp.resolved) {
-      uint32_t pat_len = 0;
-      for (uint32_t k = 0; k < rr.piece_n; k++)
-        pat_len += lp.pieces[rr.piece_start + k].len;
-      if (lp.litpar && pat_len > 0 && pat_len <= 8 && rr.len <= 256) {
-        uint8_t buf[8] = {0};
-        uint32_t o = 0;
-        bool ok = true;
-        for (uint32_t k = 0; k < rr.piece_n && ok; k++) {
-          const Lz4Piece& pc = lp.pieces[rr.piece_start + k];
-          ok = lit_bytes(pc.src, pc.len, buf + o);
-          o += pc.len;
-        }
-        if (ok) {
-          uint64_t pat;
-          std::memcpy(&pat, buf, 8);
-          cb.brinl.push_back({(dst_abs + rr.dst) |
-                                  ((uint64_t)rr.len << 40) |
-                                  ((uint64_t)pat_len << 52),
-                              pat});
-          if (st) st->n_inl++;
-          continue;
-        }
-      }
-      uint32_t ps = (uint32_t)cb.piece_pool.size();
-      for (uint32_t k = 0; k < rr.piece_n; k++) {
-        const Lz4Piece& pc = lp.pieces[rr.piece_start + k];
-        cb.piece_pool.push_back({dst_abs + pc.src, pc.len, 0});
-      }
-      DevBrRes rec{dst_abs + rr.dst, rr.len, rr.off, ps, rr.piece_n};
-      if (rr.len <= 256) cb.res_lane.push_back(rec);
-      else cb.res_wave.push_back(rec);
-      if (st) {
-        (rr.len <= 256 ? st->n_res_lane : st->n_res_wave)++;
-        st->n_pieces += rr.piece_n;
+    return;
+  }
+  auto lit_bytes = [&](uint32_t src, uint32_t len, uint8_t* out) -> bool {
+    const auto& Ls = lp.lits;
+    size_t lo = 0, hi = Ls.size();
+    while (lo < hi) {
+      size_t mid = (lo + hi) / 2;
+      if (Ls[mid].dst <= src) lo = mid + 1;
+      else hi = mid;
+    }
+    if (lo == 0) return false;
+    const Lz4Lit& L = Ls[lo - 1];
+    if (src < L.dst || src + len > L.dst + L.len) return false;
+    std::memcpy(out, praw + L.src + (src - L.dst), len);
+    return true;
+  };
+  auto try_inline = [&](const Lz4Resolved& rr, uint64_t* pat,
+                        uint32_t* period) -> bool {
+    uint32_t pat_len = 0;
+    for (uint32_t k = 0; k < rr.piece_n; k++)
+      pat_len += lp.pieces[rr.piece_start + k].len;
+    if (!lp.litpar || pat_len == 0 || pat_len > 8 || rr.len > 256)
+      return false;
+    uint8_t buf[8] = {0};
+    uint32_t o = 0;
+    for (uint32_t k = 0; k < rr.piece_n; k++) {
+      const Lz4Piece& pc = lp.pieces[rr.piece_start + k];
+      if (!lit_bytes(pc.src, pc.len, buf + o)) return false;
+      o += pc.len;
+    }
+    std::memcpy(pat, buf, 8);
+    *period = pat_len;
+    return true;
+  };
+  auto push_resolved = [&](const Lz4Resolved& rr) {
+    uint32_t ps = (uint32_t)cb.piece_pool.size();
+    for (uint32_t k = 0; k < rr.piece_n; k++) {
+      const Lz4Piece& pc = lp.pieces[rr.piece_start + k];
+      cb.piece_pool.push_back({dst_abs + pc.src, pc.len, 0});
+    }
+    DevBrRes rec{dst_abs + rr.dst, rr.len, rr.off, ps, rr.piece_n};
+    if (rr.len <= 256) cb.res_lane.push_back(rec);
+    else cb.res_wave.push_back(rec);
+    if (st) {
+      (rr.len <= 256 ? st->n_res_lane : st->n_res_wave)++;
+      st->n_pieces += rr.piece_n;
+    }
+  };
+  bool open = false;
+  auto push_seq = [&](uint64_t dst, const DevSeq& rec, uint32_t len) {
+    if (open) {
+      const DevSeqTile& t = cb.tiles.back();
+      if (t.dst0 + t.out_len != dst || t.n_rec == SEQ_TILE_RECS ||
+          t.out_len + len > SEQ_TILE_BYTES)
+        open = false;
+    }
+    if (!open) {
+      cb.tiles.push_back({dst, (uint64_t)cb.seqs.size(), 0, 0});
+      open = true;
+      if (st) st->n_tile++;
+    }
+    cb.seqs.push_back(rec);
+    cb.tiles.back().n_rec++;
+    cb.tiles.back().out_len += len;
+    if (st) st->n_tile_rec++;
+  };
+  auto match_bits = [](uint32_t len, uint32_t period) {
+    return ((uint64_t)len << 49) | ((uint64_t)period << 58);
+  };
+  size_t li = 0, ri = 0;
+  const size_t nl = lp.lits.size(), nr = lp.resolved.size();
+  while (li < nl || ri < nr) {
+    uint64_t pat = 0;
+    uint32_t period = 0;
+    if (ri >= nr || (li < nl && lp.lits[li].dst < lp.resolved[ri].dst)) {
+      const Lz4Lit& lt = lp.lits[li++];
+      if (lt.len > 256) {
+        cb.lits_wave.push_back({(src_abs + lt.src) | ((uint64_t)lt.len << 40),
+                                dst_abs + lt.dst});
+        if (st) st->n_lit_wave++;
+        continue;
+      }
+      if (st) st->n_lit_lane++;
+      DevSeq rec{(src_abs + lt.src) | ((uint64_t)lt.len << 40), 0};
+      uint32_t len = lt.len;
+      if (ri < nr && lp.resolved[ri].dst == lt.dst + lt.len &&
+          try_inline(lp.resolved[ri], &pat, &period)) {
+        const Lz4Resolved& rr = lp.resolved[ri++];
+        rec.a |= match_bits(rr.len, period);
+        rec.pat = pat;
+        len += rr.len;
+        if (st) st->n_inl++;
+      }
+      push_seq(dst_abs + lt.dst, rec, len);
+    } else {
+      const Lz4Resolved& rr = lp.resolved[ri++];
+      if (try_inline(rr, &pat, &period)) {
+        push_seq(dst_abs + rr.dst, {src_abs | match_bits(rr.len, period), pat},
+                 rr.len);
+        if (st) st->n_inl++;
+      } else {
+        push_resolved(rr);
       }
     }
   }
@@ -827,9 +874,9 @@
   const uint8_t* d_raw;
   uint8_t* d_dec;
   const DevSeg* d_segs; int n_segs;
-  const DevLit* d_lits_lane; int64_t n_lits_lane;
+  const DevSeq* d_seqs;
+  const DevSeqTile* d_tiles; int n_tiles;
   const DevLit* d_lits_wave; int n_lits_wave;
-  const DevBrInl* d_brinl; int64_t n_brinl;
   const DevBrRes* d_res_lane; int64_t n_res_lane;
   const DevBrRes* d_res_wave; int n_res_wave;
   const DevPiece* d_piece_pool;
@@ -840,9 +887,8 @@
 
 void launch_decompress(hipStream_t st, const DecompDev& d) {
   launch_lz4_seg(st, d.d_raw, d.d_dec, d.d_segs, d.n_segs, d.d_err);
-  launch_lit_lane(st, d.d_raw, d.d_dec, d.d_lits_lane, d.n_lits_lane);
+  launch_seq_tile(st, d.d_raw, d.d_dec, d.d_seqs, d.d_tiles, d.n_tiles);
   launch_lit_wave(st, d.d_raw, d.d_dec, d.d_lits_wave, d.n_lits_wave);
-  launch_brres_inl(st, d.d_dec, d.d_brinl, d.n_brinl);
   launch_brres_lane(st, d.d_dec, d.d_res_lane, d.d_piece_pool, d.n_res_lane);
   launch_brres_wave(st, d.d_dec, d.d_res_wave, d.d_piece_pool, d.n_res_wave);
   launch_lz4_backrefs(st, d.d_dec, d.d_brs, d.d_pagebrs, d.n_pagebrs);
@@ -1562,8 +1608,8 @@
       const size_t nc = cbs.size();
       std::vector<size_t> o_pages(nc + 1, 0), o_segs(nc + 1, 0),
           o_brs(nc + 1, 0), o_pagebrs(nc + 1, 0), o_rl(nc + 1, 0),
-          o_rw(nc + 1, 0), o_pp(nc + 1, 0), o_bi(nc + 1, 0),
-          o_ll(nc + 1, 0), o_lw(nc + 1, 0);
+          o_rw(nc + 1, 0), o_pp(nc + 1, 0), o_sq(nc + 1, 0),
+          o_ti(nc + 1, 0), o_lw(nc + 1, 0);
       for (size_t i = 0; i < nc; i++) {
         const auto& cb = cbs[i];
         o_pages[i + 1] = o_pages[i] + cb.pages.size();
@@ -1573,8 +1619,8 @@
         o_rl[i + 1] = o_rl[i] + cb.res_lane.size();
         o_rw[i + 1] = o_rw[i] + cb.res_wave.size();
         o_pp[i + 1] = o_pp[i] + cb.piece_pool.size();
-        o_bi[i + 1] = o_bi[i] + cb.brinl.size();
-        o_ll[i + 1] = o_ll[i] + cb.lits_lane.size();
+        o_sq[i + 1] = o_sq[i] + cb.seqs.size();
+        o_ti[i + 1] = o_ti[i] + cb.tiles.size();
         o_lw[i + 1] = o_lw[i] + cb.lits_wave.size();
       }
       part.pages.resize(o_pages[nc]);
@@ -1584,8 +1630,8 @@
       part.res_lane.resize(o_rl[nc]);
       part.res_wave.resize(o_rw[nc]);
       part.piece_pool.resize(o_pp[nc]);
-      part.brinl.resize(o_bi[nc]);
-      part.lits_lane.resize(o_ll[nc]);
+      part.seqs.resize(o_sq[nc]);
+      part.tiles.resize(o_ti[nc]);
       part.lits_wave.resize(o_lw[nc]);
       parallel_for(nc, [&](size_t i) {
         auto& cb = cbs[i];
@@ -1613,10 +1659,13 @@
           r2.piece_start += piece_base;
           part.res_wave[o_rw[i] + j] = r2;
         }
-        std::copy(cb.brinl.begin(), cb.brinl.end(),
-                  part.brinl.begin() + o_bi[i]);
-        std::copy(cb.lits_lane.begin(), cb.lits_lane.end(),
-                  part.lits_lane.begin() + o_ll[i]);
+        std::copy(cb.seqs.begin(), cb.seqs.end(),
+                  part.seqs.begin() + o_sq[i]);
+        for (size_t j = 0; j < cb.tiles.size(); j++) {
+          DevSeqTile t2 = cb.tiles[j];
+          t2.rec0 += o_sq[i];
+          part.tiles[o_ti[i] + j] = t2;
+        }
         std::copy(cb.lits_wave.begin(), cb.lits_wave.end(),
                   part.lits_wave.begin() + o_lw[i]);
       });
@@ -1919,13 +1968,25 @@
     }
     for (size_t p = 0; p < plan->parts.size(); p++) {
       const auto& pt = plan->parts[p];
+      size_t period_le3 = 0;
+      for (const DevSeq& r : pt.seqs) {
+        const uint32_t ml = (uint32_t)(r.a >> 49) & 0x1ff;
+        const uint32_t n = std::min(ml, (uint32_t)(r.a >> 58));
+        for (uint32_t q = 1; q <= 3 && ml; q++) {
+          bool ok = true;
+          for (uint32_t j = q; j < n && ok; j++)
+            ok = (uint8_t)(r.pat >> (j * 8)) == (uint8_t)(r.pat >> ((j - q) * 8));
+          if (ok) { period_le3++; break; }
+        }
+      }
       fprintf(stderr,
               "[gpuq plan] part %zu: rows=%lld chunks=%zu pages=%zu segs=%zu "
-              "lits=%zu/%zu brinl=%zu res=%zu/%zu pieces=%zu raw=%.2fGB "
+              "tiles=%zu tile_recs=%zu period_le3=%zu lits_wave=%zu "
+              "res=%zu/%zu pieces=%zu raw=%.2fGB "
               "dec=%.2fGB cwins=%zu\n",
               p, (long long)pt.n_rows, pt.chunks.size(), pt.pages.size(),
-              pt.segs.size(), pt.lits_lane.size(), pt.lits_wave.size(),
-              pt.brinl.size(), pt.res_lane.size(), pt.res_wave.size(),
+              pt.segs.size(), pt.tiles.size(), pt.seqs.size(), period_le3,
+              pt.lits_wave.size(), pt.res_lane.size(), pt.res_wave.size(),
               pt.piece_pool.size(), pt.raw_bytes / 1e9, pt.dec_bytes / 1e9,
               pt.cwins.size());
     }
@@ -2175,12 +2236,12 @@
               (void**)&part.d_res_wave);
   upload_pool(part.piece_pool.data(), part.piece_pool.size() * sizeof(DevPiece),
               (void**)&part.d_piece_pool);
-  upload_pool(part.lits_lane.data(), part.lits_lane.size() * sizeof(DevLit),
-              (void**)&part.d_lits_lane);
+  upload_pool(part.seqs.data(), part.seqs.size() * sizeof(DevSeq),
+              (void**)&part.d_seqs);
+  upload_pool(part.tiles.data(), part.tiles.size() * sizeof(DevSeqTile),
+              (void**)&part.d_tiles);
   upload_pool(part.lits_wave.data(), part.lits_wave.size() * sizeof(DevLit),
               (void**)&part.d_lits_wave);
-  upload_pool(part.brinl.data(), part.brinl.size() * sizeof(DevBrInl),
-              (void**)&part.d_brinl);
   upload_pool(part.cwins.data(), part.cwins.size() * sizeof(DevCWin),
               (void**)&part.d_cwins);
   upload_pool(part.cstarts.data(), part.cstarts.size() * sizeof(uint16_t),
@@ -2669,9 +2730,8 @@
   launch_decompress(st, DecompDev{
       part.d_raw, part.d_dec,
       part.d_segs, (int)part.segs.size(),
-      part.d_lits_lane, (int64_t)part.lits_lane.size(),
+      part.d_seqs, part.d_tiles, (int)part.tiles.size(),
       part.d_lits_wave, (int)part.lits_wave.size(),
-      part.d_brinl, (int64_t)part.brinl.size(),
       part.d_res_lane, (int64_t)part.res_lane.size(),
       part.d_res_wave, (int)part.res_wave.size(),
       part.d_piece_pool, part.d_brs,
@@ -3619,8 +3679,8 @@
     for (auto* ptr : part.d_gid2pair) F(ptr); F(part.d_needle); F(part.d_all_ids);
     F(part.d_rowof); F(part.d_rank); F(part.d_scr);
     F(part.d_present); F(part.d_tmpvalid);
-    F(part.d_lits_lane); F(part.d_lits_wave);
-    F(part.d_cwins); F(part.d_cstarts); F(part.d_brinl);
+    F(part.d_seqs); F(part.d_tiles); F(part.d_lits_wave);
+    F(part.d_cwins); F(part.d_cstarts);
     F(part.d_segs); F(part.d_brs); F(part.d_pagebrs);
     F(part.d_res_lane); F(part.d_res_wave); F(part.d_piece_pool);
     F(part.d_keys); F(part.d_keys_sorted); F(part.d_rows);
@@ -3681,16 +3741,22 @@
     }
     if (d != sg.out_len) throw std::runtime_error("replay: segment size mismatch");
   }
-  for (const auto* lits : {&R.lits_lane, &R.lits_wave})
-    for (const DevLit& L : *lits)
-      std::memcpy(dec + L.b, raw + (L.a & ((1ull << 40) - 1)), L.a >> 40);
-  for (const DevBrInl& r : R.brinl) {
-    uint8_t* o = dec + (r.meta & ((1ull << 40) - 1));
-    uint32_t len = (uint32_t)(r.meta >> 40) & 0xfff;
-    uint32_t period = (uint32_t)(r.meta >> 52);
-    for (uint32_t j = 0; j < len; j++)
-      o[j] = (uint8_t)(r.pat >> ((j % period) * 8));
-  }
+  for (const DevSeqTile& t : R.tiles) {
+    uint8_t* o = dec + t.dst0;
+    for (uint32_t k = 0; k < t.n_rec; k++) {
+      const DevSeq& r = R.seqs[t.rec0 + k];
+      const uint32_t lit = (uint32_t)(r.a >> 40) & 0x1ff;
+      const uint32_t ml = (uint32_t)(r.a >> 49) & 0x1ff;
+      const uint32_t period = (uint32_t)(r.a >> 58);
+      std::memcpy(o, raw + (r.a & ((1ull << 40) - 1)), lit);
+      o += lit;
+      for (uint32_t j = 0; j < ml; j++)
+        o[j] = (uint8_t)(r.pat >> ((j % period) * 8));
+      o += ml;
+    }
+  }
+  for (const DevLit& L : R.lits_wave)
+    std::memcpy(dec + L.b, raw + (L.a & ((1ull << 40) - 1)), L.a >> 40);
   for (const auto* recs : {&R.res_lane, &R.res_wave})
     for (const DevBrRes& rec : *recs) {
       uint32_t pat_off = 0;
@@ -3718,14 +3784,24 @@
   };
   for (const DevSeg& s : R.segs)
     need(s.src_off + s.comp_len <= raw_len && s.dst_off + s.out_len <= img_len);
-  for (const auto* lits : {&R.lits_lane, &R.lits_wave})
-    for (const DevLit& L : *lits)
-      need((L.a & ((1ull << 40) - 1)) + (L.a >> 40) <= raw_len &&
-           L.b + (L.a >> 40) <= img_len);
-  for (const DevBrInl& r : R.brinl) {
-    uint64_t period = r.meta >> 52;
-    need(period >= 1 && period <= 8 &&
-         (r.meta & ((1ull << 40) - 1)) + ((r.meta >> 40) & 0xfff) <= img_len);
+  for (const DevLit& L : R.lits_wave)
+    need((L.a & ((1ull << 40) - 1)) + (L.a >> 40) <= raw_len &&
+         L.b + (L.a >> 40) <= img_len);
+  for (const DevSeqTile& t : R.tiles) {
+    need(t.n_rec >= 1 && t.n_rec <= SEQ_TILE_RECS &&
+         t.out_len <= SEQ_TILE_BYTES && t.rec0 + t.n_rec <= R.seqs.size() &&
+         t.dst0 + t.out_len <= img_len);
+    uint64_t sum = 0;
+    for (uint32_t k = 0; k < t.n_rec; k++) {
+      const DevSeq& r = R.seqs[t.rec0 + k];
+      const uint64_t lit = (r.a >> 40) & 0x1ff, ml = (r.a >> 49) & 0x1ff;
+      const uint64_t period = r.a >> 58;
+      need(lit <= 256 && ml <= 256 &&
+           (r.a & ((1ull << 40) - 1)) + lit <= raw_len &&
+           (ml == 0 || (period >= 1 && period <= 8)));
+      sum += lit + ml;
+    }
+    need(sum == t.out_len);
   }
   for (const auto* recs : {&R.res_lane, &R.res_wave})
     for (const DevBrRes& r : *recs) {
@@ -3865,9 +3941,8 @@
   DecompDev D{
       d_raw, d_dec,
       B.upload(R.segs), (int)R.segs.size(),
-      B.upload(R.lits_lane), (int64_t)R.lits_lane.size(),
+      B.upload(R.seqs), B.upload(R.tiles), (int)R.tiles.size(),
       B.upload(R.lits_wave), (int)R.lits_wave.size(),
-      B.upload(R.brinl), (int64_t)R.brinl.size(),
       B.upload(R.res_lane), (int64_t)R.res_lane.size(),
       B.upload(R.res_wave), (int)R.res_wave.size(),
       B.upload(R.piece_pool), B.upload(R.brs),
diff --git a/parseable_amd/csrc/kernels.hip b/parseable_amd/csrc/kernels.hip
--- a/parseable_amd/csrc/kernels.hip
+++ b/parseable_amd/csrc/kernels.hip
@@ -187,18 +187,6 @@
     pat_off += pc.len;
   }
 }
-__global__ void k_brres_inl(uint8_t* __restrict__ dec,
-                            const DevBrInl* __restrict__ recs, int64_t n) {
-  int64_t r = (int64_t)blockIdx.x * blockDim.x + threadIdx.x;
-  if (r >= n) return;
-  const DevBrInl R = recs[r];
-  const uint64_t dst = R.meta & ((1ull << 40) - 1);
-  const uint32_t len = (uint32_t)(R.meta >> 40) & 0xfff;
-  const uint32_t period = (uint32_t)(R.meta >> 52);
-  uint8_t* o = dec + dst;
-  for (uint32_t j = 0; j < len; j++)
-    o[j] = (uint8_t)(R.pat >> ((j % period) * 8));
-}
 __global__ void __launch_bounds__(WAVE)
 k_brres_wave(uint8_t* __restrict__ dec, const DevBrRes* __restrict__ recs,
              const DevPiece* __restrict__ pieces, int n) {
@@ -217,22 +205,60 @@
   }
 }
 
-__global__ void k_lit_lane(const uint8_t* __restrict__ raw,
-                           uint8_t* __restrict__ dec,
-                           const DevLit* __restrict__ lits, int64_t n) {
-  int64_t i = (int64_t)blockIdx.x * blockDim.x + threadIdx.x;
-  if (i >= n) return;
-  const DevLit L = lits[i];
-  const uint8_t* s = raw + (L.a & ((1ull << 40) - 1));
-  const uint32_t len = (uint32_t)(L.a >> 40);
-  uint8_t* o = dec + L.b;
-  uint32_t k = 0;
-  for (; k + 8 <= len; k += 8) {
-    uint64_t w;
-    __builtin_memcpy(&w, s + k, 8);
-    __builtin_memcpy(o + k, &w, 8);
-  }
-  for (; k < len; k++) o[k] = s[k];
+__global__ void __launch_bounds__(SEQ_TILE_RECS)
+k_seq_tile(const uint8_t* __restrict__ raw, uint8_t* __restrict__ dec,
+           const DevSeq* __restrict__ seqs,
+           const DevSeqTile* __restrict__ tiles, int n) {
+  __shared__ __attribute__((aligned(16))) uint8_t stage[SEQ_TILE_BYTES + 16];
+  __shared__ uint32_t wtot[SEQ_TILE_RECS / WAVE];
+  if (blockIdx.x >= (unsigned)n) return;
+  const DevSeqTile T = tiles[blockIdx.x];
+  const uint32_t t = threadIdx.x, lane = t & (WAVE - 1);
+  const uint32_t out_len = min(T.out_len, SEQ_TILE_BYTES);
+  uint8_t* o = dec + T.dst0;
+  const uint32_t pad = (uint32_t)((uintptr_t)o & 15);
+
+  DevSeq R{0, 0};
+  if (t < T.n_rec) R = seqs[T.rec0 + t];
+  const uint32_t lit = (uint32_t)(R.a >> 40) & 0x1ff;
+  const uint32_t ml = (uint32_t)(R.a >> 49) & 0x1ff;
+  const uint32_t period = (uint32_t)(R.a >> 58);
+  const uint32_t len = lit + ml;
+  uint32_t incl = len;
+#pragma unroll
+  for (int d = 1; d < WAVE; d <<= 1) {
+    uint32_t y = __shfl_up(incl, d, WAVE);
+    if (lane >= (uint32_t)d) incl += y;
+  }
+  if (lane == WAVE - 1) wtot[t / WAVE] = incl;
+  __syncthreads();
+  uint32_t off = incl - len;
+  for (uint32_t w = 0; w < t / WAVE; w++) off += wtot[w];
+
+  if (off + len <= out_len) {
+    uint8_t* sp = stage + pad + off;
+    const uint8_t* s = raw + (R.a & ((1ull << 40) - 1));
+    for (uint32_t k = 0; k < lit; k += 8) {
+      uint64_t w;
+      __builtin_memcpy(&w, s + k, 8);
+      const uint32_t m = min(8u, lit - k);
+      for (uint32_t j = 0; j < m; j++) sp[k + j] = (uint8_t)(w >> (j * 8));
+    }
+    sp += lit;
+    for (uint32_t j = 0, q = 0; j < ml; j++) {
+      sp[j] = (uint8_t)(R.pat >> (q * 8));
+      if (++q == period) q = 0;
+    }
+  }
+  __syncthreads();
+
+  const uint32_t head = min((16u - pad) & 15u, out_len);
+  if (t < head) o[t] = stage[pad + t];
+  const uint32_t body = (out_len - head) & ~15u;
+  for (uint32_t i = t * 16u; i < body; i += SEQ_TILE_RECS * 16u)
+    *(uint4*)(o + head + i) = *(const uint4*)(stage + pad + head + i);
+  const uint32_t tl = head + body + t;
+  if (tl < out_len) o[tl] = stage[pad + tl];
 }
 __global__ void __launch_bounds__(WAVE)
 k_lit_wave(const uint8_t* __restrict__ raw, uint8_t* __restrict__ dec,
@@ -2333,9 +2359,9 @@
                     const DevSeg* segs, int n, int32_t* d_err) {
   if (n) hipLaunchKernelGGL(k_lz4_seg, dim3(n), dim3(WAVE), 0, st, raw, dec, segs, n, d_err);
 }
-void launch_lit_lane(hipStream_t st, const uint8_t* raw, uint8_t* dec,
-                     const DevLit* lits, int64_t n) {
-  if (n) hipLaunchKernelGGL(k_lit_lane, dim3((int)((n + 255) / 256)), dim3(256), 0, st, raw, dec, lits, n);
+void launch_seq_tile(hipStream_t st, const uint8_t* raw, uint8_t* dec,
+                     const DevSeq* seqs, const DevSeqTile* tiles, int n) {
+  if (n) hipLaunchKernelGGL(k_seq_tile, dim3(n), dim3(SEQ_TILE_RECS), 0, st, raw, dec, seqs, tiles, n);
 }
 void launch_lit_wave(hipStream_t st, const uint8_t* raw, uint8_t* dec,
                      const DevLit* lits, int n) {
@@ -2348,10 +2374,6 @@
 void launch_brres_lane(hipStream_t st, uint8_t* dec, const DevBrRes* recs,
                        const DevPiece* pieces, int64_t n) {
   if (n) hipLaunchKernelGGL(k_brres_lane, dim3((int)((n + 255) / 256)), dim3(256), 0, st, dec, recs, pieces, n);
-}
-void launch_brres_inl(hipStream_t st, uint8_t* dec, const DevBrInl* recs,
-                      int64_t n) {
-  if (n) hipLaunchKernelGGL(k_brres_inl, dim3((int)((n + 255) / 256)), dim3(256), 0, st, dec, recs, n);
 }
 void launch_brres_wave(hipStream_t st, uint8_t* dec, const DevBrRes* recs,
                        const DevPiece* pieces, int n) {
diff --git a/parseable_amd/csrc/kernels_api.h b/parseable_amd/csrc/kernels_api.h
--- a/parseable_amd/csrc/kernels_api.h
+++ b/parseable_amd/csrc/kernels_api.h
@@ -5,16 +5,14 @@
 namespace gpuq {
 void launch_lz4_seg(hipStream_t, const uint8_t* raw, uint8_t* dec,
                     const DevSeg*, int n, int32_t* d_err);
-void launch_lit_lane(hipStream_t, const uint8_t* raw, uint8_t* dec,
-                     const DevLit* lits, int64_t n);
+void launch_seq_tile(hipStream_t, const uint8_t* raw, uint8_t* dec,
+                     const DevSeq* seqs, const DevSeqTile* tiles, int n);
 void launch_lit_wave(hipStream_t, const uint8_t* raw, uint8_t* dec,
                      const DevLit* lits, int n);
 void launch_lz4_backrefs(hipStream_t, uint8_t* dec, const DevBr*,
                          const DevPageBr*, int n);
 void launch_brres_lane(hipStream_t, uint8_t* dec, const DevBrRes*,
                        const DevPiece*, int64_t n);
-void launch_brres_inl(hipStream_t, uint8_t* dec, const DevBrInl* recs,
-                      int64_t n);
 void launch_brres_wave(hipStream_t, uint8_t* dec, const DevBrRes*,
                        const DevPiece*, int n);
 void launch_def_levels(hipStream_t, const uint8_t* dec, const DevPage*,
```

Measured after the change: 31.77 billion rows/s, median of 6. 1.09x the previous value.
